# hhcho/sfgwas

Hardware: AMD Instinct MI355X
Metric: pca_power_iter_ring_macs_per_s (higher is better)
Workload: dtype u64 ring words, exact integers: int8 digits on the matrix core for the MAC of all five moduli, fp64-held integers in the encode and key-switch kernels

## Files before the change

sfgwas_amd/csrc/common.hpp:

```cpp
#pragma once
#include <hip/hip_runtime.h>
#include <cstdint>
#include <cstdio>
#include <cstring>
#include <string>
#include <vector>
#include <map>
#include <set>
#include <unistd.h>
#include "../../include/sfgwas_hip.h"
#include "consts.hpp"

typedef unsigned long long u64;
typedef unsigned __int128 u128;

constexpr unsigned long long SFG_I8_BIG_QMAX = 0x7F7F7F7F7F80ULL;

struct ModConst {
    double q, qinv;
    double ninv, ninv_q;
    u64 qi;
};

struct RotKey {
    u64 *key_dev = nullptr;
    uint16_t *index_dev = nullptr;
};

struct PhaseStat { double ms = 0; int launches = 0; double bytes = 0; };
struct PendingEvent { hipEvent_t e0, e1; std::string name; int launches; double bytes; };

struct sfg_geno {
    const int8_t *dev = nullptr;
    size_t nrow = 0, ncol = 0, ld = 0;
    bool owned = false;
    bool packed = false;
    struct PtcEntry { double *slot; bool transposed; };
    mutable std::map<uint64_t, PtcEntry> ptc;
    mutable size_t ptc_budget = 0, ptc_used = 0;
    mutable double *ptc_arena = nullptr;
    mutable uint32_t *ptc_perm = nullptr;
    mutable const void *ptc_owner = nullptr;
    mutable size_t ptc_hits = 0, ptc_fills = 0;
};

struct SfgConfig {
    int mm_group = 8;
    bool mm_group_auto = true;
    size_t acc_budget = 24ULL << 30;
    size_t assoc_cache_budget = 160ULL << 30;
    size_t ksw_budget = 4ULL << 30;
    int enc_batch = 2048;
    bool upload_blocking = false;
    bool test_hooks = false;
    std::string test_scratch_oom;
    double tie_band = 0x1p-50;
    bool mac_i8_big = true;
    bool mac_reg = false;
    bool mac_bc = true;
    bool mac_i8 = true;
    bool mac_i8_nolds = true;
    bool mac_i8_ring = true;
    int mac_i8_waves = 12;
    bool mac_i8_wg1 = false;
    int mac_wc = 1;
    bool no_overlap = true;
    bool ntt_fwd_full = false;
    bool ntt_half_full = false;
    bool pt_compact = true;
    bool pt_kmajor = true;
    int pt_ride = 192;
    int i8_mover_depth_ride = 1, i8_mover_nt_ride = 1;
    bool mac_plain_pt = false;
    bool assoc_trace = false;
};

struct SfgShared {
    int device = 0;
    int logN = SFG_LOGN, N = SFG_N, nq = 0, np = 0, nmod = 0, beta = 0;
    double scale = 0;
    u64 q[SFG_MAXMOD] = {0}, psi[SFG_MAXMOD] = {0};
    double *tw_fwd = nullptr;
    double *tw_inv = nullptr;
    double2 *pack_fwd = nullptr;
    double2 *pack_inv = nullptr;
    ModConst *modc = nullptr;
    ModConst modc_host[SFG_MAXMOD];
    void *enc_tables = nullptr;
    void *rvec_tables = nullptr;
    void *zeros_dev = nullptr;
    u64 *sk_dev = nullptr;
    u64 *pk_dev = nullptr;
    u64 *skqp_dev = nullptr;
    uint32_t enc_key[8] = {0, 0, 0, 0, 0, 0, 0, 0}; uint32_t *enc_key_dev = nullptr; bool enc_seeded = false;
    u64 enc_next = 0;
    std::map<u64, RotKey> rotkeys;
    SfgConfig cfg;
    int refs = 1;
};

struct sfg_ctx {
    SfgShared *sh = nullptr;
    bool is_fork = false;
    int device = 0;
    int logN = SFG_LOGN, N = SFG_N, nq = 0, np = 0, nmod = 0, beta = 0;
    double scale = 0;
    u64 q[SFG_MAXMOD] = {0}, psi[SFG_MAXMOD] = {0};
    double *tw_fwd = nullptr, *tw_inv = nullptr;
    double2 *pack_fwd = nullptr, *pack_inv = nullptr;
    ModConst *modc = nullptr;
    ModConst modc_host[SFG_MAXMOD];
    SfgConfig cfg;
    unsigned ntt_plain_seq = 0;
    struct I8Slot { const void *src = nullptr; u64 sig[8] = {0, 0, 0, 0, 0, 0, 0, 0}; u64 last_use = 0; };
    static constexpr int I8_SLOTS = 16;
    u64 i8_gen = 1, i8_clock = 0; I8Slot i8_slot[2][I8_SLOTS];
    hipStream_t own_stream = nullptr, stream = nullptr;
    hipStream_t user_stream = nullptr;
    hipStream_t aux_stream = nullptr;
    unsigned char *pin = nullptr; size_t pin_bytes = 0, pin_head = 0;
    hipStream_t coll_stream = nullptr;
    hipEvent_t ev_pipe[4] = {nullptr, nullptr, nullptr, nullptr};
    std::vector<hipEvent_t> ev_pool; size_t ev_next = 0;
    std::map<int, void *> ksw_cache;
    void *ws = nullptr; size_t ws_bytes = 0;
    std::map<std::string, std::pair<void *, size_t>> pool;
    std::map<std::string, std::pair<void *, size_t>> host_pool;
    std::map<std::string, unsigned long long> pool_epoch;
    unsigned long long api_epoch = 0; int api_depth = 0;
    int scratch_oom_seen = 0;
    std::vector<PendingEvent> pending;
    std::string err;
    std::map<std::string, PhaseStat> phases;
    std::set<const sfg_geno *> ptc_genos;
    bool test_hooks = false;
    void *tie_count_dev = nullptr;
    hipStream_t main_stream() const { return user_stream ? user_stream : own_stream; }
    std::map<u64, RotKey> &rotkeys() { return sh->rotkeys; }
    const std::map<u64, RotKey> &rotkeys() const { return sh->rotkeys; }
    void *enc_tables() const { return sh->enc_tables; }
    void *zeros_dev() const { return sh->zeros_dev; }
};

int sfg_sync_all(sfg_ctx *ctx);
int sfg_encoder_check(sfg_ctx *ctx);
void sfg_ptc_detach_all(sfg_ctx *ctx);
void sfg_ptc_invalidate_all(sfg_ctx *ctx);

int encrypt_set_attrs(sfg_ctx *ctx);
int sfg_rows_from_montgomery(sfg_ctx *ctx, unsigned long long *rows_dev, size_t nrows, int nmod);
void sfg_encrypt_destroy(SfgShared *sh);
int enc_take_indices(sfg_ctx *ctx, const char *what, int nct, unsigned long long *first);
int keygen_set_attrs(sfg_ctx *ctx);
void sfg_keygen_destroy(SfgShared *sh);
int sfg_rvec_init(sfg_ctx *ctx);
void sfg_rvec_destroy(SfgShared *sh);

extern thread_local std::string g_create_error;

#define SFG_FAIL(ctx, ...) do { char _b[512]; snprintf(_b, sizeof _b, __VA_ARGS__); (ctx)->err = _b; return 1; } while (0)
#ifdef SFG_AB
#include "ab/ab.hpp"
#endif
#define SFG_HIP(ctx, call) do { hipError_t _e = (call); if (_e != hipSuccess) { char _b[512]; \
    snprintf(_b, sizeof _b, "HIP call failed: %s (%s:%d)", hipGetErrorString(_e), __FILE__, __LINE__); (ctx)->err = _b; return 1; } } while (0)
#define SFG_TRY(expr) do { int _rc = (expr); if (_rc) return _rc; } while (0)

int sfg_ws_reserve(sfg_ctx *ctx, size_t bytes);

static inline u64 h_mulmod(u64 a, u64 b, u64 q) { return (u64)(((u128)a * b) % q); }
static inline u64 h_powmod(u64 a, u64 e, u64 q) { u64 r = 1 % q; a %= q; while (e) { if (e & 1) r = h_mulmod(r, a, q); a = h_mulmod(a, a, q); e >>= 1; } return r; }
static inline u64 h_invmod(u64 a, u64 q) { return h_powmod(a, q - 2, q); }
static inline uint32_t h_brev(uint32_t x, int bits) { uint32_t r = 0; for (int i = 0; i < bits; i++) { r = (r << 1) | (x & 1); x >>= 1; } return r; }

int sfg_upload_small(sfg_ctx *ctx, void *dst_dev, const void *src_host, size_t bytes);
struct ApiScope {
    sfg_ctx *c;
    explicit ApiScope(sfg_ctx *c_) : c(c_) { if (c->api_depth++ == 0) c->api_epoch++; }
    ~ApiScope() { c->api_depth--; }
};
struct AuxScope {
    sfg_ctx *c; hipStream_t saved;
    explicit AuxScope(sfg_ctx *c_, bool on = true) : c(c_), saved(c_->stream) { if (on) c->stream = c->aux_stream; }
    ~AuxScope() { c->stream = saved; }
};
template <class T, hipError_t (*Free)(T)> struct HipOwner {
    T h = T();
    HipOwner() {}
    HipOwner(HipOwner &&o) : h(o.release()) {}
    HipOwner(const HipOwner &) = delete; HipOwner &operator=(const HipOwner &) = delete;
    ~HipOwner() { if (h) (void)Free(h); }
    T release() { T t = h; h = T(); return t; }
};
typedef HipOwner<void *, hipFree> DevMem;
typedef HipOwner<hipEvent_t, hipEventDestroy> EventOwner;
typedef HipOwner<hipStream_t, hipStreamDestroy> StreamOwner;
struct FdOwner {
    int fd;
    explicit FdOwner(int fd_ = -1) : fd(fd_) {}
    FdOwner(FdOwner &&o) : fd(o.fd) { o.fd = -1; }
    FdOwner(const FdOwner &) = delete; FdOwner &operator=(const FdOwner &) = delete;
    ~FdOwner() { reset(); }
    void reset(int fd_ = -1) { if (fd >= 0) close(fd); fd = fd_; }
};
int sfg_stream_after(sfg_ctx *ctx, hipStream_t waiter, hipStream_t signaller);
int sfg_scratch(sfg_ctx *ctx, const char *name, size_t bytes, void **out);
int sfg_host_scratch(sfg_ctx *ctx, const char *name, size_t bytes, void **out);
void sfg_phases_resolve(sfg_ctx *ctx);

struct PhaseTimer {
    sfg_ctx *ctx; const char *name; hipEvent_t e0, e1; bool on;
    PhaseTimer(sfg_ctx *c, const char *n, bool enable = true) : ctx(c), name(n), on(enable) {
        if (on) { (void)hipEventCreate(&e0); (void)hipEventCreate(&e1); (void)hipEventRecord(e0, ctx->stream); }
    }
    void stop(int launches = 1, double bytes = 0) {
        if (!on) return;
        (void)hipEventRecord(e1, ctx->stream);
        ctx->pending.push_back(PendingEvent{e0, e1, name, launches, bytes});
        on = false;
        if (ctx->pending.size() > 4096) sfg_phases_resolve(ctx);
    }
    ~PhaseTimer() { stop(0); }
};

constexpr u64 PACKED_ZERO = 0ULL;
#ifdef __HIPCC__
__device__ __host__ __forceinline__ u64 pack_limbs(u64 w) {
    return (w & 0xFFF) | (((w >> 12) & 0xFFF) << 16) | ((w >> 24) << 32);
}

__device__ __forceinline__ double mulmod_lazy(double x, double w, double wq, double q) {
    double qh = __builtin_rint(x * wq);
    double h = x * w;
    double l = __builtin_fma(x, w, -h);
    double r = __builtin_fma(-qh, q, h);
    return r + l;
}
__device__ __forceinline__ double mulmod_lazy_q(double x, double w, double q, double qinv) {
    double h = x * w;
    double qh = __builtin_rint(h * qinv);
    double l = __builtin_fma(x, w, -h);
    double r = __builtin_fma(-qh, q, h);
    return r + l;
}
__device__ __forceinline__ double canon(double x, double q, double qinv) {
    const double r = __builtin_fma(-__builtin_floor(x * qinv), q, x);
    return r == q ? 0.0 : r;
}
__device__ __forceinline__ double canon_le(double x, double q, double qinv) {
    return __builtin_fma(-__builtin_floor(x * qinv), q, x);
}
__device__ __forceinline__ double pred(double x, double q, double qinv) {
    double qh = __builtin_rint(x * qinv);
    return __builtin_fma(-qh, q, x);
}
__device__ __forceinline__ double u64_to_f64(u64 x) {
    return __longlong_as_double((long long)(x | 0x4330000000000000ULL)) - 4503599627370496.0;
}
__device__ __forceinline__ u64 f64_to_u64(double x) {
    return (u64)__double_as_longlong(x + 4503599627370496.0) & 0x000FFFFFFFFFFFFFULL;
}
__device__ __forceinline__ void bytes_tr4(unsigned w0, unsigned w1, unsigned w2, unsigned w3, unsigned (&o)[4]) {
    const unsigned p0 = __builtin_amdgcn_perm(w1, w0, 0x05010400u), p1 = __builtin_amdgcn_perm(w1, w0, 0x07030602u);
    const unsigned q0 = __builtin_amdgcn_perm(w3, w2, 0x05010400u), q1 = __builtin_amdgcn_perm(w3, w2, 0x07030602u);
    o[0] = __builtin_amdgcn_perm(q0, p0, 0x05040100u); o[1] = __builtin_amdgcn_perm(q0, p0, 0x07060302u);
    o[2] = __builtin_amdgcn_perm(q1, p1, 0x05040100u); o[3] = __builtin_amdgcn_perm(q1, p1, 0x07060302u);
}
__device__ __forceinline__ int sq_sum4_i8(int w) {
    const int sq = __builtin_amdgcn_sdot4(w, w, 0, false);
    if (sq < 128) return sq;
    int s = 0;
#pragma unroll
    for (int k = 0; k < 4; k++) { const int x = (int)(int8_t)(w >> (8 * k)); s += (int)(int8_t)(x * x); }
    return s;
}
__device__ __forceinline__ u64 pack_limbs_f64(double x) {
    const u64 b = (u64)__double_as_longlong(x + 4503599627370496.0);
    const unsigned lo = (unsigned)b, hi = (unsigned)(b >> 32);
    const unsigned x01 = ((lo << 4) & 0x0FFF0000u) | (lo & 0xFFFu);
    const unsigned x2 = __builtin_amdgcn_alignbit(hi, lo, 24) & 0xFFFu;
    return ((u64)x2 << 32) | x01;
}
__device__ __forceinline__ u64 d_mulmod_u64(u64 a, u64 b, u64 q) {
    u64 hi = __umul64hi(a, b), lo = a * b;
    u64 r = hi % q;
    for (int i = 63; i >= 0; i--) { u64 top = r >> 63; r = (r << 1) | ((lo >> i) & 1); if (top || r >= q) r -= q; }
    return r;
}
__device__ __forceinline__ u64 splitmix_at(u64 seed, u64 idx) {
    u64 z = seed + 0x9E3779B97F4A7C15ULL * (idx + 1);
    z = (z ^ (z >> 30)) * 0xBF58476D1CE4E5B9ULL;
    z = (z ^ (z >> 27)) * 0x94D049BB133111EBULL;
    return z ^ (z >> 31);
}
#endif
```

sfgwas_amd/csrc/kernels.hpp:

```cpp
#pragma once
#include "common.hpp"
#include "mm_plan.hpp"
#include "assoc_plan.hpp"

constexpr int SFG_MAXPATTERN = 128;
struct ModPattern { int period; int8_t m[SFG_MAXPATTERN]; };
struct RowMap { int rpg; size_t gstride_in, gstride_out; };
struct PanelMap { int G, g, shift0; unsigned packed_mask = 0; int K = 0; };

int launch_ntt_fwd(sfg_ctx *ctx, const u64 *in, u64 *out, size_t nrows, const ModPattern &pat);
int launch_ntt_inv(sfg_ctx *ctx, const u64 *in, u64 *out, size_t nrows, const ModPattern &pat);
int launch_ntt_plain(sfg_ctx *ctx, const double *pc, u64 *out, size_t nplain, int L);
struct MoveJob;
struct PtRide;
int launch_ntt_plain_half(sfg_ctx *ctx, const double *pc, u64 *out_half, size_t nplain, int L, PanelMap pm, const uint32_t *perm = nullptr, const MoveJob *mv = nullptr);
int launch_expand_half(sfg_ctx *ctx, const u64 *half, u64 *full, size_t nrows);
int launch_ntt_fwd_map(sfg_ctx *ctx, const u64 *in, u64 *out, size_t nrows, const ModPattern &pat, const RowMap &rm);
int launch_ntt_inv_map(sfg_ctx *ctx, const u64 *in, u64 *out, size_t nrows, const ModPattern &pat, const RowMap &rm);
struct MacStrides { size_t rot_k, rot_r, pt_k, pt_n, out_n, out_r; bool pt_half = false; bool pt_packed = false; bool pt_digits = false; bool i8 = false; bool i8_big = false; bool pt_digits_big = false;
                    const int8_t *B_small = nullptr, *B_big = nullptr;
                    int pt_layout = 0, pt_L = 0;
                    int B_mode = 0;
                    const int8_t *A_small = nullptr, *A_big = nullptr; };
int launch_mac_i8_small(sfg_ctx *ctx, const double *rotf, size_t rotf_k_stride, size_t rotf_r_stride, int plane0, const u64 *pt, u64 *out, int K, int R, int r0, int Ncols,
                        int l0, int nl, int accumulate, const MacStrides &st);
int launch_mac_i8_big(sfg_ctx *ctx, const double *rotf, size_t rotf_k_stride, size_t rotf_r_stride, int plane0, const u64 *pt, u64 *out, int K, int R, int r0, int Ncols,
                      int l0, int accumulate, const MacStrides &st);
int launch_skew(sfg_ctx *ctx, const int8_t *blk, size_t ld, int r, int c, int transposed, int square, int8_t *D);
struct PcCache { double *slot = nullptr; int mode = 0; const uint32_t *perm = nullptr; };
int launch_encode_rows(sfg_ctx *ctx, const int8_t *D, int shift0, int nshift, int L, u64 *pt, bool half_rows = false, int G = 0, int g = 0, unsigned packed_mask = 0, const PcCache *pcache = nullptr,
                       PtRide *ride = nullptr);
int encode_rows_launches(const sfg_ctx *ctx, int nshift);
int i8_ride_prepare(sfg_ctx *ctx, const u64 *panel, int K, int Ncols, size_t pt_k, size_t pt_n, int layout, int L, int launches, PtRide &ride);
int i8_ride_finish(sfg_ctx *ctx, PtRide &ride);
int i8_ride_tiles(sfg_ctx *ctx, int K, int L, int8_t **Bs, int8_t **Bb);
struct I8Args;
void launch_i8_pack_pt_digits(hipStream_t q, const I8Args &a, unsigned items, bool big);
void launch_move_alone(hipStream_t q, const MoveJob &j);
int launch_share(sfg_ctx *ctx, const u64 *rows, size_t rows_ct_stride, const u64 *xr, size_t x_ct_stride, u64 *h, int nl, int nct);
int launch_add_rows(sfg_ctx *ctx, const u64 *a, size_t a_ct_stride, const u64 *b, size_t b_ct_stride, u64 *out, size_t out_ct_stride, int nl, int nct);
int encrypt_errors_moddown(sfg_ctx *ctx, const int32_t *e0, const int32_t *e1, int nct, int level, u64 *out);
int launch_geno_unpack(sfg_ctx *ctx, const sfg_geno *g, size_t r0, size_t c0, size_t nr, size_t nc, int8_t *out, size_t ld_out);
int launch_rotate_right(sfg_ctx *ctx, const u64 *in, u64 *out, int nct, int level, const int *nrot_host);
int launch_rotate_right_indexed(sfg_ctx *ctx, const u64 *in, int nin, u64 *out, int nct, int level, const int *nrot_host, const int *in_index);
int launch_rotate_right_indexed_f64(sfg_ctx *ctx, const u64 *in, int nin, double *outf, int nct, int level, const int *nrot_host, const int *in_index, int L,
                                    const size_t *out_slot = nullptr);
int launch_relinearize(sfg_ctx *ctx, const u64 *tmp, int nct, int level, const u64 *mid, u64 *out);
int launch_ct_add(sfg_ctx *ctx, const u64 *a, const u64 *b, u64 *out, size_t nct, int level);
int mac_dma_planes(sfg_ctx *ctx, int L, std::vector<int> &plane_of, std::vector<int> &is_big);
double mac_big_maxterm(u64 q);
int launch_rot_to_f64(sfg_ctx *ctx, const u64 *rot, size_t nrows, int nl_rot, int L, double *rotf);
int launch_mac_dma(sfg_ctx *ctx, const double *rotf, size_t rows_per_k, const u64 *pt, u64 *out, int K, int R, int Ncols, int L, int accumulate, const MacStrides &st,
                   const double *rotsum = nullptr);
int launch_rot_sum(sfg_ctx *ctx, const double *rotf, size_t rows_per_k, int K, int L, double *rotsum);
int launch_pack_pt(sfg_ctx *ctx, const u64 *in, u64 *out, size_t nrows, size_t words_per_row, int L, unsigned packed_mask);
unsigned mac_dma_packed_mask(sfg_ctx *ctx, int L);
bool mac_use_dma(const sfg_ctx *ctx);
int launch_mac_bc(sfg_ctx *ctx, const double *rotf, size_t rows_per_k, const u64 *pt, u64 *out, int K, int R, int Ncols, int L, int accumulate, const MacStrides &st,
                  const double *rotsum);
int rotcache_build_rows_tab(sfg_ctx *ctx, const u64 *A, int s, int in_level, int max_level, int nbr, int b0, int b1, const std::vector<std::vector<uint8_t>> *tabs, double *cache);
int assoc_build_rotcache(sfg_ctx *ctx, const u64 *A_dev, int s, int in_level, int max_level, size_t nr, const std::vector<size_t> &widths, double **out);
struct I8RotPre { int G = 0, nbr = 0, s = 0, L = 0; std::vector<int8_t *> As, Ab; };
int i8_rotpre_build(sfg_ctx *ctx, const u64 *A_dev, int s, int in_level, int max_level, int nbr, const std::vector<std::vector<uint8_t>> *tabs, size_t budget_bytes, const char *prefix, I8RotPre &pre);
void i8_rotpre_free(I8RotPre &pre);
struct I8RotPreScope { I8RotPre pre; ~I8RotPreScope() { i8_rotpre_free(pre); } };
int matmul_resident_range_i8pre(sfg_ctx *ctx, const I8RotPre &pre, int s, int max_level, const sfg_geno *g, unsigned flags, int blk0, int blk1, uint64_t *out);
int matmul_accumulate_i8pre(sfg_ctx *ctx, const I8RotPre &pre, int s, int max_level, const sfg_geno *g, unsigned flags, int j0, int j1, int accumulate, uint64_t *acc,
                            size_t acc_col_words = 0);
int launch_i8_pack_rot_to(sfg_ctx *ctx, const double *rotf, size_t rotf_k_stride, size_t rotf_r_stride, int plane0, int K, int R, int l0, int nl, bool big, int8_t *A_out);
struct AssocRot { double *f64 = nullptr; I8RotPre pre; };
int assoc_build_rot(sfg_ctx *ctx, const u64 *A_dev, int s, int in_level, int max_level, size_t nr, const std::vector<size_t> &widths, AssocRot &out);
void assoc_free_rot(AssocRot &r);
struct AssocRotScope { AssocRot r; ~AssocRotScope() { assoc_free_rot(r); } };
int assoc_product(sfg_ctx *ctx, const AssocRot &r, const uint64_t *A_dev, int s, int in_level, int max_level, const sfg_geno *g, unsigned flags, int nct, uint64_t *out);
int assoc_batch_tail(sfg_ctx *ctx, const u64 *tmp, const sfg_geno *g, int s, size_t nct, size_t ctw, uint64_t *out_dev, size_t out_ct_capacity, size_t out_shift,
                     double *sum_host, double *sqsum_host);

int launch_bed_decode(sfg_ctx *ctx, hipStream_t st, const uint8_t *dbed, size_t bps, size_t num_sample, size_t num_snp, const int32_t *rmap, const int32_t *cmap,
                      int8_t *out, size_t ld);
int launch_bed_decode_lut(sfg_ctx *ctx, hipStream_t st, const uint8_t *dbed, size_t bps, size_t num_sample, size_t num_snp, const int32_t *rmap, const int32_t *cmap,
                          int8_t *out, size_t ld, unsigned lut);
int upload_filter_map(sfg_ctx *ctx, const uint8_t *filt, size_t n, DevMem &map, size_t *kept);

int assoc_stream_part(sfg_ctx *ctx, int fmt, const char *path, size_t num_sample, size_t num_snp, const uint8_t *row_filter, const uint8_t *col_filter,
                      size_t batch_snps, const uint64_t *A_dev, int s, int in_level, int max_level, unsigned flags,
                      uint64_t *out_dev, size_t out_ct_capacity, size_t *out_ct, double *sum_host, double *sqsum_host,
                      int part, int nparts, std::vector<std::pair<size_t, size_t>> *ranges);
```

sfgwas_amd/csrc/matmul.hip:

```cpp
#include "common.hpp"
#include "kernels.hpp"
#include "i8_move.hpp"
#include <algorithm>
#include <string>

static inline int ceil_div(size_t a, size_t b) { return (int)((a + b - 1) / b); }

struct Shape {
    size_t nrow, ncol;
    int nbr, m_ct;
    bool transposed;
    const int8_t *dev; size_t ld;
    const sfg_geno *g;
    int rows_of(int bi) const { return (int)(std::min((size_t)(bi + 1) * SFG_SLOTS, nrow) - (size_t)bi * SFG_SLOTS); }
    int cols_of(int bj) const { return (int)(std::min((size_t)(bj + 1) * SFG_SLOTS, ncol) - (size_t)bj * SFG_SLOTS); }
    const int8_t *block(int bi, int bj) const {
        return transposed ? dev + (size_t)bj * SFG_SLOTS * ld + (size_t)bi * SFG_SLOTS
                          : dev + (size_t)bi * SFG_SLOTS * ld + (size_t)bj * SFG_SLOTS;
    }
};
static Shape make_shape(const sfg_geno *g, unsigned flags) {
    Shape sh; sh.transposed = (flags & SFG_TRANSPOSE) != 0;
    sh.nrow = sh.transposed ? g->ncol : g->nrow; sh.ncol = sh.transposed ? g->nrow : g->ncol;
    sh.nbr = ceil_div(sh.nrow, SFG_SLOTS); sh.m_ct = ceil_div(sh.ncol, SFG_SLOTS);
    sh.dev = g->dev; sh.ld = g->ld; sh.g = g; return sh;
}

__global__ void __launch_bounds__(256) k_drop_level(const u64 *in, u64 *out, int nl_in, int nl) {
    const int N = SFG_N; const size_t row = blockIdx.x / (N / 256);
    const size_t ctp = row / nl, m = row % nl;
    const size_t x = (blockIdx.x % (N / 256)) * 256 + threadIdx.x;
    out[row * N + x] = in[(ctp * nl_in + m) * N + x];
}
__global__ void __launch_bounds__(256) k_sum_giants(const u64 *rot, int ngiant, int s, int L, u64 *out, size_t out_i_stride,
                                                    int accumulate, const ModConst *modc) {
    const int N = SFG_N; const size_t row = blockIdx.x / (N / 256);
    const int i = (int)(row / (2 * L)), pl = (int)(row % (2 * L)), l = pl % L;
    const size_t x = (blockIdx.x % (N / 256)) * 256 + threadIdx.x;
    const double q = modc[l].q, qinv = modc[l].qinv;
    double acc = accumulate ? u64_to_f64(out[(size_t)i * out_i_stride + (size_t)pl * N + x]) : 0.0;
    for (int g = 0; g < ngiant; g++) {
        acc += u64_to_f64(rot[(((size_t)g * s + i) * 2 * L + pl) * N + x]);
        if ((g & 31) == 31) acc = pred(acc, q, qinv);
    }
    out[(size_t)i * out_i_stride + (size_t)pl * N + x] = f64_to_u64(canon(acc, q, qinv));
}
__global__ void __launch_bounds__(256) k_reduce_rows(u64 *rows, int L, const ModConst *modc) {
    const int N = SFG_N; const size_t row = blockIdx.x / (N / 256); const int l = (int)(row % L);
    const size_t off = row * N + (blockIdx.x % (N / 256)) * 256 + threadIdx.x;
    rows[off] = rows[off] % modc[l].qi;
}
__global__ void __launch_bounds__(256) k_pt_zero(u64 *pt, size_t pitch_words, size_t seg_words, int L, size_t prow, unsigned packed_mask) {
    const size_t seg = blockIdx.y, x = (size_t)blockIdx.x * 256 + threadIdx.x;
    if (x >= seg_words) return;
    const int l = (int)((x / prow) % L);
    pt[seg * pitch_words + x] = ((packed_mask >> l) & 1u) ? PACKED_ZERO : 0ULL;
}
__global__ void __launch_bounds__(256) k_pt_zero_kmajor(uint8_t *pt, int K, int planes, int n0, int k0, int nk) {
    const size_t blk = ((size_t)(n0 + blockIdx.y) * planes * 64 + blockIdx.x) * (size_t)K * 128 + (size_t)k0 * 128;
    uint4 *p = reinterpret_cast<uint4 *>(pt + blk);
    for (int i = threadIdx.x; i < nk * 8; i += 256) p[i] = make_uint4(0, 0, 0, 0);
}
static int launch_pt_zero_kmajor(sfg_ctx *ctx, u64 *pt, int K, int planes, int n0, int n1, int k0, int k1) {
    if (n1 <= n0 || k1 <= k0) return 0;
    hipLaunchKernelGGL(k_pt_zero_kmajor, dim3((unsigned)(planes * 64), (unsigned)(n1 - n0)), dim3(256), 0, ctx->stream, reinterpret_cast<uint8_t *>(pt), K, planes, n0, k0, k1 - k0);
    SFG_HIP(ctx, hipGetLastError());
    return 0;
}
static int launch_pt_zero(sfg_ctx *ctx, u64 *pt, size_t pitch_words, size_t seg_words, int nseg, int L, size_t prow, unsigned packed_mask) {
    if (!packed_mask) {
        if (nseg == 1) SFG_HIP(ctx, hipMemsetAsync(pt, 0, seg_words * 8, ctx->stream));
        else SFG_HIP(ctx, hipMemset2DAsync(pt, pitch_words * 8, 0, seg_words * 8, nseg, ctx->stream));
        return 0;
    }
    hipLaunchKernelGGL(k_pt_zero, dim3((unsigned)((seg_words + 255) / 256), (unsigned)nseg), dim3(256), 0, ctx->stream, pt, pitch_words, seg_words, L, prow, packed_mask);
    SFG_HIP(ctx, hipGetLastError());
    return 0;
}
constexpr int CS_ROWS = 4096;
__global__ void __launch_bounds__(256) k_colsums(const int8_t *g, size_t nrow, size_t ncol, size_t ld, double *sum, double *sqsum) {
    __shared__ int red[2][16][256 + 1];
    const int tid = threadIdx.x, cg = tid & 15, rl = tid >> 4;
    const size_t col = (size_t)blockIdx.x * 256 + (size_t)cg * 16, r0 = (size_t)blockIdx.y * CS_ROWS, r1 = r0 + CS_ROWS < nrow ? r0 + CS_ROWS : nrow;
    int p1[16], p2[16];
#pragma unroll
    for (int k = 0; k < 16; k++) p1[k] = p2[k] = 0;
    const bool vec = col + 16 <= ncol && ((reinterpret_cast<uintptr_t>(g) | ld) & 15) == 0;
    auto load = [&](size_t i) -> uint4 {
        uint4 v = make_uint4(0, 0, 0, 0);
        if (i >= r1) return v;
        if (vec) v = *reinterpret_cast<const uint4 *>(g + i * ld + col);
        else if (col < ncol) { int8_t b[16]; for (int k = 0; k < 16; k++) b[k] = col + k < ncol ? g[i * ld + col + k] : (int8_t)0; v = *reinterpret_cast<uint4 *>(b); }
        return v;
    };
    for (size_t i = r0 + rl; i < r1; i += 64) {
        const uint4 v0 = load(i), v1 = load(i + 16), v2 = load(i + 32), v3 = load(i + 48);
        const unsigned a0[4] = {v0.x, v0.y, v0.z, v0.w}, a1[4] = {v1.x, v1.y, v1.z, v1.w}, a2[4] = {v2.x, v2.y, v2.z, v2.w}, a3[4] = {v3.x, v3.y, v3.z, v3.w};
#pragma unroll
        for (int q = 0; q < 4; q++) {
            unsigned o[4]; bytes_tr4(a0[q], a1[q], a2[q], a3[q], o);
#pragma unroll
            for (int t = 0; t < 4; t++) {
                unsigned w = o[t];
                const unsigned m = w & 0x80808080u; w &= ~((m << 1) - (m >> 7));
                p1[4 * q + t] = __builtin_amdgcn_sdot4((int)w, 0x01010101, p1[4 * q + t], false);
                p2[4 * q + t] += sq_sum4_i8((int)w);
            }
        }
    }
#pragma unroll
    for (int k = 0; k < 16; k++) { red[0][rl][cg * 16 + k] = p1[k]; red[1][rl][cg * 16 + k] = p2[k]; }
    __syncthreads();
    long long s1 = 0, s2 = 0;
#pragma unroll
    for (int r = 0; r < 16; r++) { s1 += red[0][r][tid]; s2 += red[1][r][tid]; }
    const size_t j = (size_t)blockIdx.x * 256 + tid;
    if (j < ncol) {
        if (sum) atomicAdd(&sum[j], (double)s1);
        if (sqsum) atomicAdd(&sqsum[j], (double)s2);
    }
}

extern "C" int sfg_ct_drop_level_dev(sfg_ctx *ctx, const uint64_t *in, uint64_t *out, int nct, int level_in, int level_out) {
    SFG_HIP(ctx, hipSetDevice(ctx->device));
    if (level_out > level_in) SFG_FAIL(ctx, "DropLevel: requested level %d when input is %d", level_out, level_in);
    if (level_out < 0 || level_in >= ctx->nq || nct < 0) SFG_FAIL(ctx, "DropLevel: level out of range");
    if (!nct) return 0;
    const int nl = level_out + 1, nl_in = level_in + 1;
    if (nl == nl_in) { SFG_HIP(ctx, hipMemcpyAsync(out, in, (size_t)nct * 2 * nl * SFG_N * 8, hipMemcpyDeviceToDevice, ctx->stream)); return 0; }
    hipLaunchKernelGGL(k_drop_level, dim3((unsigned)((size_t)nct * 2 * nl * (SFG_N / 256))), dim3(256), 0, ctx->stream, (const u64 *)in, (u64 *)out, nl_in, nl);
    SFG_HIP(ctx, hipGetLastError());
    return 0;
}
extern "C" int sfg_memcpy_d2d(sfg_ctx *ctx, void *dst, const void *src, size_t bytes) {
    SFG_HIP(ctx, hipSetDevice(ctx->device));
    SFG_HIP(ctx, hipMemcpyAsync(dst, src, bytes, hipMemcpyDeviceToDevice, ctx->stream));
    return 0;
}

extern "C" int sfg_geno_upload(sfg_ctx *ctx, const int8_t *host, size_t nrow, size_t ncol, size_t ld, sfg_geno **out) {
    SFG_HIP(ctx, hipSetDevice(ctx->device));
    if (!nrow || !ncol || ld < ncol) SFG_FAIL(ctx, "sfg_geno_upload: bad dimensions");
    int8_t *d = nullptr;
    SFG_HIP(ctx, hipMalloc(&d, nrow * ncol));
    SFG_HIP(ctx, hipMemcpy2DAsync(d, ncol, host, ld, ncol, nrow, hipMemcpyHostToDevice, ctx->stream));
    SFG_HIP(ctx, hipStreamSynchronize(ctx->stream));
    sfg_geno *g = new sfg_geno(); g->dev = d; g->nrow = nrow; g->ncol = ncol; g->ld = ncol; g->owned = true;
    *out = g; return 0;
}
extern "C" int sfg_geno_create(sfg_ctx *ctx, size_t nrow, size_t ncol, sfg_geno **out) {
    SFG_HIP(ctx, hipSetDevice(ctx->device));
    if (!out) SFG_FAIL(ctx, "sfg_geno_create: null result pointer");
    *out = nullptr;
    if (!nrow || !ncol) SFG_FAIL(ctx, "sfg_geno_create: bad dimensions");
    int8_t *d = nullptr;
    SFG_TRY(sfg_malloc(ctx, (void **)&d, nrow * ncol));
    sfg_geno *g = new sfg_geno(); g->dev = d; g->nrow = nrow; g->ncol = ncol; g->ld = ncol; g->owned = true;
    *out = g; return 0;
}
extern "C" int sfg_geno_write_rows(sfg_ctx *ctx, sfg_geno *g, size_t row0, size_t nrows, const int8_t *rows_host, size_t ld) {
    SFG_HIP(ctx, hipSetDevice(ctx->device));
    if (!g || !g->owned || g->packed) SFG_FAIL(ctx, "sfg_geno_write_rows: not a matrix made by sfg_geno_create");
    if (!nrows) return 0;
    if (!rows_host || ld < g->ncol || row0 > g->nrow || nrows > g->nrow - row0) SFG_FAIL(ctx, "sfg_geno_write_rows: rows [%zu, %zu) of a %zu x %zu matrix, row stride %zu", row0, row0 + nrows, g->nrow, g->ncol, ld);
    if (!g->ptc.empty()) SFG_FAIL(ctx, "sfg_geno_write_rows: the matrix has cached plaintexts (sfg_geno_set_plaintext_cache): it must not change");
    SFG_HIP(ctx, hipMemcpy2DAsync(const_cast<int8_t *>(g->dev) + row0 * g->ld, g->ld, rows_host, ld, g->ncol, nrows, hipMemcpyHostToDevice, ctx->stream));
    SFG_HIP(ctx, hipStreamSynchronize(ctx->stream));
    return 0;
}
__global__ void __launch_bounds__(256) k_geno_compare(const int8_t *chunk, const int8_t *stored, size_t ld, size_t row0, size_t nrows, size_t ncol_l, int transposed, unsigned long long *ndiff) {
    const size_t total = nrows * ncol_l;
    unsigned long long bad = 0;
    for (size_t i = (size_t)blockIdx.x * 256 + threadIdx.x; i < total; i += (size_t)gridDim.x * 256) {
        size_t r, c;
        if (transposed) { r = i % nrows; c = i / nrows; } else { r = i / ncol_l; c = i % ncol_l; }
        const int8_t want = transposed ? stored[c * ld + row0 + r] : stored[(row0 + r) * ld + c];
        bad += chunk[r * ncol_l + c] != want;
    }
    if (bad) atomicAdd(ndiff, bad);
}
extern "C" int sfg_geno_compare_rows(sfg_ctx *ctx, const sfg_geno *g, unsigned flags, size_t row0, size_t nrows, const int8_t *rows_host, size_t ld, uint64_t *ndiff) {
    SFG_HIP(ctx, hipSetDevice(ctx->device));
    if (!g || g->packed || !ndiff) SFG_FAIL(ctx, "sfg_geno_compare_rows: needs an unpacked resident matrix and a result pointer");
    const bool tr = flags & SFG_TRANSPOSE;
    const size_t nrow_l = tr ? g->ncol : g->nrow, ncol_l = tr ? g->nrow : g->ncol;
    if (!nrows) return 0;
    if (!rows_host || ld < ncol_l || row0 > nrow_l || nrows > nrow_l - row0) SFG_FAIL(ctx, "sfg_geno_compare_rows: rows [%zu, %zu) of a %zu x %zu matrix, row stride %zu", row0, row0 + nrows, nrow_l, ncol_l, ld);
    int8_t *chunk = nullptr; unsigned long long *cnt = nullptr;
    SFG_TRY(sfg_scratch(ctx, "geno.cmp", nrows * ncol_l, (void **)&chunk));
    SFG_TRY(sfg_scratch(ctx, "geno.cmpcnt", 8, (void **)&cnt));
    SFG_HIP(ctx, hipMemsetAsync(cnt, 0, 8, ctx->stream));
    SFG_HIP(ctx, hipMemcpy2DAsync(chunk, ncol_l, rows_host, ld, ncol_l, nrows, hipMemcpyHostToDevice, ctx->stream));
    const size_t total = nrows * ncol_l;
    hipLaunchKernelGGL(k_geno_compare, dim3((unsigned)std::min<size_t>((total + 255) / 256, 65536)), dim3(256), 0, ctx->stream, (const int8_t *)chunk, g->dev, g->ld, row0, nrows, ncol_l, tr ? 1 : 0, cnt);
    SFG_HIP(ctx, hipGetLastError());
    unsigned long long h = 0;
    SFG_HIP(ctx, hipMemcpyAsync(&h, cnt, 8, hipMemcpyDeviceToHost, ctx->stream));
    SFG_HIP(ctx, hipStreamSynchronize(ctx->stream));
    *ndiff += h;
    return 0;
}
extern "C" int sfg_pinned_alloc(sfg_ctx *ctx, void **host_ptr, size_t bytes) {
    SFG_HIP(ctx, hipSetDevice(ctx->device));
    if (!host_ptr || !bytes) SFG_FAIL(ctx, "sfg_pinned_alloc: bad arguments");
    SFG_HIP(ctx, hipHostMalloc(host_ptr, bytes, hipHostMallocDefault));
    return 0;
}
extern "C" int sfg_pinned_free(sfg_ctx *ctx, void *host_ptr) {
    SFG_HIP(ctx, hipSetDevice(ctx->device));
    if (host_ptr) SFG_HIP(ctx, hipHostFree(host_ptr));
    return 0;
}
extern "C" int sfg_geno_from_device(sfg_ctx *ctx, const int8_t *dev, size_t nrow, size_t ncol, size_t ld, sfg_geno **out) {
    if (!nrow || !ncol || ld < ncol) SFG_FAIL(ctx, "sfg_geno_from_device: bad dimensions");
    sfg_geno *g = new sfg_geno(); g->dev = dev; g->nrow = nrow; g->ncol = ncol; g->ld = ld; g->owned = false;
    *out = g; return 0;
}
static void ptc_drop(sfg_ctx *ctx, const sfg_geno *g) {
    sfg_ctx *own = g->ptc_owner ? (sfg_ctx *)g->ptc_owner : ctx;
    own->ptc_genos.erase(g);
    if (g->ptc.empty() && !g->ptc_perm) return;
    (void)hipSetDevice(own->device); (void)sfg_sync_all(own);
    if (own != ctx) (void)sfg_sync_all(ctx);
    g->ptc.clear(); g->ptc_used = 0;
    if (g->ptc_arena) { (void)hipFree(g->ptc_arena); g->ptc_arena = nullptr; }
    if (g->ptc_perm) { (void)hipFree(g->ptc_perm); g->ptc_perm = nullptr; }
}
void sfg_ptc_invalidate_all(sfg_ctx *ctx) {
    for (const sfg_geno *g : ctx->ptc_genos) { g->ptc.clear(); g->ptc_used = 0; }
}
void sfg_ptc_detach_all(sfg_ctx *ctx) {
    for (const sfg_geno *g : ctx->ptc_genos) {
        g->ptc.clear(); g->ptc_used = 0; g->ptc_budget = 0;
        if (g->ptc_arena) { (void)hipFree(g->ptc_arena); g->ptc_arena = nullptr; }
        if (g->ptc_perm) { (void)hipFree(g->ptc_perm); g->ptc_perm = nullptr; }
        g->ptc_owner = nullptr;
    }
    ctx->ptc_genos.clear();
}
extern "C" void sfg_geno_free(sfg_ctx *ctx, sfg_geno *g) {
    if (!g) return;
    ptc_drop(ctx, g);
    if (g->owned) { (void)hipSetDevice(ctx->device); (void)sfg_sync_all(ctx); (void)hipFree((void *)g->dev); }
    delete g;
}
extern "C" int sfg_geno_set_plaintext_cache(sfg_ctx *ctx, const sfg_geno *g, size_t max_bytes) {
    SFG_HIP(ctx, hipSetDevice(ctx->device));
    if (!g) SFG_FAIL(ctx, "sfg_geno_set_plaintext_cache: null matrix");
    if (!max_bytes) { ptc_drop(ctx, g); g->ptc_budget = 0; g->ptc_owner = nullptr; return 0; }
    if (g->ptc_owner && g->ptc_owner != (const void *)ctx) SFG_FAIL(ctx, "sfg_geno_set_plaintext_cache: the cache of this matrix belongs to another context (drop it there first)");
    if (!g->ptc_perm) {
        const int n = SFG_SLOTS, d = SFG_D; const unsigned M = 2u * SFG_N;
        std::vector<uint32_t> tab(n);
        std::vector<unsigned> pow5(n); pow5[0] = 1; for (int k = 1; k < n; k++) pow5[k] = (unsigned)(((u64)pow5[k - 1] * 5u) % M);
        for (int t = 0; t < n; t++) {
            const int u = (n - t) % n, k = ((t % d) + d * (u / d)) % n;
            tab[t] = (uint32_t)u | (uint32_t)pow5[k] << 16;
        }
        uint32_t *dv = nullptr;
        SFG_HIP(ctx, hipMalloc((void **)&dv, (size_t)n * 4));
        if (hipMemcpy(dv, tab.data(), (size_t)n * 4, hipMemcpyHostToDevice) != hipSuccess) { (void)hipFree(dv); SFG_FAIL(ctx, "sfg_geno_set_plaintext_cache: table upload failed"); }
        g->ptc_perm = dv;
    }
    const size_t slot_bytes = (size_t)SFG_SLOTS * SFG_SLOTS * 8, want = max_bytes / slot_bytes * slot_bytes;
    if (want != g->ptc_budget || !g->ptc_arena) {
        (void)hipStreamSynchronize(ctx->stream);
        g->ptc.clear(); g->ptc_used = 0;
        if (g->ptc_arena) { (void)hipFree(g->ptc_arena); g->ptc_arena = nullptr; }
        g->ptc_budget = 0;
        if (!want) SFG_FAIL(ctx, "sfg_geno_set_plaintext_cache: max_bytes is less than one block (%zu bytes)", slot_bytes);
        void *a = nullptr;
        if (hipMalloc(&a, want) != hipSuccess) { (void)hipGetLastError(); SFG_FAIL(ctx, "sfg_geno_set_plaintext_cache: cannot allocate %zu bytes", want); }
        g->ptc_arena = (double *)a; g->ptc_budget = want;
    }
    g->ptc_owner = ctx; ctx->ptc_genos.insert(g);
    return 0;
}
extern "C" int sfg_geno_plaintext_cache_stats(sfg_ctx *ctx, const sfg_geno *g, size_t *blocks, size_t *bytes, size_t *hits, size_t *fills) {
    if (!g) SFG_FAIL(ctx, "sfg_geno_plaintext_cache_stats: null matrix");
    if (blocks) *blocks = g->ptc.size();
    if (bytes) *bytes = g->ptc_used;
    if (hits) *hits = g->ptc_hits;
    if (fills) *fills = g->ptc_fills;
    return 0;
}
extern "C" int sfg_geno_colsums(sfg_ctx *ctx, const sfg_geno *g, double *sum_host, double *sqsum_host) {
    SFG_HIP(ctx, hipSetDevice(ctx->device));
    if (g->packed) {
        sfg_geno *u = nullptr; SFG_TRY(sfg_geno_unpack(ctx, g, &u));
        const int rc = sfg_geno_colsums(ctx, u, sum_host, sqsum_host); sfg_geno_free(ctx, u); return rc;
    }
    SFG_TRY(sfg_ws_reserve(ctx, g->ncol * 16));
    double *ds = (double *)ctx->ws, *dq = ds + g->ncol;
    SFG_HIP(ctx, hipMemsetAsync(ds, 0, g->ncol * 16, ctx->stream));
    hipLaunchKernelGGL(k_colsums, dim3((unsigned)((g->ncol + 255) / 256), (unsigned)((g->nrow + CS_ROWS - 1) / CS_ROWS)), dim3(256), 0, ctx->stream, g->dev, g->nrow, g->ncol, g->ld, ds, dq);
    SFG_HIP(ctx, hipGetLastError());
    if (sum_host) SFG_HIP(ctx, hipMemcpyAsync(sum_host, ds, g->ncol * 8, hipMemcpyDeviceToHost, ctx->stream));
    if (sqsum_host) SFG_HIP(ctx, hipMemcpyAsync(sqsum_host, dq, g->ncol * 8, hipMemcpyDeviceToHost, ctx->stream));
    SFG_HIP(ctx, hipStreamSynchronize(ctx->stream));
    return 0;
}
extern "C" int sfg_reduce_rows_dev(sfg_ctx *ctx, uint64_t *rows, size_t nrows_of_L, int L) {
    SFG_HIP(ctx, hipSetDevice(ctx->device));
    const size_t rows_total = nrows_of_L * L;
    if (!rows_total) return 0;
    hipLaunchKernelGGL(k_reduce_rows, dim3((unsigned)(rows_total * (SFG_N / 256))), dim3(256), 0, ctx->stream, (u64 *)rows, L, ctx->modc);
    SFG_HIP(ctx, hipGetLastError());
    return 0;
}

static int build_rot_row_tab(sfg_ctx *ctx, const u64 *A, int s, int nl_in, int nl, int lev, int L, int nbr, int bi, const std::vector<uint8_t> &baby_t,
                             u64 *a_row, u64 *rotc, bool dma, double *rotf_dst);
static int build_rot_row(sfg_ctx *ctx, const u64 *A, int s, int nl_in, int nl, int lev, int L, const Shape &sh, int bi, u64 *a_row, u64 *rotc,
                         bool dma, double *rotf_dst) {
    const int d = SFG_D;
    const int nr = sh.rows_of(bi);
    std::vector<uint8_t> baby_t(d, 0);
    for (int shift = 0; shift < SFG_SLOTS; shift++) {
        if (baby_t[shift % d]) continue;
        bool any = false;
        for (int bj = 0; bj < sh.m_ct && !any; bj++) any = diag_bool(nr, sh.cols_of(bj), SFG_SLOTS, -shift);
        if (any) baby_t[shift % d] = 1;
    }
    return build_rot_row_tab(ctx, A, s, nl_in, nl, lev, L, sh.nbr, bi, baby_t, a_row, rotc, dma, rotf_dst);
}
static int build_rot_row_tab(sfg_ctx *ctx, const u64 *A, int s, int nl_in, int nl, int lev, int L, int nbr, int bi, const std::vector<uint8_t> &baby_t,
                             u64 *a_row, u64 *rotc, bool dma, double *rotf_dst) {
    const int N = SFG_N, d = SFG_D; const size_t ctw = (size_t)2 * nl * N;
    for (int i = 0; i < s; i++) {
        const u64 *src = A + ((size_t)i * nbr + bi) * 2 * nl_in * N;
        if (nl == nl_in) SFG_HIP(ctx, hipMemcpyAsync(a_row + (size_t)i * ctw, src, ctw * 8, hipMemcpyDeviceToDevice, ctx->stream));
        else hipLaunchKernelGGL(k_drop_level, dim3((unsigned)(2 * nl * (N / 256))), dim3(256), 0, ctx->stream, src, a_row + (size_t)i * ctw, nl_in, nl);
    }
    SFG_HIP(ctx, hipGetLastError());
    {
        PhaseTimer t(ctx, "rotate");
        std::vector<int> nrv((size_t)d * s, 0), inv((size_t)d * s, 0);
        for (int baby = 0; baby < d; baby++) for (int i = 0; i < s; i++) { nrv[(size_t)baby * s + i] = baby_t[baby] ? -baby : 0; inv[(size_t)baby * s + i] = i; }
        if (dma) SFG_TRY(launch_rotate_right_indexed_f64(ctx, a_row, s, rotf_dst, d * s, lev, nrv.data(), inv.data(), L));
        else SFG_TRY(launch_rotate_right_indexed(ctx, a_row, s, rotc, d * s, lev, nrv.data(), inv.data()));
        t.stop(1);
    }
    return 0;
}

static MmPlanIn plan_input(sfg_ctx *ctx, int s, int L, int nblockrows, int ncolb, RotSrc rot, int pre_G) {
    const SfgConfig &c = ctx->cfg;
    MmPlanIn in;
    in.mm_group = c.mm_group; in.mm_group_auto = c.mm_group_auto; in.mac_i8 = c.mac_i8; in.mac_i8_big = c.mac_i8_big;
    in.pt_compact = c.pt_compact; in.pt_kmajor = c.pt_kmajor; in.pt_ride = c.pt_ride; in.no_overlap = c.no_overlap;
    in.dma = mac_use_dma(ctx); in.packed_mask = in.dma ? mac_dma_packed_mask(ctx, L) : 0u; in.mods = ModSplit(ctx->q, L);
    in.s = s; in.L = L; in.nblockrows = nblockrows; in.ncolb = ncolb; in.rot = rot; in.pre_G = pre_G;
    if (mm_plan_reads_memory(in)) {
        size_t fr = 0, tot = 0;
        in.mem_failed = hipMemGetInfo(&fr, &tot) != hipSuccess;
        in.mem_search = in.mem_keep = fr;
        for (const auto &kv : ctx->pool) {
            if (kv.first == "mm.pt" || kv.first == "mm.rotf" || kv.first.rfind("mi8.", 0) == 0) in.mem_search += kv.second.second;
            if (kv.first.rfind("mi8.A", 0) == 0) in.mem_keep += kv.second.second;
        }
    }
    return in;
}
struct MmCall {
    sfg_ctx *ctx; const Shape &sh; unsigned flags; const u64 *A; const I8RotPre *pre8;
    int s, L, lev, nl, nl_in; bool dma; unsigned packed_mask; size_t ctw, accw, rowf = 0;
    MmPlan plan;
    u64 *a_row = nullptr, *rotc = nullptr; int8_t *skew = nullptr, *unpacked = nullptr; double *rotf = nullptr, *rotsum = nullptr;
    int8_t *rideBs = nullptr, *rideBb = nullptr;
};
struct MacJob { bool on = false; u64 *ptp = nullptr; int gsn = 0, gi = 0, acc_flag = 0; u64 *accj = nullptr; const double *rotf_grp = nullptr, *rotsum_grp = nullptr; };

static int build_group(const MmCall &c, int bg, int b1, int buf) {
    sfg_ctx *ctx = c.ctx; const int d = SFG_D, s = c.s, ng = std::min(c.plan.G, b1 - bg);
    ctx->i8_gen++;
    double *dst = c.rotf + (size_t)buf * c.plan.grp_slices * s * 2 * c.rowf;
    for (int g = 0; g < ng; g++) SFG_TRY(build_rot_row(ctx, c.A, s, c.nl_in, c.nl, c.lev, c.L, c.sh, bg + g, c.a_row, c.rotc, c.dma, c.dma ? dst + (size_t)g * d * s * 2 * c.rowf : nullptr));
    if (c.dma && (ng * d) % 4)
        SFG_HIP(ctx, hipMemsetAsync(dst + (size_t)ng * d * s * 2 * c.rowf, 0, (size_t)3 * s * 2 * c.rowf * 8, ctx->stream));
    if (c.packed_mask) SFG_TRY(launch_rot_sum(ctx, dst, (size_t)s * 2, ng * d, c.L, c.rotsum + (size_t)buf * s * 2 * c.rowf));
    return 0;
}
static int run_mac(const MmCall &c, const MacJob &m, int B_mode) {
    sfg_ctx *ctx = c.ctx; const MmPlan &p = c.plan; const int N = SFG_N, d = SFG_D;
    PhaseTimer t(ctx, "mac");
    MacStrides st;
    if (c.rideBs) { st.B_small = c.rideBs; st.B_big = c.rideBb; st.B_mode = B_mode; }
    if (c.pre8) { st.A_small = c.pre8->As[m.gi]; st.A_big = c.pre8->Ab[m.gi]; }
    st.rot_k = (size_t)c.s * c.ctw; st.rot_r = (size_t)c.nl * N;
    st.pt_k = p.plw; st.pt_n = (size_t)m.gsn * d * p.plw; st.pt_half = c.dma; st.pt_packed = c.packed_mask != 0; st.pt_digits = st.i8 = p.use_i8; st.i8_big = st.pt_digits_big = p.use_i8_big;
    st.pt_layout = p.pt_layout; st.pt_L = c.L;
    st.out_n = c.accw; st.out_r = (size_t)c.L * N;
    int rc;
    if (c.dma) rc = launch_mac_dma(ctx, c.pre8 ? nullptr : m.rotf_grp, (size_t)c.s * 2, m.ptp, m.accj, m.gsn * d, 2 * c.s, d, c.L, m.acc_flag, st, m.rotsum_grp);
#ifdef SFG_AB
    else rc = launch_mac_strided(ctx, c.rotc, m.ptp, m.accj, d, 2 * c.s, d, c.L, m.acc_flag, st);
#else
    else { rc = 1; ctx->err = "matmul: the register-staged MAC exists in the A/B build only (make ab)"; }
#endif
    t.stop(1);
    return rc;
}
struct PtcSlot {
    static constexpr size_t slot_bytes = (size_t)SFG_SLOTS * SFG_SLOTS * 8;
    PcCache pcc; const sfg_geno *g; uint64_t key = 0; bool fresh = false;
    PtcSlot(const MmCall &c, int bi, int bj) : g(c.sh.g) {
        if (!c.dma || !g->ptc_budget || g->ptc_owner != (const void *)c.ctx) return;
        const uint64_t sr = c.sh.transposed ? bj : bi, sc = c.sh.transposed ? bi : bj;
        key = sr << 33 | sc << 1 | ((c.flags & SFG_SQUARE) ? 1u : 0u);
        auto it = g->ptc.find(key);
        if (it != g->ptc.end()) { pcc.slot = it->second.slot; pcc.mode = it->second.transposed == c.sh.transposed ? 2 : 3; pcc.perm = g->ptc_perm; g->ptc_hits++; }
        else if (g->ptc_used + slot_bytes <= g->ptc_budget) {
            double *slot = g->ptc_arena + g->ptc_used / 8;
            g->ptc[key] = sfg_geno::PtcEntry{slot, c.sh.transposed}; g->ptc_used += slot_bytes; g->ptc_fills++;
            pcc.slot = slot; pcc.mode = 1; fresh = true;
        }
    }
    void undo() {
        if (!fresh) return;
        auto it = g->ptc.find(key);
        if (it != g->ptc.end()) { g->ptc.erase(it); g->ptc_used -= slot_bytes; }
        fresh = false;
    }
};
static int encode_block(const MmCall &c, int bi, int bj, int g, int ng, u64 *pt, PtRide *ride) {
    sfg_ctx *ctx = c.ctx; const Shape &sh = c.sh; const MmPlan &p = c.plan;
    const int d = SFG_D, L = c.L, nr = sh.rows_of(bi), nc = sh.cols_of(bj), tr = sh.transposed ? 1 : 0, sq = (c.flags & SFG_SQUARE) ? 1 : 0;
    const size_t plw = p.plw, nplain = (size_t)d * d;
    PtcSlot ptc(c, bi, bj);
    int rc = 0;
    if (ptc.pcc.mode < 2) {
        PhaseTimer t(ctx, "skew");
        if (sh.g->packed) {
            const size_t sr0 = (size_t)(tr ? bj : bi) * SFG_SLOTS, sc0 = (size_t)(tr ? bi : bj) * SFG_SLOTS;
            rc = launch_geno_unpack(ctx, sh.g, sr0, sc0, tr ? nc : nr, tr ? nr : nc, c.unpacked, SFG_SLOTS);
            if (!rc) rc = launch_skew(ctx, c.unpacked, SFG_SLOTS, nr, nc, tr, sq, c.skew);
        } else rc = launch_skew(ctx, sh.block(bi, bj), sh.ld, nr, nc, tr, sq, c.skew);
        t.stop(1);
    }
    if (rc) { ptc.undo(); return rc; }
    int runs[2][2]; int nruns = 0;
    if (nr + nc > SFG_SLOTS) { runs[0][0] = 0; runs[0][1] = SFG_SLOTS; nruns = 1; }
    else { runs[0][0] = 0; runs[0][1] = nr; runs[1][0] = SFG_SLOTS - nc + 1; runs[1][1] = SFG_SLOTS; nruns = runs[1][0] < runs[1][1] ? 2 : 1; }
    const bool full = nruns == 1 && runs[0][1] - runs[0][0] == SFG_SLOTS;
    if (p.kmajor) {
        const int kb0 = g * d;
        if (full) rc = launch_pt_zero_kmajor(ctx, pt, ng * d, p.pt_planes, d - 1, d, kb0 + (SFG_SLOTS - (d - 1) * d), kb0 + d);
        else rc = launch_pt_zero_kmajor(ctx, pt, ng * d, p.pt_planes, 0, d, kb0, kb0 + d);
    } else if (full) {
        rc = launch_pt_zero(ctx, pt + (((size_t)(d - 1) * ng + g) * d + (SFG_SLOTS - (d - 1) * d)) * plw, 0, (nplain - SFG_SLOTS) * plw, 1, L, p.prow, c.packed_mask);
    } else {
        rc = launch_pt_zero(ctx, pt + (size_t)g * d * plw, (size_t)ng * d * plw, (size_t)d * plw, d, L, p.prow, c.packed_mask);
    }
    if (rc) { ptc.undo(); return rc; }
    PhaseTimer t(ctx, "encode");
    for (int r = 0; r < nruns && !rc; r++) {
        if (c.dma) rc = launch_encode_rows(ctx, c.skew, runs[r][0], runs[r][1] - runs[r][0], L, pt, true, ng, g, p.enc_flags, ptc.pcc.mode ? &ptc.pcc : nullptr, ride);
        else rc = launch_encode_rows(ctx, c.skew, runs[r][0], runs[r][1] - runs[r][0], L, pt + (size_t)runs[r][0] * plw, false);
    }
    t.stop(nruns);
    if (rc) ptc.undo();
    return rc;
}
static int ride_launch_count(const MmCall &c, int bg, int ng, int nc) {
    int launches = 0;
    for (int g = 0; g < ng; g++) {
        const int nr = c.sh.rows_of(bg + g);
        if (nr + nc > SFG_SLOTS) launches += encode_rows_launches(c.ctx, SFG_SLOTS);
        else launches += encode_rows_launches(c.ctx, nr) + (nc > 1 ? encode_rows_launches(c.ctx, nc - 1) : 0);
    }
    return launches;
}

static int matmul_accumulate(sfg_ctx *ctx, const u64 *A, int s, int in_level, int max_level, const Shape &sh, unsigned flags,
                             int b0, int b1, int j0, int j1, int accumulate, u64 *acc, const double *rotf_pre = nullptr, const double *rotsum_pre = nullptr,
                             const I8RotPre *pre8 = nullptr, size_t acc_col_words = 0) {
    const int N = SFG_N, d = SFG_D, L = max_level;
    if (pre8 && (rotf_pre || !mac_use_dma(ctx) || b0 != 0 || b1 != pre8->nbr || sh.nbr != pre8->nbr || s != pre8->s || L != pre8->L))
        SFG_FAIL(ctx, "matmul: internal: the int8 rot tiles were built for another product (block rows %d, s = %d, level %d)", pre8->nbr, pre8->s, pre8->L);
    const int lev = in_level > max_level ? max_level : in_level, nl = lev + 1, nl_in = in_level + 1;
    if (L < 1 || L > ctx->nq) SFG_FAIL(ctx, "matmul: max_level out of range");
    if (nl < L) SFG_FAIL(ctx, "matmul: input level %d has fewer than max_level = %d moduli", in_level, max_level);
    if (b0 < 0 || b1 > sh.nbr || b0 > b1 || j0 < 0 || j1 > sh.m_ct || j0 > j1) SFG_FAIL(ctx, "matmul: block range out of bounds");
    const size_t ctw = (size_t)2 * nl * N, accw = (size_t)s * 2 * L * N;
    const int ncolb = j1 - j0;
    const size_t acc_col = acc_col_words ? acc_col_words : (size_t)d * accw;
    if (acc_col < (size_t)d * accw) SFG_FAIL(ctx, "matmul: internal: accumulator column stride below 91 giant steps");
    if (b0 == b1 || j0 == j1) {
        if (!accumulate) for (int c = 0; c < ncolb; c++) SFG_HIP(ctx, hipMemsetAsync(acc + (size_t)c * acc_col, 0, (size_t)d * accw * 8, ctx->stream));
        return 0;
    }
    const MmPlanIn in = plan_input(ctx, s, L, b1 - b0, ncolb, rotf_pre ? RotSrc::f64_cache : pre8 ? RotSrc::i8_tiles : RotSrc::own, pre8 ? pre8->G : 0);
    if (in.dma && in.mods.too_big) SFG_FAIL(ctx, "sfg_mac: modulus >= 2^47 unsupported by the fp64 limb schedule");
    MmCall c{ctx, sh, flags, A, pre8, s, L, lev, nl, nl_in, in.dma, in.packed_mask, ctw, accw};
    c.plan = mm_plan(in);
    MmPlan &plan = c.plan;
    const int G = plan.G; const bool dma = in.dma, rot_ext = in.rot != RotSrc::own;
    if (rotsum_pre && G < rotsum_group_size(in.mm_group, in.nblockrows)) SFG_FAIL(ctx, "matmul: internal: fewer rot-sum groups than MAC groups");
    u64 *pt = nullptr;
    SFG_TRY(sfg_scratch(ctx, "mm.a_row", (size_t)s * ctw * 8, (void **)&c.a_row));
    SFG_TRY(sfg_scratch(ctx, "mm.rotc", dma ? 8 : (size_t)d * s * ctw * 8, (void **)&c.rotc));
    if (plan.ride_want && sfg_scratch(ctx, "mm.pt", plan.panel_words * 8 * 2 + 65536, (void **)&pt)) { ctx->err.clear(); plan.ride_want = false; }
    if (!plan.ride_want) SFG_TRY(sfg_scratch(ctx, "mm.pt", plan.panel_words * 8 + 65536, (void **)&pt));
    u64 *const pt_base = pt;
    SFG_TRY(sfg_scratch(ctx, "mm.skew", (size_t)SFG_SLOTS * SFG_SLOTS, (void **)&c.skew));
    if (sh.g->packed) SFG_TRY(sfg_scratch(ctx, "mm.unpack", (size_t)SFG_SLOTS * SFG_SLOTS, (void **)&c.unpacked));
    if (dma) {
        c.rowf = (size_t)in.mods.fp64_planes * N;
        if (!rot_ext) SFG_TRY(sfg_scratch(ctx, "mm.rotf", plan.grp_slices * s * 2 * c.rowf * 8 * (plan.pipelined ? 2 : 1), (void **)&c.rotf));
        if (!rot_ext && in.packed_mask) SFG_TRY(sfg_scratch(ctx, "mm.rotsum", (size_t)2 * s * 2 * c.rowf * 8, (void **)&c.rotsum));
    }
    const size_t rot_half = plan.grp_slices * s * 2 * c.rowf, rotsum_half = (size_t)s * 2 * c.rowf;
    hipStream_t main_stream = ctx->stream;
    if (plan.pipelined) {
        SFG_TRY(sfg_stream_after(ctx, ctx->aux_stream, main_stream));
        { AuxScope aux(ctx); SFG_TRY(build_group(c, b0, b1, 0)); }
        SFG_HIP(ctx, hipEventRecord(ctx->ev_pipe[0], ctx->aux_stream));
    }
    int rc = 0, gi = 0, it = 0;
    MacJob held;
    for (int bg = b0; bg < b1; bg += G, gi++) {
        const int ng = std::min(G, b1 - bg);
        if (held.on && !pre8) { SFG_TRY(run_mac(c, held, 2)); held.on = false; }
        const double *rotf_grp = c.rotf, *rotsum_grp = c.rotsum;
        if (rotf_pre) { rotf_grp = rotf_pre + (size_t)(bg - b0) * d * s * 2 * c.rowf; rotsum_grp = rotsum_pre ? rotsum_pre + (size_t)gi * rotsum_half : nullptr; }
        else if (pre8) { rotf_grp = nullptr; rotsum_grp = nullptr; }
        else if (plan.pipelined) {
            if (bg + G < b1) {
                SFG_TRY(sfg_stream_after(ctx, ctx->aux_stream, main_stream));
                { AuxScope aux(ctx); SFG_TRY(build_group(c, bg + G, b1, (gi + 1) & 1)); }
                SFG_HIP(ctx, hipEventRecord(ctx->ev_pipe[(gi + 1) & 1], ctx->aux_stream));
            }
            SFG_HIP(ctx, hipStreamWaitEvent(main_stream, ctx->ev_pipe[gi & 1], 0));
            rotf_grp = c.rotf + (size_t)(gi & 1) * rot_half;
            if (c.rotsum) rotsum_grp = c.rotsum + (size_t)(gi & 1) * rotsum_half;
        } else SFG_TRY(build_group(c, bg, b1, 0));
        for (int bj = j0; bj < j1; bj++, it++) {
            pt = pt_base + (size_t)(plan.ride_want ? (it & 1) : 0) * plan.panel_words;
            PtRide ride;
            if (plan.ride_want && !c.rideBs) SFG_TRY(i8_ride_tiles(ctx, G * d, L, &c.rideBs, &c.rideBb));
            if (held.on && plan.ride_want && c.rideBs) {
                SFG_TRY(i8_ride_prepare(ctx, held.ptp, held.gsn * d, d, plan.plw, (size_t)held.gsn * d * plan.plw, plan.pt_layout, L, ride_launch_count(c, bg, ng, sh.cols_of(bj)), ride));
                if (ride.on && (ride.job.a5.B != c.rideBs || (ride.job.n6 && ride.job.a6.B != c.rideBb))) SFG_FAIL(ctx, "matmul: internal: the riding transposition's tile buffers moved");
            }
            if (held.on && !ride.on) { SFG_TRY(run_mac(c, held, c.rideBs ? 2 : 0)); held.on = false; }
            for (int g = 0; g < ng; g++) SFG_TRY(encode_block(c, bg + g, bj, g, ng, pt, ride.on ? &ride : nullptr));
            if (held.on) { SFG_TRY(i8_ride_finish(ctx, ride)); SFG_TRY(run_mac(c, held, 1)); held.on = false; }
            MacJob m; m.on = true; m.ptp = pt; m.gsn = ng; m.gi = gi;
            m.acc_flag = (accumulate || bg != b0) ? 1 : 0;
            m.accj = acc + (size_t)(bj - j0) * acc_col; m.rotf_grp = rotf_grp; m.rotsum_grp = rotsum_grp;
            if (plan.ride_want && c.rideBs) held = m;
            else SFG_TRY(run_mac(c, m, c.rideBs ? 2 : 0));
        }
    }
    if (held.on) rc = run_mac(c, held, 2);
    return rc;
}

static int matmul_finalize(sfg_ctx *ctx, const u64 *acc, int s, int max_level, int ncolb, int m_ct_out, int jout0, int g0, int g1,
                           const std::vector<uint8_t> *giant_active, int accumulate, u64 *out, int acc_giants = SFG_D, int giant_base = 0) {
    const int N = SFG_N, d = SFG_D, L = max_level;
    const size_t accw = (size_t)s * 2 * L * N, ctw = (size_t)2 * L * N;
    if (g0 < 0 || g1 > acc_giants || g0 > g1 || giant_base < 0) SFG_FAIL(ctx, "finalize: giant range out of bounds");
    u64 *rot = nullptr;
    SFG_TRY(sfg_scratch(ctx, "mm.fin_rot", (size_t)d * accw * 8, (void **)&rot));
    std::vector<int> glist;
    for (int g = g0; g < g1; g++) if (giant_base + g < d && (!giant_active || (*giant_active)[giant_base + g])) glist.push_back(g);
    const int ng = (int)glist.size();
    std::vector<int> nrv((size_t)ng * s), inv((size_t)ng * s);
    for (int k = 0; k < ng; k++) for (int i = 0; i < s; i++) { nrv[(size_t)k * s + i] = -(giant_base + glist[k]) * d; inv[(size_t)k * s + i] = glist[k] * s + i; }
    int rc = 0;
    for (int jb = 0; jb < ncolb && !rc; jb++) {
        const u64 *accj = acc + (size_t)jb * acc_giants * accw;
        u64 *o = out + (size_t)(jout0 + jb) * ctw;
        if (ng) {
            PhaseTimer t(ctx, "rotate");
            rc = launch_rotate_right_indexed(ctx, accj, acc_giants * s, rot, ng * s, L - 1, nrv.data(), inv.data());
            t.stop(1);
            if (rc) break;
        }
        hipLaunchKernelGGL(k_sum_giants, dim3((unsigned)((size_t)s * 2 * L * (N / 256))), dim3(256), 0, ctx->stream, rot, ng, s, L,
                           o, (size_t)m_ct_out * ctw, accumulate, ctx->modc);
        if (hipGetLastError() != hipSuccess) { rc = 1; ctx->err = "finalize: k_sum_giants launch failed"; }
    }
    return rc;
}

static void giant_table(const Shape &sh, std::vector<uint8_t> &giant_t) {
    giant_t.assign(SFG_D, 0);
    for (int bi = 0; bi < sh.nbr; bi++) {
        const int nr = sh.rows_of(bi);
        for (int shift = 0; shift < SFG_SLOTS; shift++) {
            if (giant_t[shift / SFG_D]) { shift = (shift / SFG_D + 1) * SFG_D - 1; continue; }
            bool any = false;
            for (int bj = 0; bj < sh.m_ct && !any; bj++) any = diag_bool(nr, sh.cols_of(bj), SFG_SLOTS, -shift);
            if (any) giant_t[shift / SFG_D] = 1;
        }
    }
}

extern "C" int sfg_matmul_accumulate_dev(sfg_ctx *ctx, const uint64_t *A, int s, int in_level, int max_level, const sfg_geno *g, unsigned flags,
                                         int b0, int b1, int j0, int j1, int accumulate, uint64_t *acc) {
    ApiScope api_scope(ctx);
    SFG_HIP(ctx, hipSetDevice(ctx->device));
    Shape sh = make_shape(g, flags);
    return matmul_accumulate(ctx, (const u64 *)A, s, in_level, max_level, sh, flags, b0, b1, j0, j1, accumulate, (u64 *)acc);
}
extern "C" int sfg_matmul_finalize_dev(sfg_ctx *ctx, const uint64_t *acc, int s, int max_level, int ncolb, int g0, int g1, int accumulate, uint64_t *out) {
    ApiScope api_scope(ctx);
    SFG_HIP(ctx, hipSetDevice(ctx->device));
    return matmul_finalize(ctx, (const u64 *)acc, s, max_level, ncolb, ncolb, 0, g0, g1, nullptr, accumulate, (u64 *)out);
}

extern "C" int sfg_matmul_finalize_slots_dev(sfg_ctx *ctx, const uint64_t *acc, int s, int max_level, int ncolb, int acc_giants, int giant_base,
                                             int g0, int g1, int accumulate, uint64_t *out) {
    ApiScope api_scope(ctx);
    SFG_HIP(ctx, hipSetDevice(ctx->device));
    if (acc_giants < 1) SFG_FAIL(ctx, "finalize: acc_giants must be positive");
    return matmul_finalize(ctx, (const u64 *)acc, s, max_level, ncolb, ncolb, 0, g0, g1, nullptr, accumulate, (u64 *)out, acc_giants, giant_base);
}

static int matmul_resident_range(sfg_ctx *ctx, const uint64_t *A, int s, int in_level, int max_level, const sfg_geno *g, unsigned flags,
                                 int blk0, int blk1, uint64_t *out, const double *rotf_ext, const I8RotPre *pre8 = nullptr) {
    SFG_HIP(ctx, hipSetDevice(ctx->device));
    ctx->phases.clear();
    if (!rotf_ext && !pre8) ctx->i8_gen++;
    Shape sh = make_shape(g, flags);
    const int d = SFG_D, L = max_level, N = SFG_N;
    const size_t accw = (size_t)s * 2 * L * N;
    std::vector<uint8_t> giant_t; giant_table(sh, giant_t);
    int b0 = 0, b1 = sh.nbr, j0 = 0, j1 = sh.m_ct;
    if (sh.transposed) { b0 = blk0; b1 = blk1; } else { j0 = blk0; j1 = blk1; }
    if (b0 < 0 || b1 > sh.nbr || j0 < 0 || j1 > sh.m_ct || b0 > b1 || j0 > j1) SFG_FAIL(ctx, "matmul: SNP-block range out of bounds");
    const int m_out = j1 - j0;
    const size_t budget = ctx->cfg.acc_budget;
    int jg = (int)(budget / ((size_t)d * accw * 8)); if (jg < 1) jg = 1;
    const double *rotf_all = rotf_ext, *rotsum_all = nullptr;
    if (rotf_ext && !mac_use_dma(ctx)) SFG_FAIL(ctx, "matmul: a prebuilt rotation cache needs the LDS-DMA MAC (the A/B build selected the register-staged kernel)");
    if (!rotf_ext && !pre8 && mac_use_dma(ctx) && j1 - j0 > jg && b1 > b0) {
        std::vector<int> plane_of, is_big; const int nplanes = mac_dma_planes(ctx, L, plane_of, is_big);
        if (nplanes < 0) return 1;
        const size_t rowf = (size_t)nplanes * N, per_row = (size_t)d * s * 2 * rowf;
        const int lev = in_level > max_level ? max_level : in_level, nl = lev + 1;
        if (nl >= L && ((size_t)(b1 - b0) * per_row + 3 * (size_t)s * 2 * rowf) * 8 <= (48ULL << 30)) {
            double *buf = nullptr; u64 *a_row = nullptr, *rotc = nullptr;
            const size_t ctw = (size_t)2 * nl * N;
            SFG_TRY(sfg_scratch(ctx, "mm.rotf", ((size_t)(b1 - b0) * per_row + 3 * (size_t)s * 2 * rowf) * 8, (void **)&buf));
            SFG_TRY(sfg_scratch(ctx, "mm.a_row", (size_t)s * ctw * 8, (void **)&a_row));
            SFG_TRY(sfg_scratch(ctx, "mm.rotc", 8, (void **)&rotc));
            for (int bi = b0; bi < b1; bi++) SFG_TRY(build_rot_row(ctx, (const u64 *)A, s, in_level + 1, nl, lev, L, sh, bi, a_row, rotc, true, buf + (size_t)(bi - b0) * per_row));
            SFG_HIP(ctx, hipMemsetAsync(buf + (size_t)(b1 - b0) * per_row, 0, 3 * (size_t)s * 2 * rowf * 8, ctx->stream));
            rotf_all = buf;
            if (mac_dma_packed_mask(ctx, L)) {
                const int G = rotsum_group_size(ctx->cfg.mm_group, b1 - b0), ngrp = (b1 - b0 + G - 1) / G;
                double *rs = nullptr;
                SFG_TRY(sfg_scratch(ctx, "mm.rotsum_all", (size_t)ngrp * s * 2 * rowf * 8, (void **)&rs));
                for (int gi = 0; gi < ngrp; gi++) {
                    const int ng = std::min(G, b1 - b0 - gi * G);
                    SFG_TRY(launch_rot_sum(ctx, buf + (size_t)gi * G * per_row, (size_t)s * 2, ng * d, L, rs + (size_t)gi * s * 2 * rowf));
                }
                rotsum_all = rs;
            }
        }
    }
    const bool overlap = (rotf_all || pre8) && !ctx->cfg.no_overlap;
    if (overlap) { jg = (jg + 1) / 2; }
    hipStream_t main_stream = ctx->stream;
    int k = 0;
    for (int ja = j0; ja < j1; ja += jg, k++) {
        const int jb = std::min(j1, ja + jg);
        u64 *acc = nullptr;
        SFG_TRY(sfg_scratch(ctx, "mm.acc", (size_t)jg * d * accw * 8 * (overlap ? 2 : 1), (void **)&acc));
        if (overlap) {
            acc += (size_t)(k & 1) * jg * d * accw;
            if (k >= 2) SFG_HIP(ctx, hipStreamWaitEvent(main_stream, ctx->ev_pipe[2 + (k & 1)], 0));
        }
        int rc = matmul_accumulate(ctx, (const u64 *)A, s, in_level, max_level, sh, flags, b0, b1, ja, jb, 0, acc, rotf_all, rotsum_all, pre8);
        if (rc) return rc;
        if (overlap) {
            SFG_TRY(sfg_stream_after(ctx, ctx->aux_stream, main_stream));
            { AuxScope aux(ctx); rc = matmul_finalize(ctx, acc, s, max_level, jb - ja, m_out, ja - j0, 0, d, &giant_t, 0, (u64 *)out); }
            if (rc) return rc;
            SFG_HIP(ctx, hipEventRecord(ctx->ev_pipe[2 + (k & 1)], ctx->aux_stream));
        } else {
            rc = matmul_finalize(ctx, acc, s, max_level, jb - ja, m_out, ja - j0, 0, d, &giant_t, 0, (u64 *)out);
            if (rc) return rc;
        }
    }
    if (overlap) SFG_TRY(sfg_stream_after(ctx, main_stream, ctx->aux_stream));
    return 0;
}
extern "C" int sfg_matmul_resident_range_dev(sfg_ctx *ctx, const uint64_t *A, int s, int in_level, int max_level, const sfg_geno *g, unsigned flags,
                                             int blk0, int blk1, uint64_t *out) {
    ApiScope api_scope(ctx);
    return matmul_resident_range(ctx, A, s, in_level, max_level, g, flags, blk0, blk1, out, nullptr);
}

static int rotcache_rowf(sfg_ctx *ctx, int L, size_t &rowf) {
    if (!mac_use_dma(ctx)) SFG_FAIL(ctx, "rotation cache objects need the LDS-DMA MAC (the A/B build selected the register-staged kernel)");
    if (L < 1 || L > ctx->nq) SFG_FAIL(ctx, "rotcache: max_level out of range");
    std::vector<int> plane_of, is_big; const int nplanes = mac_dma_planes(ctx, L, plane_of, is_big);
    if (nplanes < 0) return 1;
    rowf = (size_t)nplanes * SFG_N; return 0;
}
extern "C" int sfg_rotcache_layout(sfg_ctx *ctx, int s, int max_level, size_t *job_doubles, size_t *tail_doubles) {
    size_t rowf = 0; SFG_TRY(rotcache_rowf(ctx, max_level, rowf));
    if (job_doubles) *job_doubles = (size_t)SFG_D * 2 * rowf;
    if (tail_doubles) *tail_doubles = (size_t)3 * s * 2 * rowf;
    return 0;
}
extern "C" int sfg_rotcache_build_jobs_dev(sfg_ctx *ctx, const uint64_t *A, int s, int in_level, int max_level, int nbr, int job0, int job1, double *staged) {
    ApiScope api_scope(ctx);
    SFG_HIP(ctx, hipSetDevice(ctx->device));
    const int N = SFG_N, d = SFG_D, L = max_level;
    size_t rowf = 0; SFG_TRY(rotcache_rowf(ctx, L, rowf));
    const int lev = in_level > max_level ? max_level : in_level, nl = lev + 1, nl_in = in_level + 1;
    if (nl < L || in_level >= ctx->nq) SFG_FAIL(ctx, "rotcache: input level %d unusable with max_level = %d", in_level, max_level);
    if (s < 1 || nbr < 1 || job0 < 0 || job1 > nbr * s || job0 > job1) SFG_FAIL(ctx, "rotcache: job range out of bounds");
    const size_t ctw = (size_t)2 * nl * N;
    constexpr int CH = 64;
    u64 *a_in = nullptr;
    SFG_TRY(sfg_scratch(ctx, "rc.in", (size_t)CH * ctw * 8, (void **)&a_in));
    PhaseTimer t(ctx, "rotate");
    for (int c0 = job0; c0 < job1; c0 += CH) {
        const int nj = std::min(CH, job1 - c0);
        for (int k = 0; k < nj; k++) {
            const int job = c0 + k, bi = job / s, i = job % s;
            const u64 *src = (const u64 *)A + ((size_t)i * nbr + bi) * 2 * nl_in * N;
            if (nl == nl_in) SFG_HIP(ctx, hipMemcpyAsync(a_in + (size_t)k * ctw, src, ctw * 8, hipMemcpyDeviceToDevice, ctx->stream));
            else hipLaunchKernelGGL(k_drop_level, dim3((unsigned)(2 * nl * (N / 256))), dim3(256), 0, ctx->stream, src, a_in + (size_t)k * ctw, nl_in, nl);
        }
        SFG_HIP(ctx, hipGetLastError());
        std::vector<int> nrv((size_t)d * nj), inv((size_t)d * nj); std::vector<size_t> slot((size_t)d * nj);
        for (int baby = 0; baby < d; baby++) for (int k = 0; k < nj; k++) {
            nrv[(size_t)baby * nj + k] = -baby; inv[(size_t)baby * nj + k] = k; slot[(size_t)baby * nj + k] = (size_t)(c0 - job0 + k) * d + baby;
        }
        SFG_TRY(launch_rotate_right_indexed_f64(ctx, a_in, nj, staged, d * nj, lev, nrv.data(), inv.data(), L, slot.data()));
    }
    t.stop(1);
    return 0;
}
extern "C" int sfg_rotcache_scatter_dev(sfg_ctx *ctx, const double *staged, int s, int max_level, int job0, int job1, int row0, int nrows, double *cache) {
    ApiScope api_scope(ctx);
    SFG_HIP(ctx, hipSetDevice(ctx->device));
    ctx->i8_gen++;
    const int d = SFG_D;
    size_t rowf = 0; SFG_TRY(rotcache_rowf(ctx, max_level, rowf));
    if (s < 1 || nrows < 1 || job0 < row0 * s || job1 > (row0 + nrows) * s || job0 > job1) SFG_FAIL(ctx, "rotcache: job range outside the cache rows");
    const size_t jw = (size_t)2 * rowf;
    for (int job = job0; job < job1; job++) {
        const int bi = job / s, i = job % s;
        SFG_HIP(ctx, hipMemcpy2DAsync(cache + (((size_t)(bi - row0) * d) * s + i) * jw, (size_t)s * jw * 8, staged + (size_t)(job - job0) * d * jw, jw * 8, jw * 8, d,
                                      hipMemcpyDeviceToDevice, ctx->stream));
    }
    SFG_HIP(ctx, hipMemsetAsync(cache + (size_t)nrows * d * s * jw, 0, (size_t)3 * s * jw * 8, ctx->stream));
    return 0;
}
int rotcache_build_rows_tab(sfg_ctx *ctx, const u64 *A, int s, int in_level, int max_level, int nbr, int b0, int b1, const std::vector<std::vector<uint8_t>> *tabs, double *cache) {
    ctx->i8_gen++;
    SFG_HIP(ctx, hipSetDevice(ctx->device));
    const int N = SFG_N, d = SFG_D, L = max_level;
    size_t rowf = 0; SFG_TRY(rotcache_rowf(ctx, L, rowf));
    const int lev = in_level > max_level ? max_level : in_level, nl = lev + 1;
    if (nl < L || in_level >= ctx->nq) SFG_FAIL(ctx, "rotcache: input level %d unusable with max_level = %d", in_level, max_level);
    if (s < 1 || b0 < 0 || b1 > nbr || b0 > b1) SFG_FAIL(ctx, "rotcache: block-row range out of bounds");
    const size_t ctw = (size_t)2 * nl * N, per_row = (size_t)d * s * 2 * rowf;
    u64 *a_row = nullptr, *rotc = nullptr;
    SFG_TRY(sfg_scratch(ctx, "mm.a_row", (size_t)s * ctw * 8, (void **)&a_row));
    SFG_TRY(sfg_scratch(ctx, "mm.rotc", 8, (void **)&rotc));
    const std::vector<uint8_t> all(d, 1);
    for (int bi = b0; bi < b1; bi++)
        SFG_TRY(build_rot_row_tab(ctx, A, s, in_level + 1, nl, lev, L, nbr, bi, tabs ? (*tabs)[bi - b0] : all, a_row, rotc, true, cache + (size_t)(bi - b0) * per_row));
    SFG_HIP(ctx, hipMemsetAsync(cache + (size_t)(b1 - b0) * per_row, 0, (size_t)3 * s * 2 * rowf * 8, ctx->stream));
    return 0;
}
extern "C" int sfg_rotcache_build_rows_dev(sfg_ctx *ctx, const uint64_t *A, int s, int in_level, int max_level, int nbr, int b0, int b1, double *cache) {
    ApiScope api_scope(ctx);
    return rotcache_build_rows_tab(ctx, (const u64 *)A, s, in_level, max_level, nbr, b0, b1, nullptr, cache);
}
void i8_rotpre_free(I8RotPre &pre) { pre = I8RotPre(); }
int i8_rotpre_build(sfg_ctx *ctx, const u64 *A, int s, int in_level, int max_level, int nbr, const std::vector<std::vector<uint8_t>> *tabs, size_t budget_bytes, const char *prefix, I8RotPre &pre) {
    pre = I8RotPre();
    const int d = SFG_D, L = max_level;
    const auto &c = ctx->cfg;
    if (!mac_use_dma(ctx) || !c.mac_bc || c.mac_plain_pt || !c.mac_i8 || !c.mac_i8_big || 2 * s > 30 || L < 1 || L > ctx->nq || nbr < 1) return 0;
    if (!mac_dma_packed_mask(ctx, L)) return 0;
    const ModSplit m(ctx->q, L);
    const int l_big = m.l_big, l_s0 = m.l_small0, n_s = m.nsmall; const int *plane_of = m.plane_of;
    const size_t rowf = (size_t)m.fp64_planes * SFG_N;
    size_t have = 0, tot = 0; bool mem_failed = false;
    if (c.mm_group_auto && nbr > c.mm_group) {
        mem_failed = hipMemGetInfo(&have, &tot) != hipSuccess;
        for (const auto &kv : ctx->pool) if (kv.first.rfind(prefix, 0) == 0 || kv.first == "mm.pt" || kv.first == "mm.rotf" || kv.first.rfind("mi8.", 0) == 0) have += kv.second.second;
    }
    int G = i8pre_group_size(m, c.mm_group, c.mm_group_auto, s, nbr, mem_failed, have, budget_bytes);
    if (!G) return 0;
    double *tmp = nullptr;
    auto alloc_all = [&](int Gc) -> bool {
        const int ngc = (nbr + Gc - 1) / Gc;
        pre.As.assign(ngc, nullptr); pre.Ab.assign(ngc, nullptr);
        int arc = sfg_scratch(ctx, "mm.rotf", ((size_t)Gc * d + 3) * s * 2 * rowf * 8, (void **)&tmp);
        for (int gi = 0; gi < ngc && !arc; gi++) {
            const int ng = std::min(Gc, nbr - gi * Gc);
            char nm[48];
            snprintf(nm, sizeof nm, "%s.s%d", prefix, gi);
            arc = sfg_scratch(ctx, nm, mac_i8_rot_tile_bytes(ng * d, n_s, 5), (void **)&pre.As[gi]);
            if (!arc && l_big >= 0) { snprintf(nm, sizeof nm, "%s.b%d", prefix, gi); arc = sfg_scratch(ctx, nm, mac_i8_rot_tile_bytes(ng * d, 1, 6), (void **)&pre.Ab[gi]); }
        }
        if (arc) { ctx->err.clear(); i8_rotpre_free(pre); }
        return !arc;
    };
    if (!alloc_all(G)) {
        const int G0 = std::min(c.mm_group, nbr);
        if (G0 == G) return 0;
        G = G0;
        if (!alloc_all(G)) return 0;
    }
    const int ngrp = (nbr + G - 1) / G;
    for (int gi = 0; gi < ngrp; gi++) {
        const int bg = gi * G, ng = std::min(G, nbr - bg);
        std::vector<std::vector<uint8_t>> sub;
        if (tabs) sub.assign(tabs->begin() + bg, tabs->begin() + bg + ng);
        int rc = rotcache_build_rows_tab(ctx, A, s, in_level, max_level, nbr, bg, bg + ng, tabs ? &sub : nullptr, tmp);
        if (!rc) rc = launch_i8_pack_rot_to(ctx, tmp, (size_t)s * 2 * rowf, rowf, plane_of[l_s0], ng * d, 2 * s, l_s0, n_s, false, pre.As[gi]);
        if (!rc && l_big >= 0) rc = launch_i8_pack_rot_to(ctx, tmp, (size_t)s * 2 * rowf, rowf, plane_of[l_big], ng * d, 2 * s, l_big, 1, true, pre.Ab[gi]);
        if (rc) { i8_rotpre_free(pre); return rc; }
    }
    pre.G = G; pre.nbr = nbr; pre.s = s; pre.L = L;
    return 0;
}
int matmul_resident_range_i8pre(sfg_ctx *ctx, const I8RotPre &pre, int s, int max_level, const sfg_geno *g, unsigned flags, int blk0, int blk1, uint64_t *out) {
    ApiScope api_scope(ctx);
    if (!pre.G) SFG_FAIL(ctx, "matmul: no int8 rot tiles");
    return matmul_resident_range(ctx, nullptr, s, max_level, max_level, g, flags, blk0, blk1, out, nullptr, &pre);
}
int matmul_accumulate_i8pre(sfg_ctx *ctx, const I8RotPre &pre, int s, int max_level, const sfg_geno *g, unsigned flags, int j0, int j1, int accumulate, uint64_t *acc, size_t acc_col_words) {
    ApiScope api_scope(ctx);
    SFG_HIP(ctx, hipSetDevice(ctx->device));
    if (!pre.G) SFG_FAIL(ctx, "matmul: no int8 rot tiles");
    Shape sh = make_shape(g, flags);
    return matmul_accumulate(ctx, nullptr, s, max_level, max_level, sh, flags, 0, pre.nbr, j0, j1, accumulate, (u64 *)acc, nullptr, nullptr, &pre, acc_col_words);
}
extern "C" int sfg_matmul_resident_range_rc_dev(sfg_ctx *ctx, const double *cache, int s, int max_level, const sfg_geno *g, unsigned flags,
                                                int blk0, int blk1, uint64_t *out) {
    ApiScope api_scope(ctx);
    if (!cache) SFG_FAIL(ctx, "matmul: null rotation cache");
    return matmul_resident_range(ctx, nullptr, s, max_level, max_level, g, flags, blk0, blk1, out, cache);
}
extern "C" int sfg_matmul_accumulate_rc_dev(sfg_ctx *ctx, const double *cache, int s, int max_level, const sfg_geno *g, unsigned flags,
                                            int b0, int b1, int j0, int j1, int accumulate, uint64_t *acc) {
    ApiScope api_scope(ctx);
    SFG_HIP(ctx, hipSetDevice(ctx->device));
    if (!cache) SFG_FAIL(ctx, "matmul: null rotation cache");
    if (!mac_use_dma(ctx)) SFG_FAIL(ctx, "matmul: a prebuilt rotation cache needs the LDS-DMA MAC (the A/B build selected the register-staged kernel)");
    Shape sh = make_shape(g, flags);
    return matmul_accumulate(ctx, nullptr, s, max_level, max_level, sh, flags, b0, b1, j0, j1, accumulate, (u64 *)acc, cache, nullptr);
}

extern "C" int sfg_matmul_resident_dev(sfg_ctx *ctx, const uint64_t *A, int s, int in_level, int max_level, const sfg_geno *g, unsigned flags, uint64_t *out) {
    ApiScope api_scope(ctx);
    const size_t nb = (g->ncol + SFG_SLOTS - 1) / SFG_SLOTS;
    return sfg_matmul_resident_range_dev(ctx, A, s, in_level, max_level, g, flags, 0, (int)nb, out);
}

extern "C" int sfg_matmul_stream(sfg_ctx *ctx, const uint64_t *A_host, int s, int in_level, int max_level,
                                 const int8_t *geno_host, size_t nrow, size_t ncol, size_t ld, unsigned flags,
                                 uint64_t *out_host, double *sum_host, double *sqsum_host) {
    ApiScope api_scope(ctx);
    SFG_HIP(ctx, hipSetDevice(ctx->device));
    sfg_geno *g = nullptr;
    SFG_TRY(sfg_geno_upload(ctx, geno_host, nrow, ncol, ld, &g));
    Shape sh = make_shape(g, flags);
    const size_t a_words = (size_t)s * sh.nbr * 2 * (in_level + 1) * SFG_N, o_words = (size_t)s * sh.m_ct * 2 * max_level * SFG_N;
    u64 *dA = nullptr, *dO = nullptr; int rc = 0;
    if (hipMalloc(&dA, a_words * 8) != hipSuccess || hipMalloc(&dO, o_words * 8) != hipSuccess) { rc = 1; ctx->err = "matmul_stream: out of device memory"; }
    if (!rc && hipMemcpy(dA, A_host, a_words * 8, hipMemcpyHostToDevice) != hipSuccess) { rc = 1; ctx->err = "matmul_stream: upload failed"; }
    if (!rc && (sum_host || sqsum_host)) rc = sfg_geno_colsums(ctx, g, sum_host, sqsum_host);
    if (!rc) rc = sfg_matmul_resident_dev(ctx, (const uint64_t *)dA, s, in_level, max_level, g, flags, (uint64_t *)dO);
    if (!rc && (hipMemcpyAsync(out_host, dO, o_words * 8, hipMemcpyDeviceToHost, ctx->stream) != hipSuccess ||
                hipStreamSynchronize(ctx->stream) != hipSuccess)) { rc = 1; ctx->err = "matmul_stream: download failed"; }
    (void)hipStreamSynchronize(ctx->stream);
    (void)hipFree(dA); (void)hipFree(dO); sfg_geno_free(ctx, g);
    if (!rc) rc = sfg_encoder_check(ctx);
    return rc;
}


struct DiagCacheHdr { uint64_t vectorLen, level, n, numModuli, rowSize; double scale; std::vector<uint8_t> baby, giant; long data_pos; };
static int dc_open(sfg_ctx *ctx, const std::string &fn, FILE **fp, DiagCacheHdr &h) {
    FILE *f = fopen(fn.c_str(), "rb");
    if (!f) SFG_FAIL(ctx, "matmul_from_cache: cannot open %s", fn.c_str());
    unsigned char b[48];
    auto le = [&](int k) { uint64_t v = 0; for (int i = 0; i < 8; i++) v |= (uint64_t)b[8 * k + i] << (8 * i); return v; };
    h.baby.assign(SFG_D, 0); h.giant.assign(SFG_D, 0);
    if (fread(b, 1, 48, f) != 48 || fread(h.baby.data(), 1, SFG_D, f) != (size_t)SFG_D || fread(h.giant.data(), 1, SFG_D, f) != (size_t)SFG_D) { fclose(f); SFG_FAIL(ctx, "matmul_from_cache: short header in %s", fn.c_str()); }
    h.vectorLen = le(0); h.level = le(1); uint64_t sb = le(2); memcpy(&h.scale, &sb, 8); h.n = le(3); h.numModuli = le(4); h.rowSize = le(5);
    h.data_pos = ftell(f);
    *fp = f; return 0;
}
__global__ void __launch_bounds__(256) k_cache_to_panel(const u64 *raw, const uint8_t *present, u64 *panel, int jp, int L, unsigned packed_mask,
                                                        const u64 *r64inv, const ModConst *modc, unsigned long long *asym) {
    const int N = SFG_N, n = N / 2;
    const size_t row = blockIdx.x / (n / 256);
    const int l = (int)(row % L); const size_t bj = row / L; const int j = (int)(bj % jp), baby = (int)(bj / jp);
    const int x = (int)(blockIdx.x % (n / 256)) * 256 + threadIdx.x;
    u64 *dst = panel + (((size_t)j * SFG_D + baby) * L + l) * n;
    const bool packed = (packed_mask >> l) & 1u;
    if (!present[bj]) { dst[x] = packed ? PACKED_ZERO : 0ULL; return; }
    const u64 *src = raw + row * N;
    const u64 be = src[x], bm = src[N - 1 - x];
    if (be != bm) atomicAdd(asym, 1ULL);
    const u64 w = __builtin_bswap64(be);
    const u64 v = d_mulmod_u64(w % modc[l].qi, r64inv[l], modc[l].qi);
    dst[x] = packed ? pack_limbs(v) : v;
}

__global__ void __launch_bounds__(256) k_cache_payload(const u64 *pt, u64 *out, int LV, const u64 *r64, const ModConst *modc) {
    const int N = SFG_N; const size_t row = blockIdx.x / (N / 256); const int l = (int)(row % LV);
    const size_t x = row * N + (blockIdx.x % (N / 256)) * 256 + threadIdx.x;
    out[x] = __builtin_bswap64(d_mulmod_u64(pt[x], r64[l], modc[l].qi));
}
extern "C" int sfg_diagcache_write(sfg_ctx *ctx, const sfg_geno *g, unsigned flags, int max_level, const char *prefix, int *files_written) {
    ApiScope api_scope(ctx);
    SFG_HIP(ctx, hipSetDevice(ctx->device));
    if (files_written) *files_written = 0;
    if (!g || !prefix) SFG_FAIL(ctx, "sfg_diagcache_write: null argument");
    if (flags & ~SFG_TRANSPOSE) SFG_FAIL(ctx, "sfg_diagcache_write: only the transpose flag is meaningful here (MatMult4StreamPreprocess neither squares nor sums)");
    const int LV = max_level + 1;
    if (max_level < 1 || LV > ctx->nq) SFG_FAIL(ctx, "sfg_diagcache_write: max_level out of range");
    if (g->packed) {
        sfg_geno *u = nullptr; SFG_TRY(sfg_geno_unpack(ctx, g, &u));
        const int rc = sfg_diagcache_write(ctx, u, flags, max_level, prefix, files_written); sfg_geno_free(ctx, u); return rc;
    }
    const Shape sh = make_shape(g, flags);
    const int N = SFG_N, d = SFG_D, slots = SFG_SLOTS;
    const size_t ptw = (size_t)LV * N;
    const size_t row_size = 4 + (1 + ptw * 8) * (size_t)sh.m_ct;
    u64 r64_h[SFG_MAXMOD];
    for (int l = 0; l < LV; l++) { const unsigned __int128 t = ((unsigned __int128)1 << 64) % ctx->q[l]; r64_h[l] = (u64)t; }
    u64 *r64_d = nullptr; int8_t *skew = nullptr; u64 *half = nullptr, *full = nullptr, *pay_d = nullptr; unsigned char *pay_h = nullptr;
    const int BATCH = 64;
    SFG_TRY(sfg_scratch(ctx, "dcw.r64", SFG_MAXMOD * 8, (void **)&r64_d));
    SFG_TRY(sfg_scratch(ctx, "enc.skew", (size_t)slots * slots, (void **)&skew));
    SFG_TRY(sfg_scratch(ctx, "enc.half", (size_t)BATCH * LV * (N / 2) * 8, (void **)&half));
    SFG_TRY(sfg_scratch(ctx, "dcw.full", (size_t)BATCH * ptw * 8, (void **)&full));
    SFG_TRY(sfg_scratch(ctx, "dcw.pay", (size_t)BATCH * ptw * 8, (void **)&pay_d));
    SFG_HIP(ctx, hipMemcpyAsync(r64_d, r64_h, SFG_MAXMOD * 8, hipMemcpyHostToDevice, ctx->stream));
    SFG_HIP(ctx, hipHostMalloc((void **)&pay_h, (size_t)BATCH * ptw * 8, hipHostMallocDefault));
    int rc = 0, written = 0;
    for (int bi = 0; bi < sh.nbr && !rc; bi++) {
        const std::string fn = std::string(prefix) + "_" + std::to_string(bi) + ".bin";
        if (FILE *t = fopen(fn.c_str(), "rb")) { fclose(t); continue; }
        const int nr = sh.rows_of(bi);
        std::vector<uint8_t> baby_t(d, 0), giant_t(d, 0), shift_t(slots, 0);
        std::vector<std::vector<uint8_t>> has(sh.m_ct, std::vector<uint8_t>(slots, 0));
        for (int shift = 0; shift < slots; shift++) {
            bool any = false;
            for (int bj = 0; bj < sh.m_ct; bj++) { has[bj][shift] = diag_bool(nr, sh.cols_of(bj), slots, -shift) ? 1 : 0; any = any || has[bj][shift]; }
            if (any) { baby_t[shift % d] = 1; giant_t[shift / d] = 1; shift_t[shift] = 1; }
        }
        const std::string tmp = fn + ".part";
        FILE *f = fopen(tmp.c_str(), "wb");
        if (!f) { ctx->err = "sfg_diagcache_write: cannot create " + tmp; rc = 1; break; }
        {
            uint64_t sb; const double sc = ctx->scale; memcpy(&sb, &sc, 8);
            const uint64_t hdr[6] = {(uint64_t)sh.m_ct, (uint64_t)max_level, sb, (uint64_t)N, (uint64_t)LV, (uint64_t)row_size};
            unsigned char hb[48]; for (int k = 0; k < 6; k++) for (int i = 0; i < 8; i++) hb[8 * k + i] = (unsigned char)(hdr[k] >> (8 * i));
            if (fwrite(hb, 1, 48, f) != 48 || fwrite(baby_t.data(), 1, d, f) != (size_t)d || fwrite(giant_t.data(), 1, d, f) != (size_t)d) rc = 1;
        }
        std::vector<long long> rec_pos(slots, -1); long long pos = 48 + 2 * d;
        for (int shift = 0; shift < slots && !rc; shift++) if (shift_t[shift]) {
            size_t len = 4; for (int bj = 0; bj < sh.m_ct; bj++) len += 1 + (has[bj][shift] ? ptw * 8 : 0);
            unsigned char head[12]; for (int i = 0; i < 8; i++) head[i] = (unsigned char)((uint64_t)len >> (8 * i));
            for (int i = 0; i < 4; i++) head[8 + i] = (unsigned char)((uint32_t)shift >> (8 * i));
            if (fseeko(f, pos, SEEK_SET) || fwrite(head, 1, 12, f) != 12) { rc = 1; break; }
            rec_pos[shift] = pos + 12; pos += 8 + (long long)len;
        }
        for (int bj = 0; bj < sh.m_ct && !rc; bj++) {
            const int nc = sh.cols_of(bj);
            rc = launch_skew(ctx, sh.block(bi, bj), sh.ld, nr, nc, sh.transposed ? 1 : 0, 0, skew);
            for (int s0 = 0; s0 < slots && !rc; s0 += BATCH) {
                int lo = -1, hi = -1;
                for (int sft = s0; sft < std::min(slots, s0 + BATCH); sft++) if (has[bj][sft]) { if (lo < 0) lo = sft; hi = sft + 1; }
                if (lo >= 0) {
                    const int nb = hi - lo;
                    rc = launch_encode_rows(ctx, skew, lo, nb, LV, half, true);
                    if (!rc) rc = launch_expand_half(ctx, half, full, (size_t)nb * LV);
                    if (!rc) {
                        hipLaunchKernelGGL(k_cache_payload, dim3((unsigned)((size_t)nb * LV * (N / 256))), dim3(256), 0, ctx->stream, full, pay_d, LV, r64_d, ctx->modc);
                        if (hipGetLastError() != hipSuccess || hipMemcpyAsync(pay_h, pay_d, (size_t)nb * ptw * 8, hipMemcpyDeviceToHost, ctx->stream) != hipSuccess ||
                            hipStreamSynchronize(ctx->stream) != hipSuccess) { ctx->err = "sfg_diagcache_write: device work failed"; rc = 1; }
                    }
                }
                for (int sft = s0; sft < std::min(slots, s0 + BATCH) && !rc; sft++) if (shift_t[sft]) {
                    long long off = rec_pos[sft]; for (int k = 0; k < bj; k++) off += 1 + (has[k][sft] ? (long long)ptw * 8 : 0);
                    const unsigned char flag = has[bj][sft] ? 0 : 1;
                    if (fseeko(f, off, SEEK_SET) || fwrite(&flag, 1, 1, f) != 1) { rc = 1; break; }
                    if (has[bj][sft] && fwrite(pay_h + (size_t)(sft - lo) * ptw * 8, 1, ptw * 8, f) != ptw * 8) { rc = 1; break; }
                }
            }
        }
        if (fclose(f)) rc = 1;
        if (!rc && rename(tmp.c_str(), fn.c_str())) rc = 1;
        if (rc) { remove(tmp.c_str()); if (ctx->err.empty()) ctx->err = "sfg_diagcache_write: I/O error on " + fn; break; }
        written++;
    }
    (void)hipHostFree(pay_h);
    if (files_written) *files_written = written;
    if (!rc) rc = sfg_encoder_check(ctx);
    return rc;
}

extern "C" int sfg_diagcache_header(sfg_ctx *ctx, const char *prefix, int block_row, uint64_t hdr[6]) {
    FILE *f = nullptr; DiagCacheHdr h;
    SFG_TRY(dc_open(ctx, std::string(prefix) + "_" + std::to_string(block_row) + ".bin", &f, h));
    fclose(f);
    uint64_t sb; memcpy(&sb, &h.scale, 8);
    hdr[0] = h.vectorLen; hdr[1] = h.level; hdr[2] = sb; hdr[3] = h.n; hdr[4] = h.numModuli; hdr[5] = h.rowSize;
    return 0;
}

extern "C" int sfg_matmul_from_cache(sfg_ctx *ctx, const uint64_t *A, int s, int in_level, int max_level, const char *prefix, int nbr, uint64_t *out) {
    ApiScope api_scope(ctx);
    SFG_HIP(ctx, hipSetDevice(ctx->device));
    ctx->phases.clear();
    if (!mac_use_dma(ctx)) SFG_FAIL(ctx, "matmul_from_cache needs the LDS-DMA MAC (the A/B build selected the register-staged kernel)");
    const int N = SFG_N, d = SFG_D, L = max_level;
    if (L < 1 || L > ctx->nq) SFG_FAIL(ctx, "matmul_from_cache: max_level out of range");
    const int lev = in_level > max_level ? max_level : in_level, nl = lev + 1, nl_in = in_level + 1;
    if (nl < L) SFG_FAIL(ctx, "matmul_from_cache: input level %d has fewer than max_level = %d moduli", in_level, max_level);
    if (nbr < 1) SFG_FAIL(ctx, "matmul_from_cache: no block rows");
    std::vector<DiagCacheHdr> hdrs(nbr); std::vector<FILE *> files(nbr, nullptr);
    auto close_all = [&]() { for (FILE *f : files) if (f) fclose(f); };
    for (int bi = 0; bi < nbr; bi++) {
        if (dc_open(ctx, std::string(prefix) + "_" + std::to_string(bi) + ".bin", &files[bi], hdrs[bi])) { close_all(); return 1; }
        const DiagCacheHdr &h = hdrs[bi];
        long fsize = -1; { const long here = ftell(files[bi]); if (!fseek(files[bi], 0, SEEK_END)) fsize = ftell(files[bi]); fseek(files[bi], here, SEEK_SET); }
        if (h.n != (uint64_t)N || h.numModuli < (uint64_t)L || h.numModuli > (uint64_t)ctx->nmod || h.vectorLen != hdrs[0].vectorLen || h.vectorLen < 1 ||
            h.vectorLen > (1u << 20) || h.rowSize != 4 + (1 + h.n * h.numModuli * 8) * h.vectorLen || fsize < 0 || h.rowSize > (uint64_t)fsize) {
            close_all(); SFG_FAIL(ctx, "matmul_from_cache: %s_%d.bin does not match this ring (n = %llu, numModuli = %llu, vectorLen = %llu)", prefix, bi,
                                  (unsigned long long)h.n, (unsigned long long)h.numModuli, (unsigned long long)h.vectorLen);
        }
    }
    const int m_ct = (int)hdrs[0].vectorLen;
    std::vector<uint8_t> giant_t(d, 0);
    for (auto &h : hdrs) for (int g = 0; g < d; g++) giant_t[g] |= h.giant[g];
    const size_t accw = (size_t)s * 2 * L * N, ctw = (size_t)2 * nl * N, prow = (size_t)N / 2, plw = (size_t)L * prow;
    std::vector<int> plane_of, is_big; const int nplanes = mac_dma_planes(ctx, L, plane_of, is_big);
    if (nplanes < 0) { close_all(); return 1; }
    const size_t rowf = (size_t)nplanes * N;
    const unsigned packed_mask = mac_dma_packed_mask(ctx, L);
    int jp = (int)(ctx->cfg.acc_budget / ((size_t)d * accw * 8)); if (jp < 1) jp = 1; if (jp > m_ct) jp = m_ct;
    u64 *a_row = nullptr, *rotc = nullptr, *acc = nullptr, *panel = nullptr, *raw_d = nullptr, *inv_d = nullptr; double *rotf = nullptr, *rotsum = nullptr;
    uint8_t *present_d = nullptr; unsigned long long *asym_d = nullptr; u64 *raw_h = nullptr;
    int rc = 0;
    auto bail = [&](int r) { close_all(); if (raw_h) (void)hipHostFree(raw_h); return r; };
    if (sfg_scratch(ctx, "mm.a_row", (size_t)s * ctw * 8, (void **)&a_row) || sfg_scratch(ctx, "mm.rotc", 8, (void **)&rotc) ||
        sfg_scratch(ctx, "mm.rotf", ((size_t)d + 3) * s * 2 * rowf * 8, (void **)&rotf) || sfg_scratch(ctx, "mm.rotsum", (size_t)2 * s * 2 * rowf * 8, (void **)&rotsum) ||
        sfg_scratch(ctx, "mm.acc", (size_t)jp * d * accw * 8, (void **)&acc) || sfg_scratch(ctx, "dc.panel", (size_t)jp * d * plw * 8, (void **)&panel) ||
        sfg_scratch(ctx, "dc.raw", (size_t)d * jp * L * N * 8 + (size_t)d * jp + 64 + 8 * SFG_MAXMOD, (void **)&raw_d)) return bail(1);
    present_d = (uint8_t *)(raw_d + (size_t)d * jp * L * N);
    asym_d = (unsigned long long *)(present_d + (((size_t)d * jp + 63) & ~(size_t)63)); inv_d = (u64 *)(asym_d + 1);
    if (hipHostMalloc((void **)&raw_h, (size_t)d * jp * L * N * 8 + (size_t)d * jp, hipHostMallocDefault) != hipSuccess) { ctx->err = "matmul_from_cache: hipHostMalloc failed"; return bail(1); }
    uint8_t *present_h = (uint8_t *)(raw_h + (size_t)d * jp * L * N);
    {
        u64 inv[SFG_MAXMOD] = {0};
        for (int l = 0; l < L; l++) { const u64 q = ctx->q[l]; inv[l] = h_invmod((u64)((((u128)1) << 64) % q), q); }
        if (hipMemcpyAsync(inv_d, inv, sizeof inv, hipMemcpyHostToDevice, ctx->stream) != hipSuccess || hipMemsetAsync(asym_d, 0, 8, ctx->stream) != hipSuccess ||
            hipStreamSynchronize(ctx->stream) != hipSuccess) { ctx->err = "matmul_from_cache: setup copy failed"; return bail(1); }
    }
    std::vector<unsigned char> rec;
    for (int ja = 0; ja < m_ct && !rc; ja += jp) {
        const int jn = std::min(jp, m_ct - ja);
        if (hipMemsetAsync(acc, 0, (size_t)jn * d * accw * 8, ctx->stream) != hipSuccess) { ctx->err = "matmul_from_cache: memset failed"; rc = 1; break; }
        for (int bi = 0; bi < nbr && !rc; bi++) {
            const DiagCacheHdr &h = hdrs[bi]; FILE *f = files[bi];
            fseek(f, h.data_pos, SEEK_SET);
            try { rec.resize(h.rowSize); } catch (const std::exception &) { ctx->err = "matmul_from_cache: out of host memory for a record"; rc = 1; break; }
            rc = build_rot_row_tab(ctx, (const u64 *)A, s, nl_in, nl, lev, L, nbr, bi, h.baby, a_row, rotc, true, rotf);
            if (!rc && hipMemsetAsync(rotf + (size_t)d * s * 2 * rowf, 0, (size_t)3 * s * 2 * rowf * 8, ctx->stream) != hipSuccess) rc = 1;
            if (!rc && packed_mask) rc = launch_rot_sum(ctx, rotf, (size_t)s * 2, d, L, rotsum);
            int cur_giant = -1; bool any = false;
            auto flush = [&]() -> int {
                if (!any) return 0;
                SFG_HIP(ctx, hipMemcpyAsync(raw_d, raw_h, (size_t)d * jn * L * N * 8, hipMemcpyHostToDevice, ctx->stream));
                SFG_HIP(ctx, hipMemcpyAsync(present_d, present_h, (size_t)d * jn, hipMemcpyHostToDevice, ctx->stream));
                hipLaunchKernelGGL(k_cache_to_panel, dim3((unsigned)((size_t)d * jn * L * (N / 2 / 256))), dim3(256), 0, ctx->stream, raw_d, present_d, panel, jn, L, packed_mask,
                                   inv_d, ctx->modc, asym_d);
                SFG_HIP(ctx, hipGetLastError());
                MacStrides st;
                st.rot_k = (size_t)s * ctw; st.rot_r = (size_t)nl * N;
                st.pt_k = plw; st.pt_n = (size_t)d * plw; st.pt_half = true; st.pt_packed = packed_mask != 0; st.i8 = ctx->cfg.mac_i8 && packed_mask; st.i8_big = st.i8 && ctx->cfg.mac_i8_big;
                st.out_n = (size_t)d * accw; st.out_r = (size_t)L * N;
                PhaseTimer t(ctx, "mac");
                int r2 = launch_mac_dma(ctx, rotf, (size_t)s * 2, panel, acc + (size_t)cur_giant * accw, d, 2 * s, jn, L, 1, st, rotsum);
                t.stop(1);
                SFG_HIP(ctx, hipStreamSynchronize(ctx->stream));
                any = false;
                return r2;
            };
            while (!rc) {
                unsigned char l8[8];
                if (fread(l8, 1, 8, f) != 8) break;
                uint64_t len = 0; for (int i = 0; i < 8; i++) len |= (uint64_t)l8[i] << (8 * i);
                if (len > h.rowSize || len < 4 || fread(rec.data(), 1, len, f) != len) { ctx->err = "matmul_from_cache: truncated record"; rc = 1; break; }
                const int shift = (int)((uint32_t)rec[0] | (uint32_t)rec[1] << 8 | (uint32_t)rec[2] << 16 | (uint32_t)rec[3] << 24);
                if (shift < 0 || shift >= SFG_SLOTS) { ctx->err = "matmul_from_cache: shift out of range"; rc = 1; break; }
                const int giant = shift / d, baby = shift % d;
                if (giant != cur_giant) { rc = flush(); if (rc) break; cur_giant = giant; memset(present_h, 0, (size_t)d * jn); }
                size_t ptr = 4; const size_t plain_bytes = (size_t)h.n * h.numModuli * 8;
                for (uint64_t j = 0; j < h.vectorLen; j++) {
                    if (ptr >= len) { ctx->err = "matmul_from_cache: malformed record"; rc = 1; break; }
                    const bool empty = rec[ptr++] == 1;
                    if (empty) continue;
                    if (ptr + plain_bytes > len) { ctx->err = "matmul_from_cache: malformed record"; rc = 1; break; }
                    if ((int)j >= ja && (int)j < ja + jn) {
                        memcpy(raw_h + ((size_t)baby * jn + (j - ja)) * L * N, rec.data() + ptr, (size_t)L * N * 8);
                        present_h[(size_t)baby * jn + (j - ja)] = 1; any = true;
                    }
                    ptr += plain_bytes;
                }
            }
            if (!rc) rc = flush();
        }
        if (!rc) rc = matmul_finalize(ctx, acc, s, max_level, jn, m_ct, ja, 0, d, &giant_t, 0, (u64 *)out);
        if (!rc && hipStreamSynchronize(ctx->stream) != hipSuccess) rc = 1;
    }
    unsigned long long asym = 0;
    if (!rc && hipMemcpy(&asym, asym_d, 8, hipMemcpyDeviceToHost) != hipSuccess) rc = 1;
    if (!rc && asym) { ctx->err = "matmul_from_cache: cached plaintexts are not mirror-symmetric (not encodings of real slot vectors)"; rc = 1; }
    return bail(rc);
}
```

sfgwas_amd/csrc/ntt.hip:

```cpp
#include "common.hpp"
#include "kernels.hpp"
#include "i8_move.hpp"
#include "ntt_core.hpp"

template <int IN_MODE>
__global__ void __launch_bounds__(512) k_ntt_fwd(const void *in_, u64 *out_, ModPattern pat, RowMap rm, const double *tw_all, const double2 *pack_all, const ModConst *modc) {
    extern __shared__ double lds[];
    const int N = SFG_N, tid = threadIdx.x;
    const size_t row = blockIdx.x;
    const int m = pat.m[row % pat.period];
    const size_t grp = row / rm.rpg, gi = row % rm.rpg;
    if (m == -2) return;
    if (m < 0) {
        const u64 *src = (const u64 *)in_ + grp * rm.gstride_in + gi * N; u64 *dst = out_ + grp * rm.gstride_out + gi * N;
        if (IN_MODE == 0 && src != dst) for (int a = 0; a < 32; a++) dst[a * 512 + tid] = src[a * 512 + tid];
        return;
    }
    const double *tw = tw_all + (size_t)m * N;
    const double2 *pack = pack_all + (size_t)m * (N / 2);
    const double q = modc[m].q, qinv = modc[m].qinv;
    double v[32];
    if (IN_MODE == 0) {
        const u64 *in = (const u64 *)in_ + grp * rm.gstride_in + gi * N;
#pragma unroll
        for (int a = 0; a < 32; a++) v[a] = u64_to_f64(in[a * 512 + tid]);
    } else {
        const double *pc = (const double *)in_ + (row / pat.period) * (size_t)(N / 2);
#pragma unroll
        for (int a = 0; a < 16; a++) v[a] = pred(pc[a * 512 + tid], q, qinv);
#pragma unroll
        for (int a = 16; a < 32; a++) {
            int x = (a - 16) * 512 + tid;
            v[a] = x == 0 ? 0.0 : -pred(pc[N / 2 - x], q, qinv);
        }
    }
    ntt_fwd_phases(v, lds, tw, pack, q, qinv, tid);
    u64 *out = out_ + grp * rm.gstride_out + gi * N;
    {
        const int b = tid >> 4, c = tid & 15;
#pragma unroll
        for (int a = 0; a < 32; a++) out[a * 512 + tid] = f64_to_u64(canon(lds[a * LDS_ROW + c * 33 + b], q, qinv));
    }
}

__global__ void __launch_bounds__(512) k_ntt_inv(const u64 *in_, u64 *out_, ModPattern pat, RowMap rm, const double *tw_all, const double2 *pack_all, const ModConst *modc) {
    extern __shared__ double lds[];
    const int N = SFG_N, tid = threadIdx.x;
    const size_t row = blockIdx.x;
    const int m = pat.m[row % pat.period];
    if (m < 0) return;
    const size_t grp = row / rm.rpg, gi = row % rm.rpg;
    const double *tw = tw_all + (size_t)m * N;
    const double2 *pack = pack_all + (size_t)m * (N / 2);
    const double q = modc[m].q, qinv = modc[m].qinv;
    const u64 *in = in_ + grp * rm.gstride_in + gi * N;
    double v[32];
    {
        const int b = tid >> 4, c = tid & 15;
#pragma unroll
        for (int a = 0; a < 32; a++) lds[a * LDS_ROW + c * 33 + b] = u64_to_f64(in[a * 512 + tid]);
    }
    __syncthreads();
#pragma unroll
    for (int h = 0; h < 2; h++) {
        const int p = tid + 512 * h, a = p >> 5, b = p & 31;
        double w[16];
#pragma unroll
        for (int c = 0; c < 16; c++) w[c] = lds[a * LDS_ROW + c * 33 + b];
        double tl[16];
        {
            const double2 *pk = pack + (size_t)(p >> 6) * 512 + (p & 63);
#pragma unroll
            for (int i = 0; i < 8; i++) { const double2 e = pk[i * 64]; tl[2 * i] = e.x; tl[2 * i + 1] = e.y; }
        }
        gs_stage<16, 1>(w, q, qinv, [&](int g) { return tl[7 + g]; });
        gs_stage<16, 2>(w, q, qinv, [&](int g) { return tl[3 + g]; });
        gs_stage<16, 4>(w, q, qinv, [&](int g) { return tl[1 + g]; });
        gs_stage<16, 8>(w, q, qinv, [&](int g) { return tl[0 + g]; });
#pragma unroll
        for (int c = 0; c < 16; c++) v[h * 16 + c] = pred(w[c], q, qinv);
    }
    __syncthreads();
#pragma unroll
    for (int h = 0; h < 2; h++) {
        const int p = tid + 512 * h, a = p >> 5, b = p & 31;
#pragma unroll
        for (int c = 0; c < 16; c++) lds[a * LDS_ROW + c * 33 + b] = v[h * 16 + c];
    }
    __syncthreads();
    {
        const int a = tid >> 4, c = tid & 15;
#pragma unroll
        for (int b = 0; b < 32; b++) v[b] = lds[a * LDS_ROW + c * 33 + b];
        gs_stage<32, 1>(v, q, qinv, [&](int g) { return tw[512 + a * 16 + g]; });
        gs_stage<32, 2>(v, q, qinv, [&](int g) { return tw[256 + a * 8 + g]; });
        gs_stage<32, 4>(v, q, qinv, [&](int g) { return tw[128 + a * 4 + g]; });
        gs_stage<32, 8>(v, q, qinv, [&](int g) { return tw[64 + a * 2 + g]; });
        gs_stage<32, 16>(v, q, qinv, [&](int g) { return tw[32 + a + g]; });
        __syncthreads();
#pragma unroll
        for (int b = 0; b < 32; b++) lds[a * LDS_ROW + b * 16 + c] = pred(v[b], q, qinv);
    }
    __syncthreads();
#pragma unroll
    for (int a = 0; a < 32; a++) v[a] = lds[a * LDS_ROW + tid];
    gs_stage<32, 1>(v, q, qinv, [&](int g) { return tw[16 + g]; });
    gs_stage<32, 2>(v, q, qinv, [&](int g) { return tw[8 + g]; });
    gs_stage<32, 4>(v, q, qinv, [&](int g) { return tw[4 + g]; });
    gs_stage<32, 8>(v, q, qinv, [&](int g) { return tw[2 + g]; });
    gs_stage<32, 16>(v, q, qinv, [&](int g) { return tw[1 + g]; });
    const double ninv = modc[m].ninv, ninv_q = modc[m].ninv_q;
    u64 *out = out_ + grp * rm.gstride_out + gi * N;
#pragma unroll
    for (int a = 0; a < 32; a++) {
        double x = mulmod_lazy(pred(v[a], q, qinv), ninv, ninv_q, q);
        out[a * 512 + tid] = f64_to_u64(canon(x, q, qinv));
    }
}

constexpr int H3_ROWA = 264;
constexpr int H3_WREG = 4 * 272;
constexpr int H3_DOUBLES = 16 * H3_ROWA > 4 * H3_WREG ? 16 * H3_ROWA : 4 * H3_WREG;
constexpr int H3_LDS_BYTES = H3_DOUBLES * 8;
struct NoFill {};
template <class First, class Store, class Fill = NoFill, bool WIDE = false>
__device__ __forceinline__ void ntt_half3_body(int hs, First first, Store store, double *lds, const double *tw, const double2 *pack, double q, double qinv, int tid, Fill fill = Fill()) {
    double v[32];
    const int a_b = tid >> 4, c_b = tid & 15;
    double w2[2][16];
    if constexpr (std::is_same<Fill, NoFill>::value) {
#pragma unroll
        for (int h = 0; h < 2; h++)
#pragma unroll
            for (int a = 0; a < 16; a++) w2[h][a] = first(a * 512 + tid + 256 * h);
    } else fill(w2);
#pragma unroll
    for (int h = 0; h < 2; h++) {
        double (&w)[16] = w2[h];
        ct_stage<16, 8>(w, q, qinv, [&](int g) { return tw[2 + hs + g]; });
        ct_stage<16, 4>(w, q, qinv, [&](int g) { return tw[4 + 2 * hs + g]; });
        ct_stage<16, 2>(w, q, qinv, [&](int g) { return tw[8 + 4 * hs + g]; });
        ct_stage<16, 1>(w, q, qinv, [&](int g) { return tw[16 + 8 * hs + g]; });
        if (h) __syncthreads();
#pragma unroll
        for (int a = 0; a < 16; a++) lds[a * H3_ROWA + tid] = w[a];
        __syncthreads();
#pragma unroll
        for (int b = 0; b < 16; b++) v[h * 16 + b] = lds[a_b * H3_ROWA + b * 16 + c_b];
    }
    const int ab = 16 * hs + a_b;
    ct_stage<32, 16>(v, q, qinv, [&](int g) { return tw[32 + ab + g]; });
    ct_stage<32, 8>(v, q, qinv, [&](int g) { return tw[64 + ab * 2 + g]; });
    ct_stage<32, 4>(v, q, qinv, [&](int g) { return tw[128 + ab * 4 + g]; });
    ct_stage<32, 2>(v, q, qinv, [&](int g) { return tw[256 + ab * 8 + g]; });
    ct_stage<32, 1>(v, q, qinv, [&](int g) { return tw[512 + ab * 16 + g]; });
    __syncthreads();
    {
        const int wv = tid >> 6, lane = tid & 63, al = lane >> 4, bk = lane & 15;
        double *img = lds + wv * H3_WREG;
        auto sw = [](int idx) { return (idx >> 8) * 272 + ((idx >> 4) & 15) * 17 + (idx & 15); };
#pragma unroll
        for (int r = 0; r < 2; r++) {
            double wc[16];
            __builtin_amdgcn_fence(__ATOMIC_ACQ_REL, "wavefront");
#pragma unroll
            for (int k = 0; k < 16; k++) img[sw(al * 256 + c_b * 16 + k)] = v[16 * r + k];
            __builtin_amdgcn_fence(__ATOMIC_ACQ_REL, "wavefront");
#pragma unroll
            for (int c = 0; c < 16; c++) wc[c] = img[sw(al * 256 + c * 16 + bk)];
            const int p = a_b * 32 + 16 * r + bk;
            double tl[16];
            {
                const double2 *pk = pack + (size_t)((p >> 6) + 8 * hs) * 512 + (p & 63);
#pragma unroll
                for (int i = 0; i < 8; i++) {
                    const double2 e = pk[i * 64];
                    tl[2 * i] = e.x; tl[2 * i + 1] = e.y;
                }
            }
            ct_stage<16, 8>(wc, q, qinv, [&](int g) { return tl[0 + g]; });
            ct_stage<16, 4>(wc, q, qinv, [&](int g) { return tl[1 + g]; });
            ct_stage<16, 2>(wc, q, qinv, [&](int g) { return tl[3 + g]; });
            ct_stage<16, 1>(wc, q, qinv, [&](int g) { return tl[7 + g]; });
            __builtin_amdgcn_fence(__ATOMIC_ACQ_REL, "wavefront");
#pragma unroll
            for (int c = 0; c < 16; c++) img[sw(al * 256 + c * 16 + bk)] = wc[c];
            __builtin_amdgcn_fence(__ATOMIC_ACQ_REL, "wavefront");
#pragma unroll
            for (int ai = 0; ai < 4; ai++) {
                if constexpr (WIDE) {
                    const int x0 = 4 * lane;
                    const int base = ai * 256 + (lane >> 2);
                    store((4 * wv + ai) * 512 + 256 * r + x0, img[sw(base + (4 * (lane & 3) + 0) * 16)], img[sw(base + (4 * (lane & 3) + 1) * 16)],
                          img[sw(base + (4 * (lane & 3) + 2) * 16)], img[sw(base + (4 * (lane & 3) + 3) * 16)]);
                } else {
#pragma unroll
                    for (int qd = 0; qd < 4; qd++) {
                        const int x = qd * 64 + lane;
                        store((4 * wv + ai) * 512 + 256 * r + x, img[sw(ai * 256 + (x & 15) * 16 + (x >> 4))]);
                    }
                }
            }
        }
    }
}
#define NT_ST(p, v) __builtin_nontemporal_store((unsigned)(v), (p))
template <bool PERM, bool DIG>
__device__ __forceinline__ void ntt_half3_wg(size_t vb, double *lds, const double *pc_all, u64 *out_, size_t nplain, int L, PanelMap pm, const double *tw_all, const double2 *pack_all,
                                             const ModConst *modc, const uint32_t *perm) {
    const int N = SFG_N, n = N / 2, tid = threadIdx.x;
    size_t row; int m;
    if (!plain_block_of(vb, nplain, L, row, m)) return;
    const double *tw = tw_all + (size_t)m * N;
    const double2 *pack = pack_all + (size_t)m * (N / 2);
    const double q = modc[m].q, qinv = modc[m].qinv;
    const double *pc = pc_all + (row / L) * (size_t)n;
    unsigned gal = 1;
    if (PERM) { const uint32_t e = perm[pm.shift0 + (int)(row / L)]; pc = pc_all + (size_t)(e & 0xFFFFu) * n; gal = e >> 16; }
    const double W = tw[1], Wq = W * qinv;
    auto first = [&](int j) { const double lo = pc[j], hi = j == 0 ? 0.0 : pc[n - j]; return lo - mulmod_lazy(hi, W, Wq, q); };
    auto fill = [&](double (&w2)[2][16]) {
        double rA[16], rB[16];
#pragma unroll
        for (int k = 0; k < 16; k++) {
            const int i = tid + 256 * k;
            const double lo = pc[i], hi = i == 0 ? 0.0 : pc[n - i];
            const unsigned qd = (((unsigned)i * gal) & (2u * N - 1u)) >> 13;
            const double ca = (qd == 1u || qd == 2u) ? -lo : lo, cb = qd >= 2u ? -hi : hi;
            rA[k] = ca - mulmod_lazy(cb, W, Wq, q);
            rB[k] = cb - mulmod_lazy(ca, W, Wq, q);
        }
#pragma unroll
        for (int h = 0; h < 2; h++) {
#pragma unroll
            for (int k = 0; k < 16; k++) {
                const unsigned raw = ((unsigned)(tid + 256 * k) * gal) & (2u * N - 1u), qd = raw >> 13;
                const int J = qd == 0u ? (int)raw : qd == 1u ? N - (int)raw : qd == 2u ? (int)raw - N : 2 * N - (int)raw, Jb = n - J;
                if (((J >> 8) & 1) == h && J < n) lds[(J >> 9) * H3_ROWA + (J & 255)] = rA[k];
                if (((Jb >> 8) & 1) == h && Jb < n) lds[(Jb >> 9) * H3_ROWA + (Jb & 255)] = rB[k];
            }
            __syncthreads();
#pragma unroll
            for (int a = 0; a < 16; a++) w2[h][a] = lds[a * H3_ROWA + tid];
            __syncthreads();
        }
        if (tid == 0) {
            const double mid = pc[n / 2];
            const double c = ((((unsigned)(n / 2) * gal) & (2u * N - 1u)) >> 13) >= 2u ? -mid : mid;
            w2[0][8] = c - mulmod_lazy(c, W, Wq, q);
        }
    };
    const size_t plain = row / L; const int shift = pm.shift0 + (int)plain;
    const size_t dst = pm.G ? ((size_t)(shift / SFG_D) * pm.G + pm.g) * SFG_D + (size_t)(shift % SFG_D) : plain;
    u64 *out = out_ + (dst * L + m) * (size_t)n;
    size_t dstride = n, cbm = 0;
    if constexpr (DIG) if (pm.packed_mask & PT_COMPACT) {
        const unsigned lm = (1u << L) - 1u, small = pm.packed_mask & lm;
        const int ns_all = __popc(small), ns_below = __popc(small & ((1u << m) - 1u));
        const size_t planes_all = (size_t)ns_all * 5 + (size_t)(L - ns_all) * 6, planes_below = (size_t)ns_below * 5 + (size_t)(m - ns_below) * 6;
        if (pm.packed_mask & PT_KMAJOR) {
            const size_t K = (size_t)pm.K, col = pm.G ? (size_t)(shift / SFG_D) : plain / K, row = pm.G ? (size_t)pm.g * SFG_D + (size_t)(shift % SFG_D) : plain % K;
            out = reinterpret_cast<u64 *>(reinterpret_cast<uint8_t *>(out_) + ((col * planes_all + planes_below) * 64 * K + row) * 128);
            dstride = 64 * K * 128; cbm = K * 128 - 128;
        } else out = reinterpret_cast<u64 *>(reinterpret_cast<uint8_t *>(out_) + dst * (planes_all * n) + planes_below * n);
    }
    if constexpr (DIG) if (!((pm.packed_mask >> m) & 1u) && (pm.packed_mask & PT_DIGITS_BIG)) {
        uint8_t *o8 = reinterpret_cast<uint8_t *>(out);
        auto dig6 = [&](double x, unsigned &lo, unsigned &hi) {
            const u64 b = (u64)__double_as_longlong(canon(x, q, qinv) + (4503599627370496.0 + 141289400074368.0));
            lo = (unsigned)b ^ 0x80808080u; hi = (unsigned)(b >> 32) ^ 0x8080u;
        };
        auto st6 = [&](int j0, double x0, double x1, double x2, double x3) {
            unsigned l0, l1, l2, l3, h0, h1, h2, h3;
            dig6(x0, l0, h0); dig6(x1, l1, h1); dig6(x2, l2, h2); dig6(x3, l3, h3);
            unsigned o[4]; bytes_tr4(l0, l1, l2, l3, o);
            uint8_t *ob = o8 + j0 + (size_t)(j0 >> 7) * cbm;
#pragma unroll
            for (int d = 0; d < 4; d++) NT_ST(reinterpret_cast<unsigned *>(ob + d * dstride), o[d]);
            unsigned p[4]; bytes_tr4(h0, h1, h2, h3, p);
            NT_ST(reinterpret_cast<unsigned *>(ob + 4 * dstride), p[0]);
            NT_ST(reinterpret_cast<unsigned *>(ob + 5 * dstride), p[1]);
        };
        if constexpr (PERM) ntt_half3_body<decltype(first), decltype(st6), decltype(fill), true>(0, first, st6, lds, tw, pack, q, qinv, tid, fill);
        else ntt_half3_body<decltype(first), decltype(st6), NoFill, true>(0, first, st6, lds, tw, pack, q, qinv, tid);
        return;
    }
    if constexpr (DIG) if ((pm.packed_mask >> m) & 1u) {
        uint8_t *o8 = reinterpret_cast<uint8_t *>(out);
        auto dig = [&](double x, unsigned &lo, unsigned &hi) {
            const u64 b = (u64)__double_as_longlong(canon_le(x, q, qinv) + (4503599627370496.0 + 551911719040.0));
            lo = (unsigned)b ^ 0x80808080u; hi = (unsigned)(b >> 32) ^ 0x80u;
        };
        auto st8 = [&](int j0, double x0, double x1, double x2, double x3) {
            unsigned l0, l1, l2, l3, h0, h1, h2, h3;
            dig(x0, l0, h0); dig(x1, l1, h1); dig(x2, l2, h2); dig(x3, l3, h3);
            unsigned o[4]; bytes_tr4(l0, l1, l2, l3, o);
            uint8_t *ob = o8 + j0 + (size_t)(j0 >> 7) * cbm;
#pragma unroll
            for (int d = 0; d < 4; d++) NT_ST(reinterpret_cast<unsigned *>(ob + d * dstride), o[d]);
            NT_ST(reinterpret_cast<unsigned *>(ob + 4 * dstride), (h0 & 255u) | ((h1 & 255u) << 8) | ((h2 & 255u) << 16) | (h3 << 24));
        };
        if constexpr (PERM) ntt_half3_body<decltype(first), decltype(st8), decltype(fill), true>(0, first, st8, lds, tw, pack, q, qinv, tid, fill);
        else ntt_half3_body<decltype(first), decltype(st8), NoFill, true>(0, first, st8, lds, tw, pack, q, qinv, tid);
        return;
    }
    if constexpr (PERM) {
        if (!DIG && ((pm.packed_mask >> m) & 1u)) ntt_half3_body(0, first, [&](int j, double x) { out[j] = pack_limbs_f64(canon_le(x, q, qinv)); }, lds, tw, pack, q, qinv, tid, fill);
        else ntt_half3_body(0, first, [&](int j, double x) { out[j] = f64_to_u64(canon(x, q, qinv)); }, lds, tw, pack, q, qinv, tid, fill);
    } else {
        (void)fill;
        if (!DIG && ((pm.packed_mask >> m) & 1u)) ntt_half3_body(0, first, [&](int j, double x) { out[j] = pack_limbs_f64(canon_le(x, q, qinv)); }, lds, tw, pack, q, qinv, tid);
        else ntt_half3_body(0, first, [&](int j, double x) { out[j] = f64_to_u64(canon(x, q, qinv)); }, lds, tw, pack, q, qinv, tid);
    }
}
template <bool PERM, bool DIG>
__global__ void __launch_bounds__(256, 4) k_ntt_half3(const double *pc_all, u64 *out_, size_t nplain, int L, PanelMap pm, const double *tw_all, const double2 *pack_all, const ModConst *modc,
                                                      const uint32_t *perm) {
    extern __shared__ double lds[];
    ntt_half3_wg<PERM, DIG>(blockIdx.x, lds, pc_all, out_, nplain, L, pm, tw_all, pack_all, modc, perm);
}
template <bool PERM, int DEPTH, bool NT>
__global__ void __launch_bounds__(256, 4) k_ntt_half3_move(const double *pc_all, u64 *out_, size_t nplain, int L, PanelMap pm, const double *tw_all, const double2 *pack_all, const ModConst *modc,
                                                           const uint32_t *perm, MoveJob job) {
    extern __shared__ double lds[];
    if (blockIdx.x < job.nblocks) { i8_move_block<DEPTH, NT>(job, blockIdx.x, reinterpret_cast<unsigned *>(lds), (int)threadIdx.x); return; }
    ntt_half3_wg<PERM, true>((size_t)blockIdx.x - job.nblocks, lds, pc_all, out_, nplain, L, pm, tw_all, pack_all, modc, perm);
}
__global__ void __launch_bounds__(256, 4) k_ntt_fwd_split(const u64 *in_, u64 *out_, size_t nrows, ModPattern pat, RowMap rm, const double *tw_all, const double2 *pack_all, const ModConst *modc) {
    extern __shared__ double lds[];
    const int N = SFG_N, n = N / 2, tid = threadIdx.x;
    const size_t b = blockIdx.x, row = (b / 16) * 8 + b % 8; const int hs = (int)((b / 8) & 1);
    if (row >= nrows) return;
    const int m = pat.m[row % pat.period];
    const size_t grp = row / rm.rpg, gi = row % rm.rpg;
    const u64 *in = in_ + grp * rm.gstride_in + gi * N;
    u64 *out = out_ + grp * rm.gstride_out + gi * N + (size_t)hs * n;
    if (m == -2) return;
    if (m < 0) {
        for (int k = 0; k < 32; k++) out[k * 256 + tid] = in[(size_t)hs * n + k * 256 + tid];
        return;
    }
    const double *tw = tw_all + (size_t)m * N;
    const double2 *pack = pack_all + (size_t)m * (N / 2);
    const double q = modc[m].q, qinv = modc[m].qinv;
    const double W = hs ? -tw[1] : tw[1], Wq = W * qinv;
    auto first = [&](int j) { return u64_to_f64(in[j]) + mulmod_lazy(u64_to_f64(in[n + j]), W, Wq, q); };
    ntt_half3_body(hs, first, [&](int j, double x) { out[j] = f64_to_u64(canon(x, q, qinv)); }, lds, tw, pack, q, qinv, tid);
}
__global__ void __launch_bounds__(256) k_expand_half(const u64 *half, u64 *full) {
    const int N = SFG_N, n = N / 2; const size_t row = blockIdx.x / (n / 256);
    const int i = (int)(blockIdx.x % (n / 256)) * 256 + threadIdx.x;
    const u64 v = half[row * n + i];
    full[row * N + i] = v; full[row * N + (N - 1 - i)] = v;
}

int ntt_set_attrs(sfg_ctx *ctx) {
    hipError_t e = hipFuncSetAttribute((const void *)k_ntt_fwd<0>, hipFuncAttributeMaxDynamicSharedMemorySize, LDS_DOUBLES * 8);
    if (e == hipSuccess) e = hipFuncSetAttribute((const void *)k_ntt_fwd<1>, hipFuncAttributeMaxDynamicSharedMemorySize, LDS_DOUBLES * 8);
    if (e == hipSuccess) e = hipFuncSetAttribute((const void *)k_ntt_inv, hipFuncAttributeMaxDynamicSharedMemorySize, LDS_DOUBLES * 8);
    if (e == hipSuccess) e = hipFuncSetAttribute((const void *)k_ntt_half3<false, false>, hipFuncAttributeMaxDynamicSharedMemorySize, H3_LDS_BYTES);
    if (e == hipSuccess) e = hipFuncSetAttribute((const void *)k_ntt_half3<true, false>, hipFuncAttributeMaxDynamicSharedMemorySize, H3_LDS_BYTES);
    if (e == hipSuccess) e = hipFuncSetAttribute((const void *)k_ntt_half3<false, true>, hipFuncAttributeMaxDynamicSharedMemorySize, H3_LDS_BYTES);
    if (e == hipSuccess) e = hipFuncSetAttribute((const void *)k_ntt_half3<true, true>, hipFuncAttributeMaxDynamicSharedMemorySize, H3_LDS_BYTES);
    if (e == hipSuccess) e = hipFuncSetAttribute((const void *)k_ntt_fwd_split, hipFuncAttributeMaxDynamicSharedMemorySize, H3_LDS_BYTES);
#define SFG_MV_ATTR(P, D, T) if (e == hipSuccess) e = hipFuncSetAttribute((const void *)k_ntt_half3_move<P, D, T>, hipFuncAttributeMaxDynamicSharedMemorySize, H3_LDS_BYTES)
    SFG_MV_ATTR(false, 1, true); SFG_MV_ATTR(true, 1, true);
#ifdef SFG_AB
    SFG_MV_ATTR(false, 1, false); SFG_MV_ATTR(false, 2, false); SFG_MV_ATTR(false, 2, true); SFG_MV_ATTR(false, 3, false); SFG_MV_ATTR(false, 3, true);
    SFG_MV_ATTR(true, 1, false); SFG_MV_ATTR(true, 2, false); SFG_MV_ATTR(true, 2, true); SFG_MV_ATTR(true, 3, false); SFG_MV_ATTR(true, 3, true);
    if (e == hipSuccess && ab_set_attrs(ctx)) return 1;
#endif
#undef SFG_MV_ATTR
    if (e != hipSuccess) SFG_FAIL(ctx, "cannot raise dynamic LDS limit for the NTT kernels");
    return 0;
}

static RowMap dense_map() { RowMap rm; rm.rpg = 1; rm.gstride_in = SFG_N; rm.gstride_out = SFG_N; return rm; }
int launch_ntt_fwd(sfg_ctx *ctx, const u64 *in, u64 *out, size_t nrows, const ModPattern &pat) { return launch_ntt_fwd_map(ctx, in, out, nrows, pat, dense_map()); }
int launch_ntt_inv(sfg_ctx *ctx, const u64 *in, u64 *out, size_t nrows, const ModPattern &pat) { return launch_ntt_inv_map(ctx, in, out, nrows, pat, dense_map()); }
int launch_ntt_fwd_map(sfg_ctx *ctx, const u64 *in, u64 *out, size_t nrows, const ModPattern &pat, const RowMap &rm) {
    if (!nrows) return 0;
    if (in != out && !ctx->cfg.ntt_fwd_full)
        hipLaunchKernelGGL(k_ntt_fwd_split, dim3((unsigned)((nrows + 7) / 8 * 16)), dim3(256), H3_LDS_BYTES, ctx->stream, in, out, nrows, pat, rm, ctx->tw_fwd, ctx->pack_fwd, ctx->modc);
    else
        hipLaunchKernelGGL(k_ntt_fwd<0>, dim3((unsigned)nrows), dim3(512), LDS_DOUBLES * 8, ctx->stream, (const void *)in, out, pat, rm, ctx->tw_fwd, ctx->pack_fwd, ctx->modc);
    SFG_HIP(ctx, hipGetLastError());
    return 0;
}
int launch_ntt_plain(sfg_ctx *ctx, const double *pc, u64 *out, size_t nplain, int L) {
    if (!nplain) return 0;
    ModPattern pat; pat.period = L; for (int l = 0; l < L; l++) pat.m[l] = (int8_t)l;
    hipLaunchKernelGGL(k_ntt_fwd<1>, dim3((unsigned)(nplain * L)), dim3(512), LDS_DOUBLES * 8, ctx->stream, (const void *)pc, out, pat, dense_map(), ctx->tw_fwd, ctx->pack_fwd, ctx->modc);
    SFG_HIP(ctx, hipGetLastError());
    return 0;
}
template <bool PERM>
static int launch_half3_move(sfg_ctx *ctx, dim3 grid, const double *pc, u64 *out_half, size_t nplain, int L, PanelMap pm, const uint32_t *perm, const MoveJob &j) {
#define SFG_MV(D, T) hipLaunchKernelGGL((k_ntt_half3_move<PERM, D, T>), grid, dim3(256), H3_LDS_BYTES, ctx->stream, pc, out_half, nplain, L, pm, ctx->tw_fwd, ctx->pack_fwd, ctx->modc, perm, j)
    if (j.depth == 1 && j.nt) { SFG_MV(1, true); return 0; }
#ifdef SFG_AB
    if (j.depth == 3) { if (j.nt) SFG_MV(3, true); else SFG_MV(3, false); return 0; }
    if (j.depth == 2) { if (j.nt) SFG_MV(2, true); else SFG_MV(2, false); return 0; }
    if (j.depth == 1) { SFG_MV(1, false); return 0; }
#endif
#undef SFG_MV
    SFG_FAIL(ctx, "plaintext NTT: the product build holds the mover with one unit in flight and streaming accesses only (other forms: make ab)");
}
int launch_ntt_plain_half(sfg_ctx *ctx, const double *pc, u64 *out_half, size_t nplain, int L, PanelMap pm, const uint32_t *perm, const MoveJob *mv) {
    if (!nplain) return 0;
    const dim3 grid((unsigned)((nplain + 7) / 8 * 8 * L));
    const bool dig = pm.packed_mask & PT_DIGITS;
    if (mv && mv->count) {
        if (!dig || mv->nblocks % 8 || !mv->nblocks) SFG_FAIL(ctx, "plaintext NTT: mover workgroups need the digit-plane form and a multiple of 8 of them");
        const dim3 g2(grid.x + mv->nblocks);
        if (perm) SFG_TRY(launch_half3_move<true>(ctx, g2, pc, out_half, nplain, L, pm, perm, *mv));
        else SFG_TRY(launch_half3_move<false>(ctx, g2, pc, out_half, nplain, L, pm, (const uint32_t *)nullptr, *mv));
        SFG_HIP(ctx, hipGetLastError());
        return 0;
    }
    if (perm && dig) hipLaunchKernelGGL((k_ntt_half3<true, true>), grid, dim3(256), H3_LDS_BYTES, ctx->stream, pc, out_half, nplain, L, pm, ctx->tw_fwd, ctx->pack_fwd, ctx->modc, perm);
    else if (perm) hipLaunchKernelGGL((k_ntt_half3<true, false>), grid, dim3(256), H3_LDS_BYTES, ctx->stream, pc, out_half, nplain, L, pm, ctx->tw_fwd, ctx->pack_fwd, ctx->modc, perm);
    else if (dig) hipLaunchKernelGGL((k_ntt_half3<false, true>), grid, dim3(256), H3_LDS_BYTES, ctx->stream, pc, out_half, nplain, L, pm, ctx->tw_fwd, ctx->pack_fwd, ctx->modc, (const uint32_t *)nullptr);
#ifdef SFG_AB
    else if (ctx->cfg.ntt_half_full) ab_launch_ntt_half_full(ctx, pc, out_half, nplain, L, pm);
#endif
    else hipLaunchKernelGGL((k_ntt_half3<false, false>), grid, dim3(256), H3_LDS_BYTES, ctx->stream, pc, out_half, nplain, L, pm, ctx->tw_fwd, ctx->pack_fwd, ctx->modc, (const uint32_t *)nullptr);
    SFG_HIP(ctx, hipGetLastError());
    return 0;
}
int launch_expand_half(sfg_ctx *ctx, const u64 *half, u64 *full, size_t nrows) {
    if (!nrows) return 0;
    hipLaunchKernelGGL(k_expand_half, dim3((unsigned)(nrows * (SFG_N / 2 / 256))), dim3(256), 0, ctx->stream, half, full);
    SFG_HIP(ctx, hipGetLastError());
    return 0;
}
int launch_ntt_inv_map(sfg_ctx *ctx, const u64 *in, u64 *out, size_t nrows, const ModPattern &pat, const RowMap &rm) {
    if (!nrows) return 0;
    hipLaunchKernelGGL(k_ntt_inv, dim3((unsigned)nrows), dim3(512), LDS_DOUBLES * 8, ctx->stream, in, out, pat, rm, ctx->tw_inv, ctx->pack_inv, ctx->modc);
    SFG_HIP(ctx, hipGetLastError());
    return 0;
}

static int pattern_from_host(sfg_ctx *ctx, const int *mod_idx, int nrows, ModPattern &pat) {
    for (int period = 1; period <= 64 && period <= nrows; period++) {
        bool ok = true;
        for (int r = 0; r < nrows && ok; r++) ok = mod_idx[r] == mod_idx[r % period];
        if (ok) { pat.period = period; for (int i = 0; i < period; i++) { if (mod_idx[i] < 0 || mod_idx[i] >= ctx->nmod) SFG_FAIL(ctx, "modulus index out of range"); pat.m[i] = (int8_t)mod_idx[i]; } return 0; }
    }
    SFG_FAIL(ctx, "mod_idx must be periodic with period <= 64");
}

extern "C" int sfg_ntt_rows(sfg_ctx *ctx, uint64_t *rows, int nrows, const int *mod_idx) {
    SFG_HIP(ctx, hipSetDevice(ctx->device));
    ModPattern pat; SFG_TRY(pattern_from_host(ctx, mod_idx, nrows, pat));
    return launch_ntt_fwd(ctx, (const u64 *)rows, (u64 *)rows, nrows, pat);
}
extern "C" int sfg_intt_rows(sfg_ctx *ctx, uint64_t *rows, int nrows, const int *mod_idx) {
    SFG_HIP(ctx, hipSetDevice(ctx->device));
    ModPattern pat; SFG_TRY(pattern_from_host(ctx, mod_idx, nrows, pat));
    return launch_ntt_inv(ctx, (const u64 *)rows, (u64 *)rows, nrows, pat);
}
```

sfgwas_amd/csrc/rotate.hip:

```cpp
#include "common.hpp"
#include "kernels.hpp"
#include "ksw.hpp"


static void fill_ext(const sfg_ctx *ctx, ExtConst &e, const std::vector<int> &src) {
    memset(&e, 0, sizeof e);
    e.a = (int)src.size();
    for (int m = 0; m < e.a; m++) e.src[m] = src[m];
    for (int m = 0; m < e.a; m++) {
        u64 qm = ctx->q[src[m]], h = 1;
        for (int k = 0; k < e.a; k++) if (k != m) h = h_mulmod(h, ctx->q[src[k]] % qm, qm);
        u64 hi = h_invmod(h, qm);
        e.qhat_inv[m] = (double)hi; e.qhat_inv_q[m] = (double)hi / (double)qm;
    }
    for (int t = 0; t < ctx->nmod; t++) {
        u64 qt = ctx->q[t], D = 1 % qt;
        for (int m = 0; m < e.a; m++) {
            u64 ht = 1 % qt;
            for (int k = 0; k < e.a; k++) if (k != m) ht = h_mulmod(ht, ctx->q[src[k]] % qt, qt);
            e.qhat_t[t][m] = (double)ht; e.qhat_t_q[t][m] = (double)ht / (double)qt;
            D = h_mulmod(D, ctx->q[src[m]] % qt, qt);
        }
        e.D_t[t] = (double)D; e.D_t_q[t] = (double)D / (double)qt;
    }
}


int get_ksw(sfg_ctx *ctx, int level, KswConst **dev, KswConst *host) {
    KswConst kc; memset(&kc, 0, sizeof kc);
    kc.level = level; kc.nl = level + 1; kc.np = ctx->np; kc.alpha = ctx->np; kc.nt = kc.nl + kc.np;
    kc.beta = (kc.nl + kc.alpha - 1) / kc.alpha;
    if (kc.alpha > KSW_MAXA || kc.beta > KSW_MAXDIG) SFG_FAIL(ctx, "key-switch shape unsupported (alpha > 4 or beta > 8)");
    if (kc.beta * kc.nt > SFG_MAXPATTERN) SFG_FAIL(ctx, "key-switch shape unsupported (beta * (level + 1 + np) = %d rows exceed the modulus pattern table)", kc.beta * kc.nt);
    for (int t = 0; t < kc.nt; t++) { kc.tmod[t] = t < kc.nl ? t : ctx->nq + (t - kc.nl); kc.digit_of[t] = t < kc.nl ? t / kc.alpha : -1; }
    for (int i = 0; i < kc.beta; i++) {
        std::vector<int> src;
        for (int m = i * kc.alpha; m < (i + 1) * kc.alpha && m < kc.nl; m++) src.push_back(m);
        fill_ext(ctx, kc.dig[i], src);
    }
    std::vector<int> ps; for (int p = 0; p < kc.np; p++) ps.push_back(ctx->nq + p);
    fill_ext(ctx, kc.pq, ps);
    for (int t = 0; t < kc.nl; t++) {
        u64 qt = ctx->q[t], P = 1;
        for (int p = 0; p < kc.np; p++) P = h_mulmod(P, ctx->q[ctx->nq + p] % qt, qt);
        u64 pi = h_invmod(P, qt);
        kc.pinv[t] = (double)pi; kc.pinv_q[t] = (double)pi / (double)qt;
    }
    *host = kc;
    auto it = ctx->ksw_cache.find(level);
    if (it == ctx->ksw_cache.end()) {
        KswConst *d = nullptr;
        SFG_HIP(ctx, hipMalloc(&d, sizeof(KswConst)));
        SFG_HIP(ctx, hipMemcpy(d, &kc, sizeof(KswConst), hipMemcpyHostToDevice));
        ctx->ksw_cache[level] = d; *dev = d;
    } else *dev = (KswConst *)it->second;
    return 0;
}


__global__ void __launch_bounds__(256) k_ksw_extend(const u64 *c2, const u64 *ct_in, u64 *ext, const KswConst *kcp, const ModConst *modc) {
    const KswConst &kc = *kcp;
    const int N = SFG_N, x = blockIdx.x * 256 + threadIdx.x, i = blockIdx.y; const size_t b = blockIdx.z;
    const ExtConst &e = kc.dig[i];
    const u64 *c2b = c2 + b * (size_t)kc.nl * N;
    u64 *eb = ext + (b * kc.beta + i) * (size_t)kc.nt * N;
    double xs[KSW_MAXA], y[KSW_MAXA], v = 0.0;
#pragma unroll
    for (int m = 0; m < KSW_MAXA; m++) xs[m] = m < e.a ? u64_to_f64(c2b[(size_t)e.src[m] * N + x]) : 0.0;
    if (e.a > 1) ext_prepare(e, modc, xs, y, v);
    for (int t = 0; t < kc.nt; t++) {
        const int tg = kc.tmod[t];
        u64 outv;
        if (kc.digit_of[t] == i) continue;
        else if (e.a == 1) outv = f64_to_u64(canon(xs[0], modc[tg].q, modc[tg].qinv));
        else outv = f64_to_u64(ext_target(e, tg, modc[tg].q, modc[tg].qinv, y, v));
        eb[(size_t)t * N + x] = outv;
    }
}

__global__ void __launch_bounds__(256) k_ksw_inner(const u64 *ext, const u64 *ct_in, const u64 *const *keys, const int *inidx, u64 *acc, const KswConst *kcp, const ModConst *modc, int nmod) {
    const KswConst &kc = *kcp;
    const int N = SFG_N, x = 2 * (blockIdx.x * 256 + threadIdx.x), t = blockIdx.y; const size_t b = blockIdx.z;
    const int tg = kc.tmod[t];
    const double q = modc[tg].q, qinv = modc[tg].qinv;
    const u64 *key = keys[b];
    const size_t bi = (size_t)inidx[b];
    double a0x = 0.0, a0y = 0.0, a1x = 0.0, a1y = 0.0;
    for (int i = 0; i < kc.beta; i++) {
        const ulonglong2 ev = kc.digit_of[t] == i ? *reinterpret_cast<const ulonglong2 *>(ct_in + (bi * 2 * (size_t)kc.nl + kc.nl + t) * N + x)
                                                  : *reinterpret_cast<const ulonglong2 *>(ext + ((bi * kc.beta + i) * (size_t)kc.nt + t) * N + x);
        const ulonglong2 k0 = *reinterpret_cast<const ulonglong2 *>(key + (((size_t)i * 2 + 0) * nmod + tg) * N + x);
        const ulonglong2 k1 = *reinterpret_cast<const ulonglong2 *>(key + (((size_t)i * 2 + 1) * nmod + tg) * N + x);
        const double ex = u64_to_f64(ev.x), ey = u64_to_f64(ev.y);
        a0x += mulmod2(ex, u64_to_f64(k0.x), q, qinv); a0y += mulmod2(ey, u64_to_f64(k0.y), q, qinv);
        a1x += mulmod2(ex, u64_to_f64(k1.x), q, qinv); a1y += mulmod2(ey, u64_to_f64(k1.y), q, qinv);
    }
    *reinterpret_cast<ulonglong2 *>(acc + ((b * 2 + 0) * (size_t)kc.nt + t) * N + x) = make_ulonglong2(f64_to_u64(canon(a0x, q, qinv)), f64_to_u64(canon(a0y, q, qinv)));
    *reinterpret_cast<ulonglong2 *>(acc + ((b * 2 + 1) * (size_t)kc.nt + t) * N + x) = make_ulonglong2(f64_to_u64(canon(a1x, q, qinv)), f64_to_u64(canon(a1y, q, qinv)));
}

__global__ void __launch_bounds__(256) k_moddown_extend(const u64 *acc, u64 *ext2, const KswConst *kcp, const ModConst *modc) {
    const KswConst &kc = *kcp;
    const int N = SFG_N, x = blockIdx.x * 256 + threadIdx.x, p = blockIdx.y; const size_t b = blockIdx.z;
    const ExtConst &e = kc.pq;
    const u64 *ap = acc + ((b * 2 + p) * (size_t)kc.nt + kc.nl) * N;
    double xs[KSW_MAXA], y[KSW_MAXA], v = 0.0;
#pragma unroll
    for (int m = 0; m < KSW_MAXA; m++) xs[m] = m < e.a ? u64_to_f64(ap[(size_t)m * N + x]) : 0.0;
    if (e.a > 1) ext_prepare(e, modc, xs, y, v);
    for (int t = 0; t < kc.nl; t++) {
        u64 outv = e.a == 1 ? f64_to_u64(canon(xs[0], modc[t].q, modc[t].qinv)) : f64_to_u64(ext_target(e, t, modc[t].q, modc[t].qinv, y, v));
        ext2[((b * 2 + p) * (size_t)kc.nl + t) * N + x] = outv;
    }
}

struct F64Form { int on, L, centre; size_t rowf; int plane_of[SFG_MAXMOD], big[SFG_MAXMOD]; };
__device__ __forceinline__ void store_rot_f64(double *row, const F64Form &ff, int t, int x, double v, double q) {
    const int N = SFG_N;
    double *o = row + (size_t)ff.plane_of[t] * N;
    if (ff.big[t]) {
        const double wc = v > __builtin_floor(q * 0.5) ? v - q : v;
        const double hi = __builtin_floor((wc + 4194304.0) * 0x1p-23), lo = wc - hi * 8388608.0;
        o[2 * x] = lo; o[2 * x + 1] = hi;
    } else o[x] = (ff.centre && v > __builtin_floor(q * 0.5)) ? v - q : v;
}
__global__ void __launch_bounds__(256) k_ksw_finish(const u64 *ct_in, const int *inidx, const u64 *acc, const u64 *ext2, const uint16_t *const *index,
                                                   u64 *const *ct_out, const KswConst *kcp, const ModConst *modc, const u64 *add1, F64Form ff) {
    const KswConst &kc = *kcp;
    const int N = SFG_N, x = blockIdx.x * 256 + threadIdx.x, t = blockIdx.y; const size_t b = blockIdx.z;
    if (ff.on && t >= ff.L) return;
    const double q = modc[t].q, qinv = modc[t].qinv, pinv = kc.pinv[t], pinv_q = kc.pinv_q[t];
    const int src = index[b][x];
#pragma unroll
    for (int p = 0; p < 2; p++) {
        const double a = u64_to_f64(acc[((b * 2 + p) * (size_t)kc.nt + t) * N + src]);
        const double e = u64_to_f64(ext2[((b * 2 + p) * (size_t)kc.nl + t) * N + src]);
        double r = mulmod_lazy(a - e, pinv, pinv_q, q);
        if (p == 0) r += u64_to_f64(ct_in[((size_t)inidx[b] * 2 * (size_t)kc.nl + t) * N + src]);
        else if (add1) r += u64_to_f64(add1[((size_t)inidx[b] * (size_t)kc.nl + t) * N + src]);
        const double v = canon(r, q, qinv);
        if (ff.on) store_rot_f64(reinterpret_cast<double *>(ct_out[b]) + (size_t)p * ff.rowf, ff, t, x, v, q);
        else ct_out[b][((size_t)p * kc.nl + t) * N + x] = f64_to_u64(v);
    }
}

__global__ void __launch_bounds__(256) k_ct_add(const u64 *a, const u64 *b, u64 *out, int nl, const ModConst *modc, size_t total_rows) {
    const int N = SFG_N; const size_t row = blockIdx.x / (N / 256); const int m = (int)(row % nl);
    const u64 q = modc[m].qi;
    const size_t off = row * N + (blockIdx.x % (N / 256)) * 256 + threadIdx.x;
    u64 v = a[off] + b[off]; out[off] = v >= q ? v - q : v;
}

static int launch_keyswitch_jobs(sfg_ctx *ctx, const u64 *in, int nin, int level, const std::vector<int> &job_in, const std::vector<const u64 *> &keyp,
                                 const std::vector<const uint16_t *> &idxp, const std::vector<u64 *> &outp, const u64 *add1, const F64Form *ffp = nullptr) {
    const int N = SFG_N, nl = level + 1;
    F64Form ff; memset(&ff, 0, sizeof ff); if (ffp) ff = *ffp;
    KswConst *kcd; KswConst kc;
    SFG_TRY(get_ksw(ctx, level, &kcd, &kc));
    const size_t ctw = (size_t)2 * nl * N;
    const int nr = (int)job_in.size();
    if (!nr) return 0;
    const size_t in_rows = (size_t)nl + (size_t)kc.beta * kc.nt, job_rows = 2 * (size_t)kc.nt + 2 * (size_t)nl;
    const size_t budget = ctx->cfg.ksw_budget;
    int in_grp = (int)(budget / (in_rows * N * 8)); if (in_grp < 1) in_grp = 1; if (in_grp > nin) in_grp = nin;
    int chunk = (int)(budget / (job_rows * N * 8)); if (chunk < 1) chunk = 1; if (chunk > nr) chunk = nr;
    const size_t ptr_bytes = (size_t)nr * (3 * sizeof(void *) + sizeof(int)) + 256;
    const size_t ext_rows = (size_t)in_grp * kc.beta * kc.nt, ext2_rows = (size_t)chunk * 2 * nl;
    SFG_TRY(sfg_ws_reserve(ctx, (in_rows * in_grp + job_rows * chunk + ext_rows + ext2_rows) * N * 8 + ptr_bytes));
    u64 *c2 = (u64 *)ctx->ws, *ext = c2 + (size_t)in_grp * nl * N;
    u64 *acc = ext + ext_rows * N, *ext2 = acc + (size_t)chunk * 2 * kc.nt * N;
    u64 *extT = ext2 + ext2_rows * N, *ext2T = extT + ext_rows * N;
    const u64 **keys_all = (const u64 **)(ext2T + ext2_rows * N);
    const uint16_t **idx_all = (const uint16_t **)(keys_all + nr);
    u64 **out_all = (u64 **)(idx_all + nr);
    int *inidx_all = (int *)(out_all + nr);
    ModPattern pq; pq.period = nl; for (int m = 0; m < nl; m++) pq.m[m] = (int8_t)m;
    ModPattern pext; pext.period = kc.beta * kc.nt;
    for (int i = 0; i < kc.beta; i++) for (int t = 0; t < kc.nt; t++) pext.m[i * kc.nt + t] = kc.digit_of[t] == i ? (int8_t)-2 : (int8_t)kc.tmod[t];
    ModPattern pp; pp.period = kc.np; for (int p = 0; p < kc.np; p++) pp.m[p] = (int8_t)(ctx->nq + p);
    for (int i0 = 0; i0 < nin; i0 += in_grp) {
        const int ni = nin - i0 < in_grp ? nin - i0 : in_grp;
        std::vector<int> jobs;
        for (int k = 0; k < nr; k++) if (job_in[k] >= i0 && job_in[k] < i0 + ni) jobs.push_back(k);
        if (jobs.empty()) continue;
        const u64 *bin = in + (size_t)i0 * ctw;
        RowMap rm1; rm1.rpg = nl; rm1.gstride_in = ctw; rm1.gstride_out = (size_t)nl * N;
        SFG_TRY(launch_ntt_inv_map(ctx, bin + (size_t)nl * N, c2, (size_t)ni * nl, pq, rm1));
        hipLaunchKernelGGL(k_ksw_extend, dim3(N / 256, kc.beta, ni), dim3(256), 0, ctx->stream, c2, bin, ext, kcd, ctx->modc);
        SFG_HIP(ctx, hipGetLastError());
        SFG_TRY(launch_ntt_fwd(ctx, ext, extT, (size_t)ni * kc.beta * kc.nt, pext));
        {
            const size_t nj = jobs.size();
            std::vector<const u64 *> kp(nj); std::vector<const uint16_t *> ip(nj); std::vector<u64 *> op(nj); std::vector<int> ii(nj);
            for (size_t k = 0; k < nj; k++) { int jb = jobs[k]; kp[k] = keyp[jb]; ip[k] = idxp[jb]; op[k] = outp[jb]; ii[k] = job_in[jb] - i0; }
            SFG_TRY(sfg_upload_small(ctx, keys_all, kp.data(), nj * sizeof(void *)));
            SFG_TRY(sfg_upload_small(ctx, idx_all, ip.data(), nj * sizeof(void *)));
            SFG_TRY(sfg_upload_small(ctx, out_all, op.data(), nj * sizeof(void *)));
            SFG_TRY(sfg_upload_small(ctx, inidx_all, ii.data(), nj * sizeof(int)));
        }
        for (size_t c0 = 0; c0 < jobs.size(); c0 += chunk) {
            const int nb = (int)(jobs.size() - c0 < (size_t)chunk ? jobs.size() - c0 : (size_t)chunk);
            const u64 **keys_d = keys_all + c0; const uint16_t **idx_d = idx_all + c0; u64 **out_d = out_all + c0; int *inidx_d = inidx_all + c0;
            hipLaunchKernelGGL(k_ksw_inner, dim3(N / 512, kc.nt, nb), dim3(256), 0, ctx->stream, extT, bin, keys_d, inidx_d, acc, kcd, ctx->modc, ctx->nmod);
            SFG_HIP(ctx, hipGetLastError());
            RowMap rm4; rm4.rpg = kc.np; rm4.gstride_in = (size_t)kc.nt * N; rm4.gstride_out = (size_t)kc.nt * N;
            SFG_TRY(launch_ntt_inv_map(ctx, acc + (size_t)nl * N, acc + (size_t)nl * N, (size_t)nb * 2 * kc.np, pp, rm4));
            hipLaunchKernelGGL(k_moddown_extend, dim3(N / 256, 2, nb), dim3(256), 0, ctx->stream, acc, ext2, kcd, ctx->modc);
            SFG_HIP(ctx, hipGetLastError());
            SFG_TRY(launch_ntt_fwd(ctx, ext2, ext2T, (size_t)nb * 2 * nl, pq));
            hipLaunchKernelGGL(k_ksw_finish, dim3(N / 256, nl, nb), dim3(256), 0, ctx->stream, bin, inidx_d, acc, ext2T, idx_d, out_d, kcd, ctx->modc,
                               add1 ? add1 + (size_t)i0 * nl * N : nullptr, ff);
            SFG_HIP(ctx, hipGetLastError());
        }
    }
    return 0;
}
int launch_rotate_right_indexed(sfg_ctx *ctx, const u64 *in, int nin, u64 *out, int nct, int level, const int *nrot_host, const int *in_index) {
    const int N = SFG_N, nl = level + 1;
    if (level < 0 || level >= ctx->nq) SFG_FAIL(ctx, "rotate: level out of range");
    const size_t ctw = (size_t)2 * nl * N;
    std::vector<int> job_in; std::vector<const u64 *> keyp; std::vector<const uint16_t *> idxp; std::vector<u64 *> outp;
    for (int j = 0; j < nct; j++) {
        int nrot = nrot_host[j] % SFG_SLOTS; if (nrot < 0) nrot += SFG_SLOTS;
        const int src = in_index ? in_index[j] : j;
        if (src < 0 || src >= nin) SFG_FAIL(ctx, "rotate: input index out of range");
        if (nrot == 0) {
            int run = 1;
            while (j + run < nct && (nrot_host[j + run] % SFG_SLOTS) == 0 && (in_index ? in_index[j + run] : j + run) == src + run && src + run < nin) run++;
            SFG_HIP(ctx, hipMemcpyAsync(out + j * ctw, in + (size_t)src * ctw, (size_t)run * ctw * 8, hipMemcpyDeviceToDevice, ctx->stream));
            j += run - 1;
            continue;
        }
        u64 g = sfg_galois_for_rotation(ctx, SFG_SLOTS - nrot);
        auto it = ctx->rotkeys().find(g);
        if (it == ctx->rotkeys().end()) SFG_FAIL(ctx, "rotate: no rotation key loaded for right-rotation by %d (galois element %llu)", nrot, g);
        job_in.push_back(src); keyp.push_back(it->second.key_dev); idxp.push_back(it->second.index_dev); outp.push_back(out + j * ctw);
    }
    return launch_keyswitch_jobs(ctx, in, nin, level, job_in, keyp, idxp, outp, nullptr);
}
int launch_rotate_right_indexed_f64(sfg_ctx *ctx, const u64 *in, int nin, double *outf, int nct, int level, const int *nrot_host, const int *in_index, int L,
                                    const size_t *out_slot) {
    const int N = SFG_N, nl = level + 1;
    ctx->i8_gen++;
    if (level < 0 || level >= ctx->nq || L > nl) SFG_FAIL(ctx, "rotate: level out of range");
    const size_t ctw = (size_t)2 * nl * N;
    std::vector<int> plane_of, is_big; const int nplanes = mac_dma_planes(ctx, L, plane_of, is_big);
    if (nplanes < 0) return 1;
    F64Form ff; memset(&ff, 0, sizeof ff);
    ff.on = 1; ff.L = L; ff.centre = mac_dma_packed_mask(ctx, L) != 0; ff.rowf = (size_t)nplanes * N;
    for (int l = 0; l < L; l++) { ff.plane_of[l] = plane_of[l]; ff.big[l] = is_big[l]; }
    std::vector<int> job_in; std::vector<const u64 *> keyp; std::vector<const uint16_t *> idxp; std::vector<u64 *> outp;
    for (int j = 0; j < nct; j++) {
        int nrot = nrot_host[j] % SFG_SLOTS; if (nrot < 0) nrot += SFG_SLOTS;
        const int src = in_index ? in_index[j] : j;
        if (src < 0 || src >= nin) SFG_FAIL(ctx, "rotate: input index out of range");
        double *dst = outf + (out_slot ? out_slot[j] : (size_t)j) * 2 * ff.rowf;
        if (nrot == 0) {
            int run = 1;
            while (!out_slot && j + run < nct && (nrot_host[j + run] % SFG_SLOTS) == 0 && (in_index ? in_index[j + run] : j + run) == src + run && src + run < nin) run++;
            SFG_TRY(launch_rot_to_f64(ctx, in + (size_t)src * ctw, (size_t)2 * run, nl, L, dst));
            j += run - 1;
            continue;
        }
        u64 g = sfg_galois_for_rotation(ctx, SFG_SLOTS - nrot);
        auto it = ctx->rotkeys().find(g);
        if (it == ctx->rotkeys().end()) SFG_FAIL(ctx, "rotate: no rotation key loaded for right-rotation by %d (galois element %llu)", nrot, g);
        job_in.push_back(src); keyp.push_back(it->second.key_dev); idxp.push_back(it->second.index_dev); outp.push_back(reinterpret_cast<u64 *>(dst));
    }
    return launch_keyswitch_jobs(ctx, in, nin, level, job_in, keyp, idxp, outp, nullptr, &ff);
}
int launch_relinearize(sfg_ctx *ctx, const u64 *tmp, int nct, int level, const u64 *mid, u64 *out) {
    auto it = ctx->rotkeys().find(1);
    if (it == ctx->rotkeys().end()) SFG_FAIL(ctx, "relinearize: no relinearisation key loaded");
    const size_t ctw = (size_t)2 * (level + 1) * SFG_N;
    std::vector<int> job_in(nct); std::vector<const u64 *> keyp(nct, it->second.key_dev); std::vector<const uint16_t *> idxp(nct, it->second.index_dev); std::vector<u64 *> outp(nct);
    for (int j = 0; j < nct; j++) { job_in[j] = j; outp[j] = out + (size_t)j * ctw; }
    return launch_keyswitch_jobs(ctx, tmp, nct, level, job_in, keyp, idxp, outp, mid);
}
int launch_rotate_right(sfg_ctx *ctx, const u64 *in, u64 *out, int nct, int level, const int *nrot_host) {
    return launch_rotate_right_indexed(ctx, in, nct, out, nct, level, nrot_host, nullptr);
}

extern "C" int sfg_rotate_right_dev(sfg_ctx *ctx, const uint64_t *in, uint64_t *out, int nct, int level, const int *nrot_host) {
    SFG_HIP(ctx, hipSetDevice(ctx->device));
    if (in == out) SFG_FAIL(ctx, "rotate: in and out must not alias");
    PhaseTimer t(ctx, "rotate");
    int rc = launch_rotate_right(ctx, (const u64 *)in, (u64 *)out, nct, level, nrot_host);
    t.stop(1);
    return rc;
}

extern "C" int sfg_ct_galois_dev(sfg_ctx *ctx, const uint64_t *in, uint64_t *out, int nct, int level, uint64_t galois_el) {
    SFG_HIP(ctx, hipSetDevice(ctx->device));
    if (in == out) SFG_FAIL(ctx, "galois: in and out must not alias");
    if (level < 0 || level >= ctx->nq) SFG_FAIL(ctx, "galois: level out of range");
    auto it = ctx->rotkeys().find(galois_el);
    if (it == ctx->rotkeys().end() || galois_el == 1) SFG_FAIL(ctx, "galois: no switching key loaded for galois element %llu", (unsigned long long)galois_el);
    const size_t ctw = (size_t)2 * (level + 1) * SFG_N;
    std::vector<int> job_in(nct); std::vector<const u64 *> keyp(nct, it->second.key_dev); std::vector<const uint16_t *> idxp(nct, it->second.index_dev); std::vector<u64 *> outp(nct);
    for (int j = 0; j < nct; j++) { job_in[j] = j; outp[j] = (u64 *)out + (size_t)j * ctw; }
    PhaseTimer t(ctx, "rotate");
    int rc = launch_keyswitch_jobs(ctx, (const u64 *)in, nct, level, job_in, keyp, idxp, outp, nullptr);
    t.stop(1);
    return rc;
}

int launch_ct_add(sfg_ctx *ctx, const u64 *a, const u64 *b, u64 *out, size_t nct, int level) {
    const int nl = level + 1; const size_t rows = nct * 2 * nl;
    if (!rows) return 0;
    hipLaunchKernelGGL(k_ct_add, dim3((unsigned)(rows * (SFG_N / 256))), dim3(256), 0, ctx->stream, a, b, out, nl, ctx->modc, rows);
    SFG_HIP(ctx, hipGetLastError());
    return 0;
}
extern "C" int sfg_ct_add_dev(sfg_ctx *ctx, const uint64_t *a, const uint64_t *b, uint64_t *out, int nct, int level) {
    SFG_HIP(ctx, hipSetDevice(ctx->device));
    if (level < 0 || level >= ctx->nq) SFG_FAIL(ctx, "evaluator op: level %d out of range", level);
    if (nct < 0) SFG_FAIL(ctx, "evaluator op: negative ciphertext count");
    return launch_ct_add(ctx, (const u64 *)a, (const u64 *)b, (u64 *)out, (size_t)nct, level);
}
```

Measured before the change: 6201 billion.

## Fuse giant-step rotation sum into key switch and pre-apply NTT stage one

Giant-step rotations are no longer written to a scratch buffer and summed by a separate kernel. A new rotate-and-sum path writes each group's sum directly in the key-switch finish kernel. The extend and mod-down kernels now compute the first forward NTT butterfly stage themselves, and a staged NTT variant skips that stage. Only the output moduli are processed, and per-ciphertext operand copies become one gather kernel. These changes cut memory traffic and launch count in exchange for more complex segment bookkeeping and host uploads.

Measured after the change: 6343 billion (median of 6 runs). 1.02x the previous value.

```diff
diff --git a/sfgwas_amd/csrc/common.hpp b/sfgwas_amd/csrc/common.hpp
--- a/sfgwas_amd/csrc/common.hpp
+++ b/sfgwas_amd/csrc/common.hpp
@@ -9,6 +9,7 @@
 #include <set>
 #include <unistd.h>
 #include "../../include/sfgwas_hip.h"
+#include "fp64mod.hpp"
 #include "consts.hpp"
 
 typedef unsigned long long u64;
@@ -228,32 +229,6 @@
 __device__ __host__ __forceinline__ u64 pack_limbs(u64 w) {
     return (w & 0xFFF) | (((w >> 12) & 0xFFF) << 16) | ((w >> 24) << 32);
 }
-
-__device__ __forceinline__ double mulmod_lazy(double x, double w, double wq, double q) {
-    double qh = __builtin_rint(x * wq);
-    double h = x * w;
-    double l = __builtin_fma(x, w, -h);
-    double r = __builtin_fma(-qh, q, h);
-    return r + l;
-}
-__device__ __forceinline__ double mulmod_lazy_q(double x, double w, double q, double qinv) {
-    double h = x * w;
-    double qh = __builtin_rint(h * qinv);
-    double l = __builtin_fma(x, w, -h);
-    double r = __builtin_fma(-qh, q, h);
-    return r + l;
-}
-__device__ __forceinline__ double canon(double x, double q, double qinv) {
-    const double r = __builtin_fma(-__builtin_floor(x * qinv), q, x);
-    return r == q ? 0.0 : r;
-}
-__device__ __forceinline__ double canon_le(double x, double q, double qinv) {
-    return __builtin_fma(-__builtin_floor(x * qinv), q, x);
-}
-__device__ __forceinline__ double pred(double x, double q, double qinv) {
-    double qh = __builtin_rint(x * qinv);
-    return __builtin_fma(-qh, q, x);
-}
 __device__ __forceinline__ double u64_to_f64(u64 x) {
     return __longlong_as_double((long long)(x | 0x4330000000000000ULL)) - 4503599627370496.0;
 }
diff --git a/sfgwas_amd/csrc/fp64mod.hpp b/sfgwas_amd/csrc/fp64mod.hpp
--- /dev/null
+++ b/sfgwas_amd/csrc/fp64mod.hpp
@@ -0,0 +1,38 @@
+#pragma once
+
+#if defined(__HIPCC__) || defined(__CUDACC__)
+#define SFG_HD __host__ __device__ __forceinline__
+#else
+#define SFG_HD inline
+#endif
+
+SFG_HD double mulmod_lazy(double x, double w, double wq, double q) {
+    double qh = __builtin_rint(x * wq);
+    double h = x * w;
+    double l = __builtin_fma(x, w, -h);
+    double r = __builtin_fma(-qh, q, h);
+    return r + l;
+}
+SFG_HD double mulmod_lazy_q(double x, double w, double q, double qinv) {
+    double h = x * w;
+    double qh = __builtin_rint(h * qinv);
+    double l = __builtin_fma(x, w, -h);
+    double r = __builtin_fma(-qh, q, h);
+    return r + l;
+}
+SFG_HD double canon(double x, double q, double qinv) {
+    const double r = __builtin_fma(-__builtin_floor(x * qinv), q, x);
+    return r == q ? 0.0 : r;
+}
+SFG_HD double canon_le(double x, double q, double qinv) {
+    return __builtin_fma(-__builtin_floor(x * qinv), q, x);
+}
+SFG_HD double pred(double x, double q, double qinv) {
+    double qh = __builtin_rint(x * qinv);
+    return __builtin_fma(-qh, q, x);
+}
+
+SFG_HD void fwd_stage1_pair(double v0, double v1, double W, double Wq, double q, double qinv, double &r0, double &r1) {
+    const double p = mulmod_lazy(v1, W, Wq, q);
+    r0 = canon(v0 + p, q, qinv); r1 = canon(v0 - p, q, qinv);
+}
diff --git a/sfgwas_amd/csrc/kernels.hpp b/sfgwas_amd/csrc/kernels.hpp
--- a/sfgwas_amd/csrc/kernels.hpp
+++ b/sfgwas_amd/csrc/kernels.hpp
@@ -17,6 +17,7 @@
 int launch_expand_half(sfg_ctx *ctx, const u64 *half, u64 *full, size_t nrows);
 int launch_ntt_fwd_map(sfg_ctx *ctx, const u64 *in, u64 *out, size_t nrows, const ModPattern &pat, const RowMap &rm);
 int launch_ntt_inv_map(sfg_ctx *ctx, const u64 *in, u64 *out, size_t nrows, const ModPattern &pat, const RowMap &rm);
+int launch_ntt_fwd_staged(sfg_ctx *ctx, const u64 *in, u64 *out, size_t nrows, const ModPattern &pat, bool staged);
 struct MacStrides { size_t rot_k, rot_r, pt_k, pt_n, out_n, out_r; bool pt_half = false; bool pt_packed = false; bool pt_digits = false; bool i8 = false; bool i8_big = false; bool pt_digits_big = false;
                     const int8_t *B_small = nullptr, *B_big = nullptr;
                     int pt_layout = 0, pt_L = 0;
@@ -45,6 +46,8 @@
 int launch_rotate_right_indexed(sfg_ctx *ctx, const u64 *in, int nin, u64 *out, int nct, int level, const int *nrot_host, const int *in_index);
 int launch_rotate_right_indexed_f64(sfg_ctx *ctx, const u64 *in, int nin, double *outf, int nct, int level, const int *nrot_host, const int *in_index, int L,
                                     const size_t *out_slot = nullptr);
+int launch_rotate_right_sum(sfg_ctx *ctx, const u64 *in, int nin, int nct, int level, const int *nrot_host, const int *in_index, const int *group, int nout,
+                            u64 *out, size_t out_stride, int accumulate);
 int launch_relinearize(sfg_ctx *ctx, const u64 *tmp, int nct, int level, const u64 *mid, u64 *out);
 int launch_ct_add(sfg_ctx *ctx, const u64 *a, const u64 *b, u64 *out, size_t nct, int level);
 int mac_dma_planes(sfg_ctx *ctx, int L, std::vector<int> &plane_of, std::vector<int> &is_big);
diff --git a/sfgwas_amd/csrc/matmul.hip b/sfgwas_amd/csrc/matmul.hip
--- a/sfgwas_amd/csrc/matmul.hip
+++ b/sfgwas_amd/csrc/matmul.hip
@@ -32,18 +32,17 @@
     const size_t x = (blockIdx.x % (N / 256)) * 256 + threadIdx.x;
     out[row * N + x] = in[(ctp * nl_in + m) * N + x];
 }
-__global__ void __launch_bounds__(256) k_sum_giants(const u64 *rot, int ngiant, int s, int L, u64 *out, size_t out_i_stride,
-                                                    int accumulate, const ModConst *modc) {
-    const int N = SFG_N; const size_t row = blockIdx.x / (N / 256);
-    const int i = (int)(row / (2 * L)), pl = (int)(row % (2 * L)), l = pl % L;
-    const size_t x = (blockIdx.x % (N / 256)) * 256 + threadIdx.x;
-    const double q = modc[l].q, qinv = modc[l].qinv;
-    double acc = accumulate ? u64_to_f64(out[(size_t)i * out_i_stride + (size_t)pl * N + x]) : 0.0;
-    for (int g = 0; g < ngiant; g++) {
-        acc += u64_to_f64(rot[(((size_t)g * s + i) * 2 * L + pl) * N + x]);
-        if ((g & 31) == 31) acc = pred(acc, q, qinv);
-    }
-    out[(size_t)i * out_i_stride + (size_t)pl * N + x] = f64_to_u64(canon(acc, q, qinv));
+__global__ void __launch_bounds__(256) k_gather_operands(const u64 *A, u64 *out, int nbr, int s, int job0, int nl_in, int nl) {
+    const int N = SFG_N; const size_t row = blockIdx.x / (N / 512);
+    const size_t k = row / (2 * (size_t)nl), p = (row / nl) & 1, m = row % nl, job = (size_t)job0 + k, bi = job / s, i = job % s;
+    const size_t x = 2 * ((blockIdx.x % (N / 512)) * 256 + threadIdx.x);
+    *reinterpret_cast<ulonglong2 *>(out + row * N + x) = *reinterpret_cast<const ulonglong2 *>(A + (((i * nbr + bi) * 2 + p) * nl_in + m) * N + x);
+}
+static int launch_gather_operands(sfg_ctx *ctx, const u64 *A, u64 *out, int nbr, int s, int job0, int njobs, int nl_in, int nl) {
+    if (njobs < 1) return 0;
+    hipLaunchKernelGGL(k_gather_operands, dim3((unsigned)((size_t)njobs * 2 * nl * (SFG_N / 512))), dim3(256), 0, ctx->stream, A, out, nbr, s, job0, nl_in, nl);
+    SFG_HIP(ctx, hipGetLastError());
+    return 0;
 }
 __global__ void __launch_bounds__(256) k_reduce_rows(u64 *rows, int L, const ModConst *modc) {
     const int N = SFG_N; const size_t row = blockIdx.x / (N / 256); const int l = (int)(row % L);
@@ -326,13 +325,8 @@
 }
 static int build_rot_row_tab(sfg_ctx *ctx, const u64 *A, int s, int nl_in, int nl, int lev, int L, int nbr, int bi, const std::vector<uint8_t> &baby_t,
                              u64 *a_row, u64 *rotc, bool dma, double *rotf_dst) {
-    const int N = SFG_N, d = SFG_D; const size_t ctw = (size_t)2 * nl * N;
-    for (int i = 0; i < s; i++) {
-        const u64 *src = A + ((size_t)i * nbr + bi) * 2 * nl_in * N;
-        if (nl == nl_in) SFG_HIP(ctx, hipMemcpyAsync(a_row + (size_t)i * ctw, src, ctw * 8, hipMemcpyDeviceToDevice, ctx->stream));
-        else hipLaunchKernelGGL(k_drop_level, dim3((unsigned)(2 * nl * (N / 256))), dim3(256), 0, ctx->stream, src, a_row + (size_t)i * ctw, nl_in, nl);
-    }
-    SFG_HIP(ctx, hipGetLastError());
+    const int d = SFG_D;
+    SFG_TRY(launch_gather_operands(ctx, A, a_row, nbr, s, bi * s, s, nl_in, nl));
     {
         PhaseTimer t(ctx, "rotate");
         std::vector<int> nrv((size_t)d * s, 0), inv((size_t)d * s, 0);
@@ -562,26 +556,18 @@
     const int N = SFG_N, d = SFG_D, L = max_level;
     const size_t accw = (size_t)s * 2 * L * N, ctw = (size_t)2 * L * N;
     if (g0 < 0 || g1 > acc_giants || g0 > g1 || giant_base < 0) SFG_FAIL(ctx, "finalize: giant range out of bounds");
-    u64 *rot = nullptr;
-    SFG_TRY(sfg_scratch(ctx, "mm.fin_rot", (size_t)d * accw * 8, (void **)&rot));
     std::vector<int> glist;
     for (int g = g0; g < g1; g++) if (giant_base + g < d && (!giant_active || (*giant_active)[giant_base + g])) glist.push_back(g);
     const int ng = (int)glist.size();
-    std::vector<int> nrv((size_t)ng * s), inv((size_t)ng * s);
-    for (int k = 0; k < ng; k++) for (int i = 0; i < s; i++) { nrv[(size_t)k * s + i] = -(giant_base + glist[k]) * d; inv[(size_t)k * s + i] = glist[k] * s + i; }
+    std::vector<int> nrv((size_t)ng * s), inv((size_t)ng * s), grp((size_t)ng * s);
+    for (int k = 0; k < ng; k++) for (int i = 0; i < s; i++) { nrv[(size_t)k * s + i] = -(giant_base + glist[k]) * d; inv[(size_t)k * s + i] = glist[k] * s + i; grp[(size_t)k * s + i] = i; }
     int rc = 0;
     for (int jb = 0; jb < ncolb && !rc; jb++) {
         const u64 *accj = acc + (size_t)jb * acc_giants * accw;
         u64 *o = out + (size_t)(jout0 + jb) * ctw;
-        if (ng) {
-            PhaseTimer t(ctx, "rotate");
-            rc = launch_rotate_right_indexed(ctx, accj, acc_giants * s, rot, ng * s, L - 1, nrv.data(), inv.data());
-            t.stop(1);
-            if (rc) break;
-        }
-        hipLaunchKernelGGL(k_sum_giants, dim3((unsigned)((size_t)s * 2 * L * (N / 256))), dim3(256), 0, ctx->stream, rot, ng, s, L,
-                           o, (size_t)m_ct_out * ctw, accumulate, ctx->modc);
-        if (hipGetLastError() != hipSuccess) { rc = 1; ctx->err = "finalize: k_sum_giants launch failed"; }
+        PhaseTimer t(ctx, "rotate");
+        rc = launch_rotate_right_sum(ctx, accj, acc_giants * s, ng * s, L - 1, nrv.data(), inv.data(), grp.data(), s, o, (size_t)m_ct_out * ctw, accumulate);
+        t.stop(1);
     }
     return rc;
 }
@@ -724,13 +710,7 @@
     PhaseTimer t(ctx, "rotate");
     for (int c0 = job0; c0 < job1; c0 += CH) {
         const int nj = std::min(CH, job1 - c0);
-        for (int k = 0; k < nj; k++) {
-            const int job = c0 + k, bi = job / s, i = job % s;
-            const u64 *src = (const u64 *)A + ((size_t)i * nbr + bi) * 2 * nl_in * N;
-            if (nl == nl_in) SFG_HIP(ctx, hipMemcpyAsync(a_in + (size_t)k * ctw, src, ctw * 8, hipMemcpyDeviceToDevice, ctx->stream));
-            else hipLaunchKernelGGL(k_drop_level, dim3((unsigned)(2 * nl * (N / 256))), dim3(256), 0, ctx->stream, src, a_in + (size_t)k * ctw, nl_in, nl);
-        }
-        SFG_HIP(ctx, hipGetLastError());
+        SFG_TRY(launch_gather_operands(ctx, (const u64 *)A, a_in, nbr, s, c0, nj, nl_in, nl));
         std::vector<int> nrv((size_t)d * nj), inv((size_t)d * nj); std::vector<size_t> slot((size_t)d * nj);
         for (int baby = 0; baby < d; baby++) for (int k = 0; k < nj; k++) {
             nrv[(size_t)baby * nj + k] = -baby; inv[(size_t)baby * nj + k] = k; slot[(size_t)baby * nj + k] = (size_t)(c0 - job0 + k) * d + baby;
diff --git a/sfgwas_amd/csrc/ntt.hip b/sfgwas_amd/csrc/ntt.hip
--- a/sfgwas_amd/csrc/ntt.hip
+++ b/sfgwas_amd/csrc/ntt.hip
@@ -326,6 +326,7 @@
     if (blockIdx.x < job.nblocks) { i8_move_block<DEPTH, NT>(job, blockIdx.x, reinterpret_cast<unsigned *>(lds), (int)threadIdx.x); return; }
     ntt_half3_wg<PERM, true>((size_t)blockIdx.x - job.nblocks, lds, pc_all, out_, nplain, L, pm, tw_all, pack_all, modc, perm);
 }
+template <bool STAGED>
 __global__ void __launch_bounds__(256, 4) k_ntt_fwd_split(const u64 *in_, u64 *out_, size_t nrows, ModPattern pat, RowMap rm, const double *tw_all, const double2 *pack_all, const ModConst *modc) {
     extern __shared__ double lds[];
     const int N = SFG_N, n = N / 2, tid = threadIdx.x;
@@ -344,7 +345,7 @@
     const double2 *pack = pack_all + (size_t)m * (N / 2);
     const double q = modc[m].q, qinv = modc[m].qinv;
     const double W = hs ? -tw[1] : tw[1], Wq = W * qinv;
-    auto first = [&](int j) { return u64_to_f64(in[j]) + mulmod_lazy(u64_to_f64(in[n + j]), W, Wq, q); };
+    auto first = [&](int j) { return STAGED ? u64_to_f64(in[(size_t)hs * n + j]) : u64_to_f64(in[j]) + mulmod_lazy(u64_to_f64(in[n + j]), W, Wq, q); };
     ntt_half3_body(hs, first, [&](int j, double x) { out[j] = f64_to_u64(canon(x, q, qinv)); }, lds, tw, pack, q, qinv, tid);
 }
 __global__ void __launch_bounds__(256) k_expand_half(const u64 *half, u64 *full) {
@@ -362,7 +363,8 @@
     if (e == hipSuccess) e = hipFuncSetAttribute((const void *)k_ntt_half3<true, false>, hipFuncAttributeMaxDynamicSharedMemorySize, H3_LDS_BYTES);
     if (e == hipSuccess) e = hipFuncSetAttribute((const void *)k_ntt_half3<false, true>, hipFuncAttributeMaxDynamicSharedMemorySize, H3_LDS_BYTES);
     if (e == hipSuccess) e = hipFuncSetAttribute((const void *)k_ntt_half3<true, true>, hipFuncAttributeMaxDynamicSharedMemorySize, H3_LDS_BYTES);
-    if (e == hipSuccess) e = hipFuncSetAttribute((const void *)k_ntt_fwd_split, hipFuncAttributeMaxDynamicSharedMemorySize, H3_LDS_BYTES);
+    if (e == hipSuccess) e = hipFuncSetAttribute((const void *)k_ntt_fwd_split<false>, hipFuncAttributeMaxDynamicSharedMemorySize, H3_LDS_BYTES);
+    if (e == hipSuccess) e = hipFuncSetAttribute((const void *)k_ntt_fwd_split<true>, hipFuncAttributeMaxDynamicSharedMemorySize, H3_LDS_BYTES);
 #define SFG_MV_ATTR(P, D, T) if (e == hipSuccess) e = hipFuncSetAttribute((const void *)k_ntt_half3_move<P, D, T>, hipFuncAttributeMaxDynamicSharedMemorySize, H3_LDS_BYTES)
     SFG_MV_ATTR(false, 1, true); SFG_MV_ATTR(true, 1, true);
 #ifdef SFG_AB
@@ -381,9 +383,17 @@
 int launch_ntt_fwd_map(sfg_ctx *ctx, const u64 *in, u64 *out, size_t nrows, const ModPattern &pat, const RowMap &rm) {
     if (!nrows) return 0;
     if (in != out && !ctx->cfg.ntt_fwd_full)
-        hipLaunchKernelGGL(k_ntt_fwd_split, dim3((unsigned)((nrows + 7) / 8 * 16)), dim3(256), H3_LDS_BYTES, ctx->stream, in, out, nrows, pat, rm, ctx->tw_fwd, ctx->pack_fwd, ctx->modc);
+        hipLaunchKernelGGL(k_ntt_fwd_split<false>, dim3((unsigned)((nrows + 7) / 8 * 16)), dim3(256), H3_LDS_BYTES, ctx->stream, in, out, nrows, pat, rm, ctx->tw_fwd, ctx->pack_fwd, ctx->modc);
     else
         hipLaunchKernelGGL(k_ntt_fwd<0>, dim3((unsigned)nrows), dim3(512), LDS_DOUBLES * 8, ctx->stream, (const void *)in, out, pat, rm, ctx->tw_fwd, ctx->pack_fwd, ctx->modc);
+    SFG_HIP(ctx, hipGetLastError());
+    return 0;
+}
+int launch_ntt_fwd_staged(sfg_ctx *ctx, const u64 *in, u64 *out, size_t nrows, const ModPattern &pat, bool staged) {
+    if (!staged) return launch_ntt_fwd(ctx, in, out, nrows, pat);
+    if (!nrows) return 0;
+    if (in == out) SFG_FAIL(ctx, "forward NTT: rows staged through stage 1 are transformed out of place");
+    hipLaunchKernelGGL(k_ntt_fwd_split<true>, dim3((unsigned)((nrows + 7) / 8 * 16)), dim3(256), H3_LDS_BYTES, ctx->stream, in, out, nrows, pat, dense_map(), ctx->tw_fwd, ctx->pack_fwd, ctx->modc);
     SFG_HIP(ctx, hipGetLastError());
     return 0;
 }
diff --git a/sfgwas_amd/csrc/rotate.hip b/sfgwas_amd/csrc/rotate.hip
--- a/sfgwas_amd/csrc/rotate.hip
+++ b/sfgwas_amd/csrc/rotate.hip
@@ -58,29 +58,34 @@
 }
 
 
-__global__ void __launch_bounds__(256) k_ksw_extend(const u64 *c2, const u64 *ct_in, u64 *ext, const KswConst *kcp, const ModConst *modc) {
+template <bool PRE1>
+__global__ void __launch_bounds__(256) k_ksw_extend(const u64 *c2, u64 *ext, const KswConst *kcp, const ModConst *modc, const double *tw_fwd) {
     const KswConst &kc = *kcp;
-    const int N = SFG_N, x = blockIdx.x * 256 + threadIdx.x, i = blockIdx.y; const size_t b = blockIdx.z;
+    const int N = SFG_N, n = N / 2, x = blockIdx.x * 256 + threadIdx.x, i = blockIdx.y; const size_t b = blockIdx.z;
     const ExtConst &e = kc.dig[i];
     const u64 *c2b = c2 + b * (size_t)kc.nl * N;
     u64 *eb = ext + (b * kc.beta + i) * (size_t)kc.nt * N;
-    double xs[KSW_MAXA], y[KSW_MAXA], v = 0.0;
+    double xs[2][KSW_MAXA], y[2][KSW_MAXA], v[2] = {0.0, 0.0};
 #pragma unroll
-    for (int m = 0; m < KSW_MAXA; m++) xs[m] = m < e.a ? u64_to_f64(c2b[(size_t)e.src[m] * N + x]) : 0.0;
-    if (e.a > 1) ext_prepare(e, modc, xs, y, v);
+    for (int h = 0; h < 2; h++)
+#pragma unroll
+        for (int m = 0; m < KSW_MAXA; m++) xs[h][m] = m < e.a ? u64_to_f64(c2b[(size_t)e.src[m] * N + h * n + x]) : 0.0;
+    if (e.a > 1) { ext_prepare(e, modc, xs[0], y[0], v[0]); ext_prepare(e, modc, xs[1], y[1], v[1]); }
     for (int t = 0; t < kc.nt; t++) {
         const int tg = kc.tmod[t];
-        u64 outv;
         if (kc.digit_of[t] == i) continue;
-        else if (e.a == 1) outv = f64_to_u64(canon(xs[0], modc[tg].q, modc[tg].qinv));
-        else outv = f64_to_u64(ext_target(e, tg, modc[tg].q, modc[tg].qinv, y, v));
-        eb[(size_t)t * N + x] = outv;
-    }
-}
-
-__global__ void __launch_bounds__(256) k_ksw_inner(const u64 *ext, const u64 *ct_in, const u64 *const *keys, const int *inidx, u64 *acc, const KswConst *kcp, const ModConst *modc, int nmod) {
+        const double q = modc[tg].q, qinv = modc[tg].qinv;
+        double o0, o1;
+        if (e.a == 1) { o0 = canon(xs[0][0], q, qinv); o1 = canon(xs[1][0], q, qinv); }
+        else { o0 = ext_target(e, tg, q, qinv, y[0], v[0]); o1 = ext_target(e, tg, q, qinv, y[1], v[1]); }
+        if (PRE1) { const double W = tw_fwd[(size_t)tg * N + 1]; fwd_stage1_pair(o0, o1, W, W * qinv, q, qinv, o0, o1); }
+        eb[(size_t)t * N + x] = f64_to_u64(o0); eb[(size_t)t * N + n + x] = f64_to_u64(o1);
+    }
+}
+
+__global__ void __launch_bounds__(256) k_ksw_inner(const u64 *ext, const u64 *ct_in, const u64 *const *keys, const int *inidx, u64 *acc, const KswConst *kcp, const ModConst *modc, int nmod, int nq_out) {
     const KswConst &kc = *kcp;
-    const int N = SFG_N, x = 2 * (blockIdx.x * 256 + threadIdx.x), t = blockIdx.y; const size_t b = blockIdx.z;
+    const int N = SFG_N, x = 2 * (blockIdx.x * 256 + threadIdx.x), t = (int)blockIdx.y < nq_out ? (int)blockIdx.y : (int)blockIdx.y + (kc.nl - nq_out); const size_t b = blockIdx.z;
     const int tg = kc.tmod[t];
     const double q = modc[tg].q, qinv = modc[tg].qinv;
     const u64 *key = keys[b];
@@ -99,18 +104,26 @@
     *reinterpret_cast<ulonglong2 *>(acc + ((b * 2 + 1) * (size_t)kc.nt + t) * N + x) = make_ulonglong2(f64_to_u64(canon(a1x, q, qinv)), f64_to_u64(canon(a1y, q, qinv)));
 }
 
-__global__ void __launch_bounds__(256) k_moddown_extend(const u64 *acc, u64 *ext2, const KswConst *kcp, const ModConst *modc) {
+template <bool PRE1>
+__global__ void __launch_bounds__(256) k_moddown_extend(const u64 *acc, u64 *ext2, const KswConst *kcp, const ModConst *modc, const double *tw_fwd, int nq_out) {
     const KswConst &kc = *kcp;
-    const int N = SFG_N, x = blockIdx.x * 256 + threadIdx.x, p = blockIdx.y; const size_t b = blockIdx.z;
+    const int N = SFG_N, n = N / 2, x = blockIdx.x * 256 + threadIdx.x, p = blockIdx.y; const size_t b = blockIdx.z;
     const ExtConst &e = kc.pq;
     const u64 *ap = acc + ((b * 2 + p) * (size_t)kc.nt + kc.nl) * N;
-    double xs[KSW_MAXA], y[KSW_MAXA], v = 0.0;
+    double xs[2][KSW_MAXA], y[2][KSW_MAXA], v[2] = {0.0, 0.0};
 #pragma unroll
-    for (int m = 0; m < KSW_MAXA; m++) xs[m] = m < e.a ? u64_to_f64(ap[(size_t)m * N + x]) : 0.0;
-    if (e.a > 1) ext_prepare(e, modc, xs, y, v);
-    for (int t = 0; t < kc.nl; t++) {
-        u64 outv = e.a == 1 ? f64_to_u64(canon(xs[0], modc[t].q, modc[t].qinv)) : f64_to_u64(ext_target(e, t, modc[t].q, modc[t].qinv, y, v));
-        ext2[((b * 2 + p) * (size_t)kc.nl + t) * N + x] = outv;
+    for (int h = 0; h < 2; h++)
+#pragma unroll
+        for (int m = 0; m < KSW_MAXA; m++) xs[h][m] = m < e.a ? u64_to_f64(ap[(size_t)m * N + h * n + x]) : 0.0;
+    if (e.a > 1) { ext_prepare(e, modc, xs[0], y[0], v[0]); ext_prepare(e, modc, xs[1], y[1], v[1]); }
+    for (int t = 0; t < nq_out; t++) {
+        const double q = modc[t].q, qinv = modc[t].qinv;
+        double o0, o1;
+        if (e.a == 1) { o0 = canon(xs[0][0], q, qinv); o1 = canon(xs[1][0], q, qinv); }
+        else { o0 = ext_target(e, t, q, qinv, y[0], v[0]); o1 = ext_target(e, t, q, qinv, y[1], v[1]); }
+        if (PRE1) { const double W = tw_fwd[(size_t)t * N + 1]; fwd_stage1_pair(o0, o1, W, W * qinv, q, qinv, o0, o1); }
+        u64 *row = ext2 + ((b * 2 + p) * (size_t)kc.nl + t) * N;
+        row[x] = f64_to_u64(o0); row[n + x] = f64_to_u64(o1);
     }
 }
 
@@ -144,6 +157,30 @@
     }
 }
 
+struct KswSeg { const u64 *plain; u64 *out; int start, count, accumulate, pad; };
+__global__ void __launch_bounds__(256) k_ksw_finish_sum(const u64 *ct_in, const int *inidx, const u64 *acc, const u64 *ext2, const uint16_t *const *index,
+                                                       const KswSeg *segs, const int *jobs, const KswConst *kcp, const ModConst *modc) {
+    const KswConst &kc = *kcp;
+    const int N = SFG_N, x = blockIdx.x * 256 + threadIdx.x, t = blockIdx.y;
+    const KswSeg sg = segs[blockIdx.z];
+    const double q = modc[t].q, qinv = modc[t].qinv, pinv = kc.pinv[t], pinv_q = kc.pinv_q[t];
+    const size_t w0 = (size_t)t * N + x, w1 = ((size_t)kc.nl + t) * N + x;
+    double s0 = 0.0, s1 = 0.0;
+    if (sg.accumulate) { s0 = u64_to_f64(sg.out[w0]); s1 = u64_to_f64(sg.out[w1]); }
+    if (sg.plain) { s0 += u64_to_f64(sg.plain[w0]); s1 += u64_to_f64(sg.plain[w1]); }
+    for (int k = 0; k < sg.count; k++) {
+        const size_t b = (size_t)jobs[sg.start + k];
+        const int src = index[b][x];
+        const double a0 = u64_to_f64(acc[((b * 2 + 0) * (size_t)kc.nt + t) * N + src]), e0 = u64_to_f64(ext2[((b * 2 + 0) * (size_t)kc.nl + t) * N + src]);
+        const double a1 = u64_to_f64(acc[((b * 2 + 1) * (size_t)kc.nt + t) * N + src]), e1 = u64_to_f64(ext2[((b * 2 + 1) * (size_t)kc.nl + t) * N + src]);
+        const double c0 = u64_to_f64(ct_in[((size_t)inidx[b] * 2 * (size_t)kc.nl + t) * N + src]);
+        s0 += canon(mulmod_lazy(a0 - e0, pinv, pinv_q, q) + c0, q, qinv);
+        s1 += canon(mulmod_lazy(a1 - e1, pinv, pinv_q, q), q, qinv);
+        if ((k & 7) == 7) { s0 = pred(s0, q, qinv); s1 = pred(s1, q, qinv); }
+    }
+    sg.out[w0] = f64_to_u64(canon(s0, q, qinv)); sg.out[w1] = f64_to_u64(canon(s1, q, qinv));
+}
+
 __global__ void __launch_bounds__(256) k_ct_add(const u64 *a, const u64 *b, u64 *out, int nl, const ModConst *modc, size_t total_rows) {
     const int N = SFG_N; const size_t row = blockIdx.x / (N / 256); const int m = (int)(row % nl);
     const u64 q = modc[m].qi;
@@ -151,20 +188,25 @@
     u64 v = a[off] + b[off]; out[off] = v >= q ? v - q : v;
 }
 
+struct KswSum { int nout; std::vector<int> group; std::vector<const u64 *> plain; u64 *out; size_t out_stride; int accumulate; };
 static int launch_keyswitch_jobs(sfg_ctx *ctx, const u64 *in, int nin, int level, const std::vector<int> &job_in, const std::vector<const u64 *> &keyp,
-                                 const std::vector<const uint16_t *> &idxp, const std::vector<u64 *> &outp, const u64 *add1, const F64Form *ffp = nullptr) {
+                                 const std::vector<const uint16_t *> &idxp, const std::vector<u64 *> &outp, const u64 *add1, const F64Form *ffp = nullptr,
+                                 const KswSum *sum = nullptr) {
     const int N = SFG_N, nl = level + 1;
     F64Form ff; memset(&ff, 0, sizeof ff); if (ffp) ff = *ffp;
     KswConst *kcd; KswConst kc;
     SFG_TRY(get_ksw(ctx, level, &kcd, &kc));
     const size_t ctw = (size_t)2 * nl * N;
-    const int nr = (int)job_in.size();
-    if (!nr) return 0;
+    const int nr = (int)job_in.size(), nout = sum ? sum->nout : 0;
+    if (sum && (ff.on || add1 || (int)sum->group.size() != nr || (int)sum->plain.size() != nout)) SFG_FAIL(ctx, "key switch: internal: malformed sum groups");
+    if (!nr && !nout) return 0;
+    const int nq_out = ff.on ? ff.L : nl;
+    const bool pre1 = !ctx->cfg.ntt_fwd_full;
     const size_t in_rows = (size_t)nl + (size_t)kc.beta * kc.nt, job_rows = 2 * (size_t)kc.nt + 2 * (size_t)nl;
     const size_t budget = ctx->cfg.ksw_budget;
     int in_grp = (int)(budget / (in_rows * N * 8)); if (in_grp < 1) in_grp = 1; if (in_grp > nin) in_grp = nin;
     int chunk = (int)(budget / (job_rows * N * 8)); if (chunk < 1) chunk = 1; if (chunk > nr) chunk = nr;
-    const size_t ptr_bytes = (size_t)nr * (3 * sizeof(void *) + sizeof(int)) + 256;
+    const size_t ptr_bytes = (size_t)nr * (3 * sizeof(void *) + 2 * sizeof(int)) + (size_t)nout * sizeof(KswSeg) + 256;
     const size_t ext_rows = (size_t)in_grp * kc.beta * kc.nt, ext2_rows = (size_t)chunk * 2 * nl;
     SFG_TRY(sfg_ws_reserve(ctx, (in_rows * in_grp + job_rows * chunk + ext_rows + ext2_rows) * N * 8 + ptr_bytes));
     u64 *c2 = (u64 *)ctx->ws, *ext = c2 + (size_t)in_grp * nl * N;
@@ -173,10 +215,34 @@
     const u64 **keys_all = (const u64 **)(ext2T + ext2_rows * N);
     const uint16_t **idx_all = (const uint16_t **)(keys_all + nr);
     u64 **out_all = (u64 **)(idx_all + nr);
-    int *inidx_all = (int *)(out_all + nr);
-    ModPattern pq; pq.period = nl; for (int m = 0; m < nl; m++) pq.m[m] = (int8_t)m;
+    KswSeg *segs_d = (KswSeg *)(out_all + nr);
+    int *inidx_all = (int *)(segs_d + nout);
+    int *segjobs_d = inidx_all + nr;
+    std::vector<char> seen(nout, 0);
+    std::vector<KswSeg> segs; std::vector<int> segjobs;
+    auto finish_sum = [&](const std::vector<int> &jobs, size_t c0, int nb, const u64 *bin, const int *inidx_d, const uint16_t **idx_d) -> int {
+        std::vector<int> cnt(nout, 0), at(nout, 0);
+        for (int k = 0; k < nb; k++) cnt[sum->group[jobs[c0 + k]]]++;
+        segs.clear(); segjobs.assign(nb, 0);
+        for (int i = 0, start = 0; i < nout; i++) {
+            if (nb ? !cnt[i] : seen[i]) continue;
+            KswSeg sg; sg.plain = seen[i] ? nullptr : sum->plain[i]; sg.out = sum->out + (size_t)i * sum->out_stride;
+            sg.start = start; sg.count = cnt[i]; sg.accumulate = (sum->accumulate || seen[i]) ? 1 : 0; sg.pad = 0;
+            at[i] = start; start += cnt[i]; seen[i] = 1; segs.push_back(sg);
+        }
+        for (int k = 0; k < nb; k++) segjobs[at[sum->group[jobs[c0 + k]]]++] = k;
+        if (segs.empty()) return 0;
+        SFG_TRY(sfg_upload_small(ctx, segs_d, segs.data(), segs.size() * sizeof(KswSeg)));
+        SFG_TRY(sfg_upload_small(ctx, segjobs_d, segjobs.data(), (size_t)nb * sizeof(int)));
+        hipLaunchKernelGGL(k_ksw_finish_sum, dim3(N / 256, nl, (unsigned)segs.size()), dim3(256), 0, ctx->stream, bin, inidx_d, acc, ext2T, idx_d, segs_d, segjobs_d, kcd, ctx->modc);
+        SFG_HIP(ctx, hipGetLastError());
+        return 0;
+    };
+    ModPattern pq; pq.period = nl; for (int m = 0; m < nl; m++) pq.m[m] = m < nq_out ? (int8_t)m : (int8_t)-2;
+    ModPattern pin; pin.period = nl; for (int m = 0; m < nl; m++) pin.m[m] = (int8_t)m;
     ModPattern pext; pext.period = kc.beta * kc.nt;
-    for (int i = 0; i < kc.beta; i++) for (int t = 0; t < kc.nt; t++) pext.m[i * kc.nt + t] = kc.digit_of[t] == i ? (int8_t)-2 : (int8_t)kc.tmod[t];
+    for (int i = 0; i < kc.beta; i++) for (int t = 0; t < kc.nt; t++)
+        pext.m[i * kc.nt + t] = (kc.digit_of[t] == i || (t >= nq_out && t < nl)) ? (int8_t)-2 : (int8_t)kc.tmod[t];
     ModPattern pp; pp.period = kc.np; for (int p = 0; p < kc.np; p++) pp.m[p] = (int8_t)(ctx->nq + p);
     for (int i0 = 0; i0 < nin; i0 += in_grp) {
         const int ni = nin - i0 < in_grp ? nin - i0 : in_grp;
@@ -185,34 +251,38 @@
         if (jobs.empty()) continue;
         const u64 *bin = in + (size_t)i0 * ctw;
         RowMap rm1; rm1.rpg = nl; rm1.gstride_in = ctw; rm1.gstride_out = (size_t)nl * N;
-        SFG_TRY(launch_ntt_inv_map(ctx, bin + (size_t)nl * N, c2, (size_t)ni * nl, pq, rm1));
-        hipLaunchKernelGGL(k_ksw_extend, dim3(N / 256, kc.beta, ni), dim3(256), 0, ctx->stream, c2, bin, ext, kcd, ctx->modc);
+        SFG_TRY(launch_ntt_inv_map(ctx, bin + (size_t)nl * N, c2, (size_t)ni * nl, pin, rm1));
+        if (pre1) hipLaunchKernelGGL(k_ksw_extend<true>, dim3(N / 512, kc.beta, ni), dim3(256), 0, ctx->stream, c2, ext, kcd, ctx->modc, ctx->tw_fwd);
+        else hipLaunchKernelGGL(k_ksw_extend<false>, dim3(N / 512, kc.beta, ni), dim3(256), 0, ctx->stream, c2, ext, kcd, ctx->modc, ctx->tw_fwd);
         SFG_HIP(ctx, hipGetLastError());
-        SFG_TRY(launch_ntt_fwd(ctx, ext, extT, (size_t)ni * kc.beta * kc.nt, pext));
+        SFG_TRY(launch_ntt_fwd_staged(ctx, ext, extT, (size_t)ni * kc.beta * kc.nt, pext, pre1));
         {
             const size_t nj = jobs.size();
             std::vector<const u64 *> kp(nj); std::vector<const uint16_t *> ip(nj); std::vector<u64 *> op(nj); std::vector<int> ii(nj);
-            for (size_t k = 0; k < nj; k++) { int jb = jobs[k]; kp[k] = keyp[jb]; ip[k] = idxp[jb]; op[k] = outp[jb]; ii[k] = job_in[jb] - i0; }
+            for (size_t k = 0; k < nj; k++) { int jb = jobs[k]; kp[k] = keyp[jb]; ip[k] = idxp[jb]; op[k] = sum ? nullptr : outp[jb]; ii[k] = job_in[jb] - i0; }
             SFG_TRY(sfg_upload_small(ctx, keys_all, kp.data(), nj * sizeof(void *)));
             SFG_TRY(sfg_upload_small(ctx, idx_all, ip.data(), nj * sizeof(void *)));
-            SFG_TRY(sfg_upload_small(ctx, out_all, op.data(), nj * sizeof(void *)));
+            if (!sum) SFG_TRY(sfg_upload_small(ctx, out_all, op.data(), nj * sizeof(void *)));
             SFG_TRY(sfg_upload_small(ctx, inidx_all, ii.data(), nj * sizeof(int)));
         }
         for (size_t c0 = 0; c0 < jobs.size(); c0 += chunk) {
             const int nb = (int)(jobs.size() - c0 < (size_t)chunk ? jobs.size() - c0 : (size_t)chunk);
             const u64 **keys_d = keys_all + c0; const uint16_t **idx_d = idx_all + c0; u64 **out_d = out_all + c0; int *inidx_d = inidx_all + c0;
-            hipLaunchKernelGGL(k_ksw_inner, dim3(N / 512, kc.nt, nb), dim3(256), 0, ctx->stream, extT, bin, keys_d, inidx_d, acc, kcd, ctx->modc, ctx->nmod);
+            hipLaunchKernelGGL(k_ksw_inner, dim3(N / 512, nq_out + kc.np, nb), dim3(256), 0, ctx->stream, extT, bin, keys_d, inidx_d, acc, kcd, ctx->modc, ctx->nmod, nq_out);
             SFG_HIP(ctx, hipGetLastError());
             RowMap rm4; rm4.rpg = kc.np; rm4.gstride_in = (size_t)kc.nt * N; rm4.gstride_out = (size_t)kc.nt * N;
             SFG_TRY(launch_ntt_inv_map(ctx, acc + (size_t)nl * N, acc + (size_t)nl * N, (size_t)nb * 2 * kc.np, pp, rm4));
-            hipLaunchKernelGGL(k_moddown_extend, dim3(N / 256, 2, nb), dim3(256), 0, ctx->stream, acc, ext2, kcd, ctx->modc);
+            if (pre1) hipLaunchKernelGGL(k_moddown_extend<true>, dim3(N / 512, 2, nb), dim3(256), 0, ctx->stream, acc, ext2, kcd, ctx->modc, ctx->tw_fwd, nq_out);
+            else hipLaunchKernelGGL(k_moddown_extend<false>, dim3(N / 512, 2, nb), dim3(256), 0, ctx->stream, acc, ext2, kcd, ctx->modc, ctx->tw_fwd, nq_out);
             SFG_HIP(ctx, hipGetLastError());
-            SFG_TRY(launch_ntt_fwd(ctx, ext2, ext2T, (size_t)nb * 2 * nl, pq));
-            hipLaunchKernelGGL(k_ksw_finish, dim3(N / 256, nl, nb), dim3(256), 0, ctx->stream, bin, inidx_d, acc, ext2T, idx_d, out_d, kcd, ctx->modc,
+            SFG_TRY(launch_ntt_fwd_staged(ctx, ext2, ext2T, (size_t)nb * 2 * nl, pq, pre1));
+            if (sum) { SFG_TRY(finish_sum(jobs, c0, nb, bin, inidx_d, idx_d)); continue; }
+            hipLaunchKernelGGL(k_ksw_finish, dim3(N / 256, nq_out, nb), dim3(256), 0, ctx->stream, bin, inidx_d, acc, ext2T, idx_d, out_d, kcd, ctx->modc,
                                add1 ? add1 + (size_t)i0 * nl * N : nullptr, ff);
             SFG_HIP(ctx, hipGetLastError());
         }
     }
+    if (sum) SFG_TRY(finish_sum(std::vector<int>(), 0, 0, in, inidx_all, idx_all));
     return 0;
 }
 int launch_rotate_right_indexed(sfg_ctx *ctx, const u64 *in, int nin, u64 *out, int nct, int level, const int *nrot_host, const int *in_index) {
@@ -237,6 +307,30 @@
         job_in.push_back(src); keyp.push_back(it->second.key_dev); idxp.push_back(it->second.index_dev); outp.push_back(out + j * ctw);
     }
     return launch_keyswitch_jobs(ctx, in, nin, level, job_in, keyp, idxp, outp, nullptr);
+}
+int launch_rotate_right_sum(sfg_ctx *ctx, const u64 *in, int nin, int nct, int level, const int *nrot_host, const int *in_index, const int *group, int nout,
+                            u64 *out, size_t out_stride, int accumulate) {
+    const int N = SFG_N, nl = level + 1;
+    if (level < 0 || level >= ctx->nq) SFG_FAIL(ctx, "rotate: level out of range");
+    const size_t ctw = (size_t)2 * nl * N;
+    KswSum sum; sum.nout = nout; sum.plain.assign(nout, nullptr); sum.out = out; sum.out_stride = out_stride; sum.accumulate = accumulate;
+    std::vector<int> job_in; std::vector<const u64 *> keyp; std::vector<const uint16_t *> idxp;
+    for (int j = 0; j < nct; j++) {
+        int nrot = nrot_host[j] % SFG_SLOTS; if (nrot < 0) nrot += SFG_SLOTS;
+        const int src = in_index ? in_index[j] : j;
+        if (src < 0 || src >= nin) SFG_FAIL(ctx, "rotate: input index out of range");
+        if (group[j] < 0 || group[j] >= nout) SFG_FAIL(ctx, "rotate: sum group out of range");
+        if (nrot == 0) {
+            if (sum.plain[group[j]]) SFG_FAIL(ctx, "rotate: more than one unrotated member in a sum group");
+            sum.plain[group[j]] = in + (size_t)src * ctw;
+            continue;
+        }
+        u64 g = sfg_galois_for_rotation(ctx, SFG_SLOTS - nrot);
+        auto it = ctx->rotkeys().find(g);
+        if (it == ctx->rotkeys().end()) SFG_FAIL(ctx, "rotate: no rotation key loaded for right-rotation by %d (galois element %llu)", nrot, g);
+        job_in.push_back(src); keyp.push_back(it->second.key_dev); idxp.push_back(it->second.index_dev); sum.group.push_back(group[j]);
+    }
+    return launch_keyswitch_jobs(ctx, in, nin, level, job_in, keyp, idxp, std::vector<u64 *>(), nullptr, nullptr, &sum);
 }
 int launch_rotate_right_indexed_f64(sfg_ctx *ctx, const u64 *in, int nin, double *outf, int nct, int level, const int *nrot_host, const int *in_index, int L,
                                     const size_t *out_slot) {
```
